# HKUDS/GPT-ST

Measured on AMD Instinct MI355X. Metric: pretrain steps/sec at (B=32,T=12,N=170,C=64), higher is better.
Workload: dtype f32; 1 GPU; BASELINE configs[1]: PEMS08-shape synthetic pretrain step, per-GPU B=32 T=12 N=170 C=64 base=1, epoch 200/300 (adaptive mask + KL), fwd+loss+bwd+clip+Adam, hipGraph=True, 4 full optimiser steps on 4 different resident batches per graph replay; global_batch=32, parallelism=dp1

## Files before the change

### gpt-st_amd/csrc/hypertem.hip

```cpp
#include "mfma_tile.h"
#include "wgrad64.h"
#include "kl_guest.h"
GPTST_STAMP_TABLES(hypertem)
GPTST_HANDOFF_COUNTER(hypertem)

#define HT_T 12
#ifndef HT_OCC
#define HT_OCC 2
#endif
#ifdef GPTST_DEBUG
__device__ long long g_ht_ts[64];
static thread_local int g_ht_dbg = 0, g_ht_nt_override = 0;
extern "C" int gptst_ht_dbg(int v) { g_ht_dbg = v; return 0; }
extern "C" int gptst_ht_variant(int fwd, int bwd) { g_ht_nt_override = fwd; (void)bwd; return 0; }
extern "C" int gptst_ht_ts(long long* out) { return (int)hipMemcpyFromSymbol(out, HIP_SYMBOL(g_ht_ts), sizeof(long long) * 64); }
#define HT_DBG(d) (d)
#else
#define HT_DBG(d) 0
static constexpr int g_ht_dbg = 0, g_ht_nt_override = 0;
#endif

__device__ __forceinline__ bool ht_work_at(int L, int ntiles, int B, int& b, int& tile) {
    const int xcd = L & 7, slot = L >> 3;
    b = xcd + 8 * (slot / ntiles);
    tile = slot % ntiles;
    return b < B;
}
__device__ __forceinline__ bool ht_work(int ntiles, int B, int& b, int& tile) { return ht_work_at(blockIdx.x, ntiles, B, b, tile); }

static int ht_pick_nt(int B, int N) {
    if (g_ht_nt_override >= 4 && g_ht_nt_override <= 16) return g_ht_nt_override;
    (void)B; (void)N;
    return 16;
}

__global__ __launch_bounds__(256, HT_OCC) void hypertem_fwd_kernel(const float* __restrict__ X, const float* __restrict__ G,
                                                              const float* __restrict__ Wbt, const float* __restrict__ bbt,
                                                              float* __restrict__ R_out, float* __restrict__ out, int N, int B, int NT,
                                                              int dbg) {
    constexpr int C = 64, P = C + 4, GP = 145;
    int tsi = 0;
#ifdef GPTST_DEBUG
#define TS() do { if ((dbg & 1) && blockIdx.x == 59 && threadIdx.x == 0) g_ht_ts[tsi] = clock64(); ++tsi; } while (0)
#else
#define TS() __builtin_amdgcn_sched_barrier(0)
#endif
    TS();
    extern __shared__ __attribute__((aligned(16))) float smem[];
    float* Xs = smem;
    float* Gs = Xs + HT_T * NT * P;
    int b, tile;
    if (!ht_work((N + NT - 1) / NT, B, b, tile)) return;
    const int n0 = tile * NT;
    const int tid = threadIdx.x, lane = tid & 63, wave = tid >> 6;
    {
        const int nl = tid >> 4, c4 = tid & 15;
        const int n = min(n0 + nl, N - 1);
        float4 v[HT_T];
        float gv[9];
#pragma unroll
        for (int t = 0; t < HT_T; ++t) v[t] = ld4(X + (((size_t)b * HT_T + t) * N + n) * C + 4 * c4);
#pragma unroll
        for (int k = 0; k < 9; ++k) gv[k] = G[min(n0 * 144 + tid + k * 256, N * 144 - 1)];
        if (nl < NT) {
#pragma unroll
            for (int t = 0; t < HT_T; ++t) st4(Xs + (t * NT + nl) * P + 4 * c4, n0 + nl < N ? v[t] : f4zero());
        }
#pragma unroll
        for (int k = 0; k < 9; ++k) {
            const int i = tid + k * 256;
            if (i < NT * 144) Gs[(i / 144) * GP + i % 144] = (n0 + i / 144 < N) ? gv[k] : 0.f;
        }
    }
    __syncthreads();
    TS();
    const int j = lane & 15, kk = lane >> 4;
    const int ja = j < NT ? j : 0;
    float4 bv[C / 16][4];
    float4 b4;
#define HT_LOAD_W(tt) do {                                                                                         \
        const float* W_ = Wbt + ((size_t)b * HT_T + (tt)) * C * C;                                                 \
        _Pragma("unroll") for (int q = 0; q < C / 16; ++q)                                                         \
            _Pragma("unroll") for (int e = 0; e < 4; ++e) bv[q][e] = ld4(W_ + (size_t)(16 * q + 4 * kk + e) * C + 4 * j); \
        b4 = ld4(bbt + ((size_t)b * HT_T + (tt)) * C + 4 * j);                                                     \
    } while (0)
    HT_LOAD_W(wave);
    for (int t = wave; t < HT_T; t += 4) {
        const size_t g = (size_t)b * HT_T + t;
        TS();
        float4 a4[C / 16];
#pragma unroll
        for (int q = 0; q < C / 16; ++q) a4[q] = f4zero();
        {
            const float* gr = Gs + ja * GP + t * HT_T;
            const float* xr = Xs + ja * P + 4 * kk;
#pragma unroll
            for (int u = 0; u < HT_T; ++u) {
                const float gu = gr[u];
#pragma unroll
                for (int q = 0; q < C / 16; ++q) a4[q] = f4fma(gu, ld4(xr + u * NT * P + 16 * q), a4[q]);
            }
        }
        TS();
        f32x4 acc[C / 16];
#pragma unroll
        for (int ct = 0; ct < C / 16; ++ct) acc[ct] = (f32x4){0.f, 0.f, 0.f, 0.f};
#pragma unroll
        for (int q = 0; q < C / 16; ++q) {
            const float av[4] = {a4[q].x, a4[q].y, a4[q].z, a4[q].w};
#pragma unroll
            for (int e = 0; e < 4; ++e) {
                acc[0] = __builtin_amdgcn_mfma_f32_16x16x4f32(av[e], bv[q][e].x, acc[0], 0, 0, 0);
                acc[1] = __builtin_amdgcn_mfma_f32_16x16x4f32(av[e], bv[q][e].y, acc[1], 0, 0, 0);
                acc[2] = __builtin_amdgcn_mfma_f32_16x16x4f32(av[e], bv[q][e].z, acc[2], 0, 0, 0);
                acc[3] = __builtin_amdgcn_mfma_f32_16x16x4f32(av[e], bv[q][e].w, acc[3], 0, 0, 0);
            }
        }
        TS();
        const float4 bias = b4;
        if (t + 4 < HT_T) HT_LOAD_W(t + 4);
        TS();
        if (R_out != nullptr && j < NT && n0 + j < N) {
#pragma unroll
            for (int q = 0; q < C / 16; ++q) st4_far(R_out + (g * N + n0 + j) * C + 16 * q + 4 * kk, a4[q]);
        }
#pragma unroll
        for (int r = 0; r < 4; ++r) {
            const int nl = kk * 4 + r;
            if (nl < NT && n0 + nl < N) {
                float4 y = f4add(f4add(make_float4(acc[0][r], acc[1][r], acc[2][r], acc[3][r]), bias), ld4(Xs + (t * NT + nl) * P + 4 * j));
                y.x = lrelu(y.x); y.y = lrelu(y.y); y.z = lrelu(y.z); y.w = lrelu(y.w);
                st4(out + (g * N + n0 + nl) * C + 4 * j, y);
            }
        }
        TS();
    }
}

static size_t ht_smem(int NT) { return ((size_t)HT_T * NT * 68 + NT * 145) * sizeof(float); }

extern "C" int gptst_hypertem_fwd(const float* X, const float* G, const float* Wbt, const float* bbt, float* R_out, float* out, int B,
                                  int T, int N, int C, void* stream) {
    if (!X || !G || !Wbt || !bbt || !out || T != HT_T) return GPTST_EARG;
    if (C != 64) return GPTST_ESHAPE;
    static int done = 0;
    if (!done) { hipFuncSetAttribute((const void*)hypertem_fwd_kernel, hipFuncAttributeMaxDynamicSharedMemorySize, (int)ht_smem(16)); done = 1; }
    const int NT = ht_pick_nt(B, N);
    hipLaunchKernelGGL(hypertem_fwd_kernel, dim3(8 * ((B + 7) / 8) * ((N + NT - 1) / NT)), dim3(256), ht_smem(NT), (hipStream_t)stream, X, G, Wbt, bbt, R_out, out, N, B, NT, g_ht_dbg);
    GPTST_CHECK_LAUNCH();
    return GPTST_OK;
}

template <bool HASY, bool PREMUL, int PAIR>
__device__ __forceinline__ void hypertem_bwd_stage(const float* __restrict__ dOut, const float* __restrict__ Y,
                                                   const float* __restrict__ X, const float* __restrict__ G,
                                                   const float* __restrict__ Wbt, float* __restrict__ dX,
                                                   float* __restrict__ dbias, float* __restrict__ dG, int N, int B, int dbg, int b, int tile,
                                                   float* __restrict__ smem, float4 (&dp)[HT_T]) {
    constexpr int C = 64, P = C + 4, GP = 145, NT = 16;
    float* Ds = smem;
    float* Gs = Ds + HT_T * NT * P;
    const int n0 = tile * NT;
    const int tid = threadIdx.x, lane = tid & 63, wave = tid >> 6;
    const int nl = tid >> 4, c4 = tid & 15;
    const bool valid = n0 + nl < N;
    const size_t rowoff = ((size_t)b * HT_T * N + min(n0 + nl, N - 1)) * C + 4 * c4;
    const int j = lane & 15, kk = lane >> 4;
    float4 aq[C / 16][C / 16];
#define HT_LOAD_WT(tt) do {                                                                                         \
        const float* W_ = Wbt + ((size_t)b * HT_T + (tt)) * C * C;                                                  \
        _Pragma("unroll") for (int it = 0; it < C / 16; ++it)                                                       \
            _Pragma("unroll") for (int q = 0; q < C / 16; ++q) aq[it][q] = ld4(W_ + (size_t)(it * 16 + j) * C + 16 * q + 4 * kk); \
    } while (0)
    static_assert(!(HASY && PREMUL), "one sign operand per launch");
    const float* __restrict__ Sg = HASY ? Y : X;
    float4 yv[HT_T];
    float gv[9];
    unsigned sb0 = 0u, sb1 = 0u;
#pragma unroll
    for (int t = 0; t < 4; ++t) { if (PAIR != 2) dp[t] = ld4(dOut + rowoff + (size_t)t * N * C); if (HASY || PREMUL) yv[t] = ld4(Sg + rowoff + (size_t)t * N * C); }
#pragma unroll
    for (int k = 0; k < 9; ++k) gv[k] = G[min(n0 * 144 + tid + k * 256, N * 144 - 1)];
    HT_LOAD_WT(wave);
#pragma unroll
    for (int t = 4; t < HT_T; ++t) { if (PAIR != 2) dp[t] = ld4(dOut + rowoff + (size_t)t * N * C); if (HASY || PREMUL) yv[t] = ld4(Sg + rowoff + (size_t)t * N * C); }
    SB();
#pragma unroll
    for (int grp = 0; grp < HT_T / 4; ++grp) {
#pragma unroll
        for (int tt = 0; tt < 4; ++tt) {
            const int t = 4 * grp + tt;
            float4 v = dp[t];
            if (HASY) v = make_float4(dp[t].x * lrelu_grad_from_out(yv[t].x), dp[t].y * lrelu_grad_from_out(yv[t].y),
                                      dp[t].z * lrelu_grad_from_out(yv[t].z), dp[t].w * lrelu_grad_from_out(yv[t].w));
            if (PREMUL) {
                const unsigned m4 = (yv[t].x > 0.f ? 1u : 0u) | (yv[t].y > 0.f ? 2u : 0u) | (yv[t].z > 0.f ? 4u : 0u) | (yv[t].w > 0.f ? 8u : 0u);
                if (t < 8) sb0 |= m4 << (4 * t); else sb1 |= m4 << (4 * (t - 8));
            }
            if (!valid) v = f4zero();
            dp[t] = v;
            st4(Ds + (t * NT + nl) * P + 4 * c4, v);
        }
        if (grp == 0) {
#pragma unroll
            for (int k = 0; k < 9; ++k) {
                const int i = tid + k * 256;
                Gs[(i / 144) * GP + i % 144] = (n0 + i / 144 < N) ? gv[k] : 0.f;
            }
        }
        __syncthreads();
        SB();
        if (PAIR != 0 && grp == 0) GPTST_STAMP(PAIR == 2 ? 6 : 1);
        const int t = 4 * grp + wave;
        if (HT_DBG(dbg) & 32) continue;
        const size_t g = (size_t)b * HT_T + t;
        float* dt = Ds + t * NT * P;
        float s = 0.f;
        if (dbias != nullptr) {
#pragma unroll
            for (int r = 0; r < NT; ++r) s += dt[r * P + lane];
        }
        float4 bq[C / 16];
#pragma unroll
        for (int q = 0; q < C / 16; ++q) bq[q] = ld4(dt + j * P + 16 * q + 4 * kk);
        f32x4 acc[C / 16];
#pragma unroll
        for (int it = 0; it < C / 16; ++it) acc[it] = (f32x4){0.f, 0.f, 0.f, 0.f};
        if (!(HT_DBG(dbg) & 64))
#pragma unroll
        for (int q = 0; q < C / 16; ++q) {
#pragma unroll
            for (int it = 0; it < C / 16; ++it) acc[it] = __builtin_amdgcn_mfma_f32_16x16x4f32(aq[it][q].x, bq[q].x, acc[it], 0, 0, 0);
#pragma unroll
            for (int it = 0; it < C / 16; ++it) acc[it] = __builtin_amdgcn_mfma_f32_16x16x4f32(aq[it][q].y, bq[q].y, acc[it], 0, 0, 0);
#pragma unroll
            for (int it = 0; it < C / 16; ++it) acc[it] = __builtin_amdgcn_mfma_f32_16x16x4f32(aq[it][q].z, bq[q].z, acc[it], 0, 0, 0);
#pragma unroll
            for (int it = 0; it < C / 16; ++it) acc[it] = __builtin_amdgcn_mfma_f32_16x16x4f32(aq[it][q].w, bq[q].w, acc[it], 0, 0, 0);
        }
        SB();
        if (t + 4 < HT_T && !(HT_DBG(dbg) & 128)) HT_LOAD_WT(t + 4);
        SB();
        if (dbias != nullptr && !(HT_DBG(dbg) & 4)) dbias[((size_t)tile * B * HT_T + g) * C + lane] = s;
#pragma unroll
        for (int it = 0; it < C / 16; ++it)
            st4(dt + j * P + it * 16 + kk * 4, make_float4(acc[it][0], acc[it][1], acc[it][2], acc[it][3]));
    }
    __syncthreads();
    if (PAIR != 0) GPTST_STAMP(PAIR == 2 ? 7 : 2);
    float4 xg[NT / 4][C / 16];
#pragma unroll
    for (int i = 0; i < NT / 4; ++i) {
        const int n = min(n0 + wave + 4 * i, N - 1);
#pragma unroll
        for (int q = 0; q < C / 16; ++q)
            xg[i][q] = j < HT_T ? ld4(X + (((size_t)b * HT_T + j) * N + n) * C + 16 * q + 4 * kk) : f4zero();
    }
    SB();
    if (valid && !(HT_DBG(dbg) & 16)) {
        float4 dr[HT_T];
#pragma unroll
        for (int t = 0; t < HT_T; ++t) dr[t] = ld4(Ds + (t * NT + nl) * P + 4 * c4);
        const float* gr = Gs + nl * GP;
#pragma unroll
        for (int u = 0; u < HT_T; ++u) {
            float4 acc = dp[u];
#pragma unroll
            for (int t = 0; t < HT_T; ++t) acc = f4fma(gr[t * HT_T + u], dr[t], acc);
            if (PREMUL) {
                const unsigned m4 = (u < 8 ? sb0 >> (4 * u) : sb1 >> (4 * (u - 8))) & 15u;
                acc.x *= (m4 & 1u) ? 1.f : LRELU_SLOPE; acc.y *= (m4 & 2u) ? 1.f : LRELU_SLOPE;
                acc.z *= (m4 & 4u) ? 1.f : LRELU_SLOPE; acc.w *= (m4 & 8u) ? 1.f : LRELU_SLOPE;
            }
            if (PAIR == 1) {
                const __amdgpu_buffer_rsrc_t rs = __builtin_amdgcn_make_buffer_rsrc(dX + (size_t)b * HT_T * N * C, 0, HT_T * N * C * 4, 0x00020000);
                st4_sc1(rs, (int)(((size_t)u * N + n0 + nl) * C + 4 * c4) * 4, acc);
                dp[u] = acc;
            } else if (!(HT_DBG(dbg) & 8)) st4(dX + rowoff + (size_t)u * N * C, acc);
            SB();
        }
    }
    SB();
    if (PAIR != 0) GPTST_STAMP(PAIR == 2 ? 8 : 3);
#pragma unroll
    for (int i = 0; i < NT / 4; ++i) {
        const int nn = wave + 4 * i, n = n0 + nn;
        if (n >= N) continue;
        f32x4 acc = {0.f, 0.f, 0.f, 0.f};
#pragma unroll
        for (int q = 0; q < C / 16; ++q) {
            const float4 a = j < HT_T ? ld4(Ds + (j * NT + nn) * P + 16 * q + 4 * kk) : f4zero();
            const float4 x = xg[i][q];
            acc = __builtin_amdgcn_mfma_f32_16x16x4f32(a.x, x.x, acc, 0, 0, 0);
            acc = __builtin_amdgcn_mfma_f32_16x16x4f32(a.y, x.y, acc, 0, 0, 0);
            acc = __builtin_amdgcn_mfma_f32_16x16x4f32(a.z, x.z, acc, 0, 0, 0);
            acc = __builtin_amdgcn_mfma_f32_16x16x4f32(a.w, x.w, acc, 0, 0, 0);
        }
#pragma unroll
        for (int r = 0; r < 4; ++r) {
            const int t = kk * 4 + r, u = j;
            if (t < HT_T && u < HT_T && !(HT_DBG(dbg) & 2)) dG[((size_t)b * N + n) * 144 + t * HT_T + u] = acc[r];
        }
    }
    if (PAIR != 0) GPTST_STAMP(PAIR == 2 ? 9 : 4);
}

template <bool HASY, bool PREMUL>
__device__ __forceinline__ void hypertem_bwd_body(const float* __restrict__ dOut, const float* __restrict__ Y,
                                                  const float* __restrict__ X, const float* __restrict__ G,
                                                  const float* __restrict__ Wbt, float* __restrict__ dX,
                                                  float* __restrict__ dbias, float* __restrict__ dG, int N, int B, int dbg, int L,
                                                  float* __restrict__ smem) {
    int b, tile;
    if (!ht_work_at(L, (N + 15) / 16, B, b, tile)) return;
    float4 dp[HT_T];
    hypertem_bwd_stage<HASY, PREMUL, 0>(dOut, Y, X, G, Wbt, dX, dbias, dG, N, B, dbg, b, tile, smem, dp);
}

template <bool HASY, bool PREMUL>
__global__ __launch_bounds__(256, HT_OCC) void hypertem_bwd_kernel(const float* __restrict__ dOut, const float* __restrict__ Y,
                                                              const float* __restrict__ X, const float* __restrict__ G,
                                                              const float* __restrict__ Wbt, float* __restrict__ dX,
                                                              float* __restrict__ dbias, float* __restrict__ dG, int N, int B, int dbg) {
    extern __shared__ __attribute__((aligned(16))) float smem[];
    hypertem_bwd_body<HASY, PREMUL>(dOut, Y, X, G, Wbt, dX, dbias, dG, N, B, dbg, blockIdx.x, smem);
}

template <bool HASY>
__device__ __forceinline__ void wgrad64_mix_body(const float* __restrict__ X, const float* __restrict__ G, const float* __restrict__ D,
                                                 const float* __restrict__ D2, float* __restrict__ dW, int N, int b, int t,
                                                 float* __restrict__ smem) {
    constexpr int C = 64, U = 2;
    float (*red)[C * C] = reinterpret_cast<float (*)[C * C]>(smem);
    float (*csred)[C] = reinterpret_cast<float (*)[C]>(smem + 4 * C * C);
    const int lane = threadIdx.x & 63, wave = threadIdx.x >> 6;
    const int j = lane & 15, kk = lane >> 4;
    const int q = (N + 3) / 4;
    const int mbeg = wave * q, mend = min(N, mbeg + q);
    const size_t g = (size_t)b * HT_T + t;
    f32x4 acc[4][4];
#pragma unroll
    for (int ca = 0; ca < 4; ++ca)
#pragma unroll
        for (int cb = 0; cb < 4; ++cb) acc[ca][cb] = (f32x4){0.f, 0.f, 0.f, 0.f};
    float4 sa = f4zero();
    for (int m0 = mbeg; m0 < mend; m0 += 4 * U) {
        float4 x[U][HT_T], gq[U][3], d[U], y[U];
#pragma unroll
        for (int u = 0; u < U; ++u) {
            const int m = min(m0 + 4 * u + kk, mend - 1);
#pragma unroll
            for (int k = 0; k < 3; ++k) gq[u][k] = ld4(G + (size_t)m * 144 + t * HT_T + 4 * k);
#pragma unroll
            for (int uu = 0; uu < HT_T; ++uu) x[u][uu] = ld4(X + (((size_t)b * HT_T + uu) * N + m) * C + 4 * j);
            const size_t off = (g * N + m) * C + 4 * j;
            d[u] = ld4(D + off);
            if (HASY) y[u] = ld4(D2 + off);
        }
        SB();
#pragma unroll
        for (int u = 0; u < U; ++u) {
            const float gs[HT_T] = {gq[u][0].x, gq[u][0].y, gq[u][0].z, gq[u][0].w, gq[u][1].x, gq[u][1].y, gq[u][1].z, gq[u][1].w,
                                    gq[u][2].x, gq[u][2].y, gq[u][2].z, gq[u][2].w};
            float4 a = f4zero();
#pragma unroll
            for (int uu = 0; uu < HT_T; ++uu) a = f4fma(gs[uu], x[u][uu], a);
            if (m0 + 4 * u + kk >= mend) a = f4zero();
            if (HASY) {
                d[u].x = __fmul_rn(d[u].x, lrelu_grad_from_out(y[u].x)); d[u].y = __fmul_rn(d[u].y, lrelu_grad_from_out(y[u].y));
                d[u].z = __fmul_rn(d[u].z, lrelu_grad_from_out(y[u].z)); d[u].w = __fmul_rn(d[u].w, lrelu_grad_from_out(y[u].w));
            }
            if (m0 + 4 * u + kk < mend) sa = make_float4(__fadd_rn(sa.x, d[u].x), __fadd_rn(sa.y, d[u].y), __fadd_rn(sa.z, d[u].z), __fadd_rn(sa.w, d[u].w));
            const float av[4] = {a.x, a.y, a.z, a.w}, dv[4] = {d[u].x, d[u].y, d[u].z, d[u].w};
#pragma unroll
            for (int ca = 0; ca < 4; ++ca)
#pragma unroll
                for (int cb = 0; cb < 4; ++cb) acc[ca][cb] = __builtin_amdgcn_mfma_f32_16x16x4f32(av[ca], dv[cb], acc[ca][cb], 0, 0, 0);
        }
        SB();
    }
#pragma unroll
    for (int ca = 0; ca < 4; ++ca)
#pragma unroll
        for (int r = 0; r < 4; ++r)
            st4(&red[wave][(4 * (kk * 4 + r) + ca) * C + 4 * j], make_float4(acc[ca][0][r], acc[ca][1][r], acc[ca][2][r], acc[ca][3][r]));
    sa.x += __shfl_xor(sa.x, 16, 64); sa.y += __shfl_xor(sa.y, 16, 64); sa.z += __shfl_xor(sa.z, 16, 64); sa.w += __shfl_xor(sa.w, 16, 64);
    sa.x += __shfl_xor(sa.x, 32, 64); sa.y += __shfl_xor(sa.y, 32, 64); sa.z += __shfl_xor(sa.z, 32, 64); sa.w += __shfl_xor(sa.w, 32, 64);
    if (kk == 0) st4(&csred[wave][4 * j], sa);
    __syncthreads();
    float* o = dW + g * (size_t)(C * C + C);
    if (threadIdx.x < C) o[C * C + threadIdx.x] = csred[0][threadIdx.x] + csred[1][threadIdx.x] + csred[2][threadIdx.x] + csred[3][threadIdx.x];
#pragma unroll
    for (int k = 0; k < C * C / 4 / 256; ++k) {
        const int f = threadIdx.x + k * 256;
        const float4 s = f4add(f4add(ld4(&red[0][4 * f]), ld4(&red[1][4 * f])), f4add(ld4(&red[2][4 * f]), ld4(&red[3][4 * f])));
        st4(o + 4 * f, s);
    }
}

template <int U, bool HASY, bool PREMUL, bool MIX>
__global__ __launch_bounds__(256, HT_OCC) void hypertem_bwd_wgrad_kernel(const float* __restrict__ dOut, const float* __restrict__ Y,
                                                                    const float* __restrict__ X, const float* __restrict__ G,
                                                                    const float* __restrict__ Wbt, const float* __restrict__ R,
                                                                    float* __restrict__ dX, float* __restrict__ dG, float* __restrict__ dWb,
                                                                    int N, int B, int nH, RowMap rm, int rows_per_split) {
    extern __shared__ __attribute__((aligned(16))) float smem[];
    if ((int)blockIdx.x < nH) {
        hypertem_bwd_body<HASY, PREMUL>(dOut, Y, X, G, Wbt, dX, nullptr, dG, N, B, 0, blockIdx.x, smem);
    } else if (MIX) {
        int b, t;
        if (!ht_work_at(blockIdx.x - nH, HT_T, B, b, t)) return;
        wgrad64_mix_body<HASY>(X, G, dOut, Y, dWb, N, b, t, smem);
    } else {
        const int w = blockIdx.x - nH;
        wgrad64_body<HASY ? PRO_DPRE : PRO_NONE, U>(R, dOut, Y, dWb, rm, rows_per_split, 64 * 64 + 64, 2, w % rm.G, w / rm.G, smem);
    }
}

extern "C" int gptst_hypertem_ntiles(int N) { return (N + 15) / 16; }

extern "C" int gptst_hypertem_bwd(const float* dOut, const float* Y, const float* X, const float* G, const float* Wbt, float* dX,
                                  float* dbias, float* dG, int premul, int B, int T, int N, int C, void* stream) {
    if (!dOut || !X || !G || !Wbt || !dX || !dG || T != HT_T || (Y && premul)) return GPTST_EARG;
    if (C != 64) return GPTST_ESHAPE;
    const size_t smem = ht_smem(16);
    static int done = 0;
    if (!done) {
        hipFuncSetAttribute((const void*)hypertem_bwd_kernel<true, false>, hipFuncAttributeMaxDynamicSharedMemorySize, (int)smem);
        hipFuncSetAttribute((const void*)hypertem_bwd_kernel<false, false>, hipFuncAttributeMaxDynamicSharedMemorySize, (int)smem);
        hipFuncSetAttribute((const void*)hypertem_bwd_kernel<false, true>, hipFuncAttributeMaxDynamicSharedMemorySize, (int)smem);
        done = 1;
    }
    const dim3 grid(8 * ((B + 7) / 8) * ((N + 15) / 16));
    if (Y) hipLaunchKernelGGL((hypertem_bwd_kernel<true, false>), grid, dim3(256), smem, (hipStream_t)stream, dOut, Y, X, G, Wbt, dX, dbias, dG, N, B, g_ht_dbg);
    else if (premul) hipLaunchKernelGGL((hypertem_bwd_kernel<false, true>), grid, dim3(256), smem, (hipStream_t)stream, dOut, Y, X, G, Wbt, dX, dbias, dG, N, B, g_ht_dbg);
    else hipLaunchKernelGGL((hypertem_bwd_kernel<false, false>), grid, dim3(256), smem, (hipStream_t)stream, dOut, Y, X, G, Wbt, dX, dbias, dG, N, B, g_ht_dbg);
    GPTST_CHECK_LAUNCH();
    return GPTST_OK;
}

extern "C" int gptst_wgrad_nsplit(int mode, int BT, int N, int C);
template <bool HASY, bool PREMUL>
static void ht_bwd_wgrad_launch(const float* dOut, const float* Y, const float* X, const float* G, const float* Wbt, const float* R, float* dX,
                                float* dG, float* dWb, int B, int N, bool u6, int nH, int nW, RowMap rm, int rps, size_t smem, hipStream_t st) {
    static int done = 0;
    if (!done) {
        hipFuncSetAttribute((const void*)hypertem_bwd_wgrad_kernel<4, HASY, PREMUL, false>, hipFuncAttributeMaxDynamicSharedMemorySize, (int)smem);
        hipFuncSetAttribute((const void*)hypertem_bwd_wgrad_kernel<6, HASY, PREMUL, false>, hipFuncAttributeMaxDynamicSharedMemorySize, (int)smem);
        hipFuncSetAttribute((const void*)hypertem_bwd_wgrad_kernel<4, HASY, PREMUL, true>, hipFuncAttributeMaxDynamicSharedMemorySize, (int)smem);
        done = 1;
    }
    if (R == nullptr) hipLaunchKernelGGL((hypertem_bwd_wgrad_kernel<4, HASY, PREMUL, true>), dim3(nH + 8 * ((B + 7) / 8) * HT_T), dim3(256), smem, st, dOut, Y, X, G, Wbt, R, dX, dG, dWb, N, B, nH, rm, rps);
    else if (u6) hipLaunchKernelGGL((hypertem_bwd_wgrad_kernel<6, HASY, PREMUL, false>), dim3(nH + nW), dim3(256), smem, st, dOut, Y, X, G, Wbt, R, dX, dG, dWb, N, B, nH, rm, rps);
    else hipLaunchKernelGGL((hypertem_bwd_wgrad_kernel<4, HASY, PREMUL, false>), dim3(nH + nW), dim3(256), smem, st, dOut, Y, X, G, Wbt, R, dX, dG, dWb, N, B, nH, rm, rps);
}

extern "C" int gptst_hypertem_bwd_wgrad(const float* dOut, const float* Y, const float* X, const float* G, const float* Wbt, const float* R,
                                        float* dX, float* dG, float* dWb, int premul, int B, int T, int N, int C, void* stream) {
    if (!dOut || !X || !G || !Wbt || !dX || !dG || !dWb || T != HT_T || (Y && premul)) return GPTST_EARG;
    if (C != 64) return GPTST_ESHAPE;
    const size_t smem_h = ht_smem(16), smem_w = WGRAD64_SMEM_FLOATS * sizeof(float), smem = smem_h > smem_w ? smem_h : smem_w;
    const RowMap rm = make_rowmap(0, B * T, N);
    const int ns = gptst_wgrad_nsplit(0, B * T, N, 64);
    if (!R && ns != 1) return GPTST_ESHAPE;
    int rps = (rm.M + ns - 1) / ns;
    rps = (rps + 1) & ~1;
    const int rows = rps < rm.M ? rps : rm.M, steps = ((rows + 3) / 4 + 3) / 4;
    const bool u6 = (steps + 5) / 6 * 6 <= (steps + 3) / 4 * 4;
    const int nH = 8 * ((B + 7) / 8) * ((N + 15) / 16), nW = rm.G * ns;
    if (Y) ht_bwd_wgrad_launch<true, false>(dOut, Y, X, G, Wbt, R, dX, dG, dWb, B, N, u6, nH, nW, rm, rps, smem, (hipStream_t)stream);
    else if (premul) ht_bwd_wgrad_launch<false, true>(dOut, Y, X, G, Wbt, R, dX, dG, dWb, B, N, u6, nH, nW, rm, rps, smem, (hipStream_t)stream);
    else ht_bwd_wgrad_launch<false, false>(dOut, Y, X, G, Wbt, R, dX, dG, dWb, B, N, u6, nH, nW, rm, rps, smem, (hipStream_t)stream);
    GPTST_CHECK_LAUNCH();
    return GPTST_OK;
}

struct HtPairArgs {
    const float* dOut1; const float* X1; const float* G1; const float* Wbt1; const float* R1;
    const float* X0; const float* G0; const float* Wbt0; const float* R0;
    float* dXmid; float* dX0; float* dG1; float* dG0; float* dWb1; float* dWb0; unsigned* cnt;
};

template <int U>
__global__ __launch_bounds__(256, HT_OCC) void hypertem_bwd_pair_kernel(HtPairArgs a, int N, int B, int nH, RowMap rm, int rows_per_split) {
    extern __shared__ __attribute__((aligned(16))) float smem[];
    const int ntiles = (N + 15) / 16;
    if ((int)blockIdx.x < nH) {
        int b, tile;
        if (!ht_work_at(blockIdx.x, ntiles, B, b, tile)) return;
        float4 dp[HT_T];
        GPTST_WG_BEGIN(); GPTST_STAMP(0);
        hypertem_bwd_stage<false, true, 1>(a.dOut1, nullptr, a.X1, a.G1, a.Wbt1, a.dXmid, nullptr, a.dG1, N, B, 0, b, tile, smem, dp);
        asm volatile("s_waitcnt vmcnt(0)" ::: "memory");
        __syncthreads();
        if (threadIdx.x == 0) { gptst_publish_fence(); __hip_atomic_fetch_add(a.cnt + b, 1u, __ATOMIC_RELAXED, __HIP_MEMORY_SCOPE_AGENT); }
        GPTST_STAMP(5);
        hypertem_bwd_stage<false, true, 2>(nullptr, nullptr, a.X0, a.G0, a.Wbt0, a.dX0, nullptr, a.dG0, N, B, 0, b, tile, smem, dp);
        GPTST_WG_END();
        return;
    }
    GPTST_WG_BEGIN();
    const int nW = rm.G * ((rm.M + rows_per_split - 1) / rows_per_split);
    int w = blockIdx.x - nH;
    if (w < nW) {
        wgrad64_body<PRO_NONE, U>(a.R1, a.dOut1, nullptr, a.dWb1, rm, rows_per_split, 64 * 64 + 64, 2, w % rm.G, w / rm.G, smem);
        GPTST_WG_END();
        return;
    }
    w -= nW;
    const int g = w % rm.G, sp = w / rm.G;
    unsigned* s_ok = reinterpret_cast<unsigned*>(smem);
    if (threadIdx.x == 0) *s_ok = gptst_wait_ge(a.cnt + g / HT_T, (unsigned)ntiles, &g_handoff_lost_hypertem) ? 1u : 0u;
    __syncthreads();
    const bool ok = *s_ok != 0u;
    __syncthreads();
    wgrad64_body<PRO_NONE, U, true>(a.R0, a.dXmid, nullptr, a.dWb0, rm, rows_per_split, 64 * 64 + 64, 2, g, sp, smem);
    if (!ok) a.dWb0[((size_t)sp * rm.G + g) * (size_t)(64 * 64 + 64) + threadIdx.x] = __int_as_float(0x7fc00000);
    GPTST_WG_END();
}

extern "C" int gptst_hypertem_bwd_pair(const float* dOut1, const float* X1, const float* G1, const float* Wbt1, const float* R1, const float* X0,
                                       const float* G0, const float* Wbt0, const float* R0, float* dXmid, float* dX0, float* dG1, float* dG0,
                                       float* dWb1, float* dWb0, void* cnt, int B, int T, int N, int C, void* stream) {
    if (!dOut1 || !X1 || !G1 || !Wbt1 || !R1 || !X0 || !G0 || !Wbt0 || !R0 || !dXmid || !dX0 || !dG1 || !dG0 || !dWb1 || !dWb0 || !cnt || T != HT_T)
        return GPTST_EARG;
    if (C != 64 || (size_t)HT_T * N * C * 4 >= ((size_t)1 << 31)) return GPTST_ESHAPE;
    const size_t smem_h = ht_smem(16), smem_w = WGRAD64_SMEM_FLOATS * sizeof(float), smem = smem_h > smem_w ? smem_h : smem_w;
    const RowMap rm = make_rowmap(0, B * T, N);
    const int ns = gptst_wgrad_nsplit(0, B * T, N, 64);
    int rps = (rm.M + ns - 1) / ns;
    rps = (rps + 1) & ~1;
    if ((rm.M + rps - 1) / rps != ns || (size_t)B * T * N * C * 4 >= ((size_t)1 << 31)) return GPTST_ESHAPE;
    const int rows = rps < rm.M ? rps : rm.M, steps = ((rows + 3) / 4 + 3) / 4;
    const bool u6 = (steps + 5) / 6 * 6 <= (steps + 3) / 4 * 4;
    const int nH = 8 * ((B + 7) / 8) * ((N + 15) / 16), nW = rm.G * ns;
    static int done = 0;
    if (!done) {
        hipFuncSetAttribute((const void*)hypertem_bwd_pair_kernel<4>, hipFuncAttributeMaxDynamicSharedMemorySize, (int)smem);
        hipFuncSetAttribute((const void*)hypertem_bwd_pair_kernel<6>, hipFuncAttributeMaxDynamicSharedMemorySize, (int)smem);
        done = 1;
    }
    const HtPairArgs a{dOut1, X1, G1, Wbt1, R1, X0, G0, Wbt0, R0, dXmid, dX0, dG1, dG0, dWb1, dWb0, (unsigned*)cnt};
    if (u6) hipLaunchKernelGGL((hypertem_bwd_pair_kernel<6>), dim3(nH + 2 * nW), dim3(256), smem, (hipStream_t)stream, a, N, B, nH, rm, rps);
    else hipLaunchKernelGGL((hypertem_bwd_pair_kernel<4>), dim3(nH + 2 * nW), dim3(256), smem, (hipStream_t)stream, a, N, B, nH, rm, rps);
    GPTST_CHECK_LAUNCH();
    return GPTST_OK;
}

struct HtStage { const float* G; const float* Wbt; const float* bbt; float* R_out; float* out; };
struct HtChain {
    int nstage;
    const float* X;
    HtStage st[3];
};

#ifndef HTC_NW
#define HTC_NW 4
#endif
template <int NSTAGE, int GUEST>
__global__ __launch_bounds__(64 * HTC_NW, HTC_NW == 6 ? 3 : HT_OCC) void hypertem_chain_fwd_kernel(HtChain ch, int N, int B, KlGuest kg) {
    constexpr int C = 64, P = C + 4, GP = 145, NT = 16, NW = HTC_NW, NTH = 64 * NW, TPW = HT_T / NW;
    static_assert(HT_T % NW == 0 && (HT_T * NT * (C / 4)) % NTH == 0 && (NT * 144) % NTH == 0, "waves must divide the steps and the staging loops");
    constexpr int GK = NT * 144 / NTH, XK = HT_T * NT * (C / 4) / NTH;
    extern __shared__ __attribute__((aligned(16))) float smem[];
    float* Xs = smem;
    float* Gs = Xs + HT_T * NT * P;
    if constexpr (GUEST != 0) {
        static_assert(NTH == 256, "the guest bodies are written for 256 threads");
        if ((int)blockIdx.x >= kg.base) { kl_guest_run<GUEST>(kg, kg.v0 + (int)blockIdx.x - kg.base, smem); return; }
    }
    int b, tile;
    if (!ht_work((N + NT - 1) / NT, B, b, tile)) return;
    const int n0 = tile * NT;
    const int tid = threadIdx.x, lane = tid & 63, wave = tid >> 6;
    const int j = lane & 15, kk = lane >> 4;
    float gv[GK];
#define HTC_LOAD_G(Gp) _Pragma("unroll") for (int k = 0; k < GK; ++k) gv[k] = (Gp)[min(n0 * 144 + tid + k * NTH, N * 144 - 1)]
#define HTC_STORE_G() _Pragma("unroll") for (int k = 0; k < GK; ++k) { const int i = tid + k * NTH; \
        Gs[(i / 144) * GP + i % 144] = (n0 + i / 144 < N) ? gv[k] : 0.f; }
    float4 bv[C / 16][4];
    float4 b4;
#define HTC_LOAD_W(W0, b0, tt) do {                                                                                \
        const float* W_ = (W0) + ((size_t)b * HT_T + (tt)) * C * C;                                                \
        _Pragma("unroll") for (int q = 0; q < C / 16; ++q)                                                         \
            _Pragma("unroll") for (int e = 0; e < 4; ++e) bv[q][e] = ld4(W_ + (size_t)(16 * q + 4 * kk + e) * C + 4 * j); \
        b4 = ld4((b0) + ((size_t)b * HT_T + (tt)) * C + 4 * j);                                                    \
    } while (0)

    {
        float4 v[XK];
#pragma unroll
        for (int k = 0; k < XK; ++k) {
            const int i = tid + k * NTH, t = i >> 8, nl = (i & 255) >> 4, c4 = i & 15;
            v[k] = ld4(ch.X + (((size_t)b * HT_T + t) * N + min(n0 + nl, N - 1)) * C + 4 * c4);
        }
        HTC_LOAD_G(ch.st[0].G);
#pragma unroll
        for (int k = 0; k < XK; ++k) {
            const int i = tid + k * NTH, t = i >> 8, nl = (i & 255) >> 4, c4 = i & 15;
            st4(Xs + (t * NT + nl) * P + 4 * c4, n0 + nl < N ? v[k] : f4zero());
        }
        HTC_STORE_G();
    }
    __syncthreads();
    SB();

#pragma unroll
    for (int s = 0; s < NSTAGE; ++s) {
        const HtStage S = ch.st[s];
        const HtStage S1 = ch.st[s + 1 < 3 ? s + 1 : 2];
        if (s + 1 < NSTAGE) {
            float4 a4a[C / 16], a4b[C / 16], a4c[C / 16];
#pragma unroll
            for (int q = 0; q < C / 16; ++q) { a4a[q] = f4zero(); a4b[q] = f4zero(); a4c[q] = f4zero(); }
            {
                const float* gr = Gs + j * GP + wave * HT_T;
                const float* xr = Xs + j * P + 4 * kk;
#pragma unroll
                for (int u = 0; u < HT_T; ++u) {
                    float4 x[C / 16];
#pragma unroll
                    for (int q = 0; q < C / 16; ++q) x[q] = ld4(xr + u * NT * P + 16 * q);
                    const float g0 = gr[u], g1 = gr[NW * HT_T + u], g2 = TPW == 3 ? gr[2 * NW * HT_T + u] : 0.f;
#pragma unroll
                    for (int q = 0; q < C / 16; ++q) {
                        a4a[q] = f4fma(g0, x[q], a4a[q]);
                        a4b[q] = f4fma(g1, x[q], a4b[q]);
                        if (TPW == 3) a4c[q] = f4fma(g2, x[q], a4c[q]);
                    }
                    if (TPW == 3 ? u % 3 == 2 : u % 2 == 1) SB();
                }
            }
            HTC_LOAD_W(S.Wbt, S.bbt, wave);
            HTC_LOAD_G(S1.G);
            __syncthreads();
            SB();
#pragma nounroll
            for (int ti = 0; ti < TPW; ++ti) {
                const int t = wave + NW * ti;
                const size_t g = (size_t)b * HT_T + t;
                float4 m4[C / 16];
#pragma unroll
                for (int q = 0; q < C / 16; ++q) { m4[q] = a4a[q]; a4a[q] = a4b[q]; a4b[q] = a4c[q]; }
                f32x4 acc[C / 16];
#pragma unroll
                for (int ct = 0; ct < C / 16; ++ct) acc[ct] = (f32x4){0.f, 0.f, 0.f, 0.f};
#pragma unroll
                for (int q = 0; q < C / 16; ++q) {
                    const float av[4] = {m4[q].x, m4[q].y, m4[q].z, m4[q].w};
#pragma unroll
                    for (int e = 0; e < 4; ++e) {
                        acc[0] = __builtin_amdgcn_mfma_f32_16x16x4f32(av[e], bv[q][e].x, acc[0], 0, 0, 0);
                        acc[1] = __builtin_amdgcn_mfma_f32_16x16x4f32(av[e], bv[q][e].y, acc[1], 0, 0, 0);
                        acc[2] = __builtin_amdgcn_mfma_f32_16x16x4f32(av[e], bv[q][e].z, acc[2], 0, 0, 0);
                        acc[3] = __builtin_amdgcn_mfma_f32_16x16x4f32(av[e], bv[q][e].w, acc[3], 0, 0, 0);
                    }
                }
                SB();
                const float4 bias = b4;
                if (ti < TPW - 1) HTC_LOAD_W(S.Wbt, S.bbt, t + NW);
                SB();
                if (S.R_out != nullptr && n0 + j < N) {
#pragma unroll
                    for (int q = 0; q < C / 16; ++q) st4_far(S.R_out + (g * N + n0 + j) * C + 16 * q + 4 * kk, m4[q]);
                }
#pragma unroll
                for (int r = 0; r < 4; ++r) {
                    const int nl = kk * 4 + r;
                    float* xs = Xs + (t * NT + nl) * P + 4 * j;
                    float4 y = f4add(f4add(make_float4(acc[0][r], acc[1][r], acc[2][r], acc[3][r]), bias), ld4(xs));
                    y.x = lrelu(y.x); y.y = lrelu(y.y); y.z = lrelu(y.z); y.w = lrelu(y.w);
                    if (n0 + nl < N) st4(S.out + (g * N + n0 + nl) * C + 4 * j, y);
                    else y = f4zero();
                    st4(xs, y);
                }
                SB();
            }
            HTC_STORE_G();
            __syncthreads();
            SB();
        } else {
            HTC_LOAD_W(S.Wbt, S.bbt, wave);
            for (int t = wave; t < HT_T; t += NW) {
                const size_t g = (size_t)b * HT_T + t;
                SB();
                float4 a4[C / 16];
#pragma unroll
                for (int q = 0; q < C / 16; ++q) a4[q] = f4zero();
                {
                    const float* gr = Gs + j * GP + t * HT_T;
                    const float* xr = Xs + j * P + 4 * kk;
#pragma unroll
                    for (int u = 0; u < HT_T; ++u) {
                        const float gu = gr[u];
#pragma unroll
                        for (int q = 0; q < C / 16; ++q) a4[q] = f4fma(gu, ld4(xr + u * NT * P + 16 * q), a4[q]);
                    }
                }
                SB();
                f32x4 acc[C / 16];
#pragma unroll
                for (int ct = 0; ct < C / 16; ++ct) acc[ct] = (f32x4){0.f, 0.f, 0.f, 0.f};
#pragma unroll
                for (int q = 0; q < C / 16; ++q) {
                    const float av[4] = {a4[q].x, a4[q].y, a4[q].z, a4[q].w};
#pragma unroll
                    for (int e = 0; e < 4; ++e) {
                        acc[0] = __builtin_amdgcn_mfma_f32_16x16x4f32(av[e], bv[q][e].x, acc[0], 0, 0, 0);
                        acc[1] = __builtin_amdgcn_mfma_f32_16x16x4f32(av[e], bv[q][e].y, acc[1], 0, 0, 0);
                        acc[2] = __builtin_amdgcn_mfma_f32_16x16x4f32(av[e], bv[q][e].z, acc[2], 0, 0, 0);
                        acc[3] = __builtin_amdgcn_mfma_f32_16x16x4f32(av[e], bv[q][e].w, acc[3], 0, 0, 0);
                    }
                }
                SB();
                const float4 bias = b4;
                if (t + NW < HT_T) HTC_LOAD_W(S.Wbt, S.bbt, t + NW);
                SB();
                if (S.R_out != nullptr && n0 + j < N) {
#pragma unroll
                    for (int q = 0; q < C / 16; ++q) st4_far(S.R_out + (g * N + n0 + j) * C + 16 * q + 4 * kk, a4[q]);
                }
#pragma unroll
                for (int r = 0; r < 4; ++r) {
                    const int nl = kk * 4 + r;
                    if (n0 + nl < N) {
                        float4 y = f4add(f4add(make_float4(acc[0][r], acc[1][r], acc[2][r], acc[3][r]), bias), ld4(Xs + (t * NT + nl) * P + 4 * j));
                        y.x = lrelu(y.x); y.y = lrelu(y.y); y.z = lrelu(y.z); y.w = lrelu(y.w);
                        st4(S.out + (g * N + n0 + nl) * C + 4 * j, y);
                    }
                }
            }
        }
    }
#undef HTC_LOAD_G
#undef HTC_STORE_G
#undef HTC_LOAD_W
}

static int ht_chain_args(HtChain& ch, const float* X, int nstage, const void* Gs, const void* Wbts, const void* bbts, const void* Rs, const void* outs,
                         int B, int T, int N, int C) {
    if (!X || nstage < 1 || nstage > 3 || !Gs || !Wbts || !bbts || !Rs || !outs || T != HT_T || B <= 0 || N <= 0) return GPTST_EARG;
    if (C != 64) return GPTST_ESHAPE;
    ch.nstage = nstage; ch.X = X;
    for (int s = 0; s < 3; ++s) {
        const int k = s < nstage ? s : nstage - 1;
        ch.st[s] = HtStage{((const float* const*)Gs)[k], ((const float* const*)Wbts)[k], ((const float* const*)bbts)[k],
                           ((float* const*)Rs)[k], ((float* const*)outs)[k]};
        if (!ch.st[s].G || !ch.st[s].Wbt || !ch.st[s].bbt || !ch.st[s].out) return GPTST_EARG;
    }
    return GPTST_OK;
}

static int ht_chain_grid(int B, int N) { return 8 * ((B + 7) / 8) * ((N + 15) / 16); }

extern "C" int gptst_hypertem_chain_fwd(const float* X, int nstage, const void* Gs, const void* Wbts, const void* bbts, const void* Rs,
                                        const void* outs, int B, int T, int N, int C, void* stream) {
    HtChain ch;
    const int rc = ht_chain_args(ch, X, nstage, Gs, Wbts, bbts, Rs, outs, B, T, N, C);
    if (rc != GPTST_OK) return rc;
    const dim3 grid(ht_chain_grid(B, N));
    const int smem = (int)ht_smem(16);
    hipStream_t st = (hipStream_t)stream;
    const KlGuest none{};
#define HTC_LAUNCH(NS_) do {                                                                                                          \
        static int done_ = 0;                                                                                                          \
        if (!done_) { (void)hipFuncSetAttribute((const void*)hypertem_chain_fwd_kernel<NS_, 0>, hipFuncAttributeMaxDynamicSharedMemorySize, smem); done_ = 1; } \
        hipLaunchKernelGGL((hypertem_chain_fwd_kernel<NS_, 0>), grid, dim3(64 * HTC_NW), smem, st, ch, N, B, none);                          \
    } while (0)
    if (nstage == 1) HTC_LAUNCH(1); else if (nstage == 2) HTC_LAUNCH(2); else HTC_LAUNCH(3);
#undef HTC_LAUNCH
    GPTST_CHECK_LAUNCH();
    return GPTST_OK;
}

GPTST_INTERNAL int gptst_tail_geometry(int rows, int* rows_per_block);
GPTST_INTERNAL int gptst_apply_wgrad_geometry(int mode, int BT, int N, int* tpw);

extern "C" int gptst_kl_guest_blocks(int stage, int B, int T, int N) {
    if (B <= 0 || T <= 0 || N <= 0) return GPTST_EARG;
    int aux;
    if (stage == 1) return gptst_tail_geometry(B * T * N, &aux);
    if (stage == 2) return B * T * gptst_apply_wgrad_geometry(0, B * T, N, &aux);
    if (stage == 3) return N;
    return GPTST_EARG;
}

extern "C" int gptst_hypertem_chain_fwd_kl(const float* X, int nstage, const void* Gs, const void* Wbts, const void* bbts, const void* Rs,
                                           const void* outs, int B, int T, int N, int C, int stage, const void* ops, int v0, int v1, int HS,
                                           int lda, float w, void* stream) {
    HtChain ch;
    const int rc = ht_chain_args(ch, X, nstage, Gs, Wbts, bbts, Rs, outs, B, T, N, C);
    if (rc != GPTST_OK) return rc;
    if (!ops || stage < 1 || stage > 3) return GPTST_EARG;
    if (nstage != 2 || HTC_NW != 4 || HS <= 0 || HS > TL_MAXJ) return GPTST_ESHAPE;
    const int nv = gptst_kl_guest_blocks(stage, B, T, N);
    if (v0 < 0 || v1 <= v0 || v1 > nv) return GPTST_EARG;
    const float* const* p = (const float* const*)ops;
    const int np = stage == 1 ? 7 : stage == 2 ? 6 : 7;
    for (int i = 0; i < np; ++i) if (!p[i]) return GPTST_EARG;
    KlGuest kg{};
    kg.base = ht_chain_grid(B, N);
    kg.v0 = v0;
    if (stage == 1) {
        TailArgs& t = kg.tail;
        t.X = p[0]; t.W = p[1]; t.prob = p[2]; t.c = p[3]; t.dX = (float*)p[4]; t.part = (float*)p[5]; t.sws = (float*)p[6];
        t.rows = B * T * N; t.J = HS; t.N = N; t.w = w; t.premul = 1;
        gptst_tail_geometry(t.rows, &t.rows_per_block);
    } else if (stage == 2) {
        kg.dOut = p[0]; kg.S = p[1]; kg.W = p[2]; kg.dS = (float*)p[3]; kg.dW = (float*)p[4]; kg.colsum = (float*)p[5];
        kg.rm = make_rowmap(0, B * T, N);
        gptst_apply_wgrad_geometry(0, B * T, N, &kg.tpw);
    } else {
        if (lda <= 0) return GPTST_EARG;
        kg.dPre = p[0]; kg.src = p[1]; kg.lda = lda; kg.w1 = p[2]; kg.b1 = p[3]; kg.Wn = p[4]; kg.dWb = (float*)p[5]; kg.dinp = (float*)p[6];
        kg.BT = B * T; kg.N = N;
    }
    const dim3 grid(kg.base + (v1 - v0));
    const size_t sg = kl_guest_lds_bytes(stage), sh = ht_smem(16);
    const int smem = (int)(sg > sh ? sg : sh);
    hipStream_t st = (hipStream_t)stream;
#define HTC_LAUNCH(G_) do {                                                                                                           \
        static int done_ = 0;                                                                                                          \
        if (!done_) { (void)hipFuncSetAttribute((const void*)hypertem_chain_fwd_kernel<2, G_>, hipFuncAttributeMaxDynamicSharedMemorySize, smem); done_ = 1; } \
        hipLaunchKernelGGL((hypertem_chain_fwd_kernel<2, G_>), grid, dim3(64 * HTC_NW), smem, st, ch, N, B, kg);                           \
    } while (0)
    if (stage == 1) HTC_LAUNCH(1); else if (stage == 2) HTC_LAUNCH(2); else HTC_LAUNCH(3);
#undef HTC_LAUNCH
    GPTST_CHECK_LAUNCH();
    return GPTST_OK;
}
```

### gpt-st_amd/csrc/wgrad64.h

```cpp
#pragma once
#include "common.h"

enum { PRO_NONE = 0, PRO_DPRE = 1 };
enum { EPI_PLAIN = 0, EPI_RES_LRELU = 1, EPI_ADD_DPRE = 2, EPI_LRELU = 3, EPI_ADD_PREMUL = 4, EPI_PREMUL = 5 };

struct RowMap {
    int G, M;
    long rs_g, rs_m;
};

__host__ __device__ inline RowMap make_rowmap(int mode, int BT, int N) {
    RowMap r;
    if (mode == 0) { r.G = BT; r.M = N; r.rs_g = N; r.rs_m = 1; }
    else if (mode == 1) { r.G = N; r.M = BT; r.rs_g = 1; r.rs_m = N; }
    else { r.G = 1; r.M = BT * N; r.rs_g = 0; r.rs_m = 1; }
    return r;
}


#define WGRAD64_SMEM_FLOATS (4 * 64 * 64 + 4 * 64)

template <int PRO, int U, bool ACQ = false>
__device__ __forceinline__ void wgrad64_body(const float* __restrict__ A, const float* __restrict__ D, const float* __restrict__ D2,
                                             float* __restrict__ dW, RowMap rm, int rows_per_split, int ostride, int csa, int g, int sp,
                                             float* __restrict__ smem) {
    constexpr int C = 64;
    float (*red)[C * C] = reinterpret_cast<float (*)[C * C]>(smem);
    float (*csred)[C] = reinterpret_cast<float (*)[C]>(smem + 4 * C * C);
    const int lane = threadIdx.x & 63, wave = threadIdx.x >> 6;
    const int j = lane & 15, kk = lane >> 4;
    const int mbeg0 = sp * rows_per_split;
    const int mend0 = min(rm.M, mbeg0 + rows_per_split);
    const int q = (mend0 - mbeg0 + 3) / 4;
    const int mbeg = mbeg0 + wave * q, mend = min(mend0, mbeg + q);
    f32x4 acc[4][4];
#pragma unroll
    for (int ca = 0; ca < 4; ++ca)
#pragma unroll
        for (int cb = 0; cb < 4; ++cb) acc[ca][cb] = (f32x4){0.f, 0.f, 0.f, 0.f};
    float4 sa = f4zero();
    const __amdgpu_buffer_rsrc_t rsD = __builtin_amdgcn_make_buffer_rsrc(const_cast<float*>(D), 0, ACQ ? (int)((size_t)rm.G * rm.M * C * 4) : 0, 0x00020000);
    for (int m0 = mbeg; m0 < mend; m0 += 4 * U) {
        float4 a[U], d[U], y[U];
#pragma unroll
        for (int u = 0; u < U; ++u) {
            const int m = min(m0 + 4 * u + kk, mend - 1);
            const size_t off = ((size_t)g * rm.rs_g + (size_t)m * rm.rs_m) * C + 4 * j;
            a[u] = ld4(A + off); d[u] = ACQ ? ld4_sc1(rsD, (int)(off * 4)) : ld4(D + off);
            if (PRO == PRO_DPRE) y[u] = ld4(D2 + off);
        }
        SB();
#pragma unroll
        for (int u = 0; u < U; ++u) {
            if (m0 + 4 * u + kk >= mend) a[u] = f4zero();
            if (PRO == PRO_DPRE) {
                d[u].x = __fmul_rn(d[u].x, lrelu_grad_from_out(y[u].x)); d[u].y = __fmul_rn(d[u].y, lrelu_grad_from_out(y[u].y));
                d[u].z = __fmul_rn(d[u].z, lrelu_grad_from_out(y[u].z)); d[u].w = __fmul_rn(d[u].w, lrelu_grad_from_out(y[u].w));
            }
            if (csa == 2) {
                if (m0 + 4 * u + kk < mend) sa = make_float4(__fadd_rn(sa.x, d[u].x), __fadd_rn(sa.y, d[u].y), __fadd_rn(sa.z, d[u].z), __fadd_rn(sa.w, d[u].w));
            }
            else sa = f4add(sa, a[u]);
            const float av[4] = {a[u].x, a[u].y, a[u].z, a[u].w}, dv[4] = {d[u].x, d[u].y, d[u].z, d[u].w};
#pragma unroll
            for (int ca = 0; ca < 4; ++ca)
#pragma unroll
                for (int cb = 0; cb < 4; ++cb) acc[ca][cb] = __builtin_amdgcn_mfma_f32_16x16x4f32(av[ca], dv[cb], acc[ca][cb], 0, 0, 0);
        }
    }
#pragma unroll
    for (int ca = 0; ca < 4; ++ca)
#pragma unroll
        for (int r = 0; r < 4; ++r)
            st4(&red[wave][(4 * (kk * 4 + r) + ca) * C + 4 * j], make_float4(acc[ca][0][r], acc[ca][1][r], acc[ca][2][r], acc[ca][3][r]));
    if (csa) {
        sa.x += __shfl_xor(sa.x, 16, 64); sa.y += __shfl_xor(sa.y, 16, 64); sa.z += __shfl_xor(sa.z, 16, 64); sa.w += __shfl_xor(sa.w, 16, 64);
        sa.x += __shfl_xor(sa.x, 32, 64); sa.y += __shfl_xor(sa.y, 32, 64); sa.z += __shfl_xor(sa.z, 32, 64); sa.w += __shfl_xor(sa.w, 32, 64);
        if (kk == 0) st4(&csred[wave][4 * j], sa);
    }
    __syncthreads();
    float* o = dW + ((size_t)sp * rm.G + g) * (size_t)ostride;
    if (csa && threadIdx.x < C) o[C * C + threadIdx.x] = csred[0][threadIdx.x] + csred[1][threadIdx.x] + csred[2][threadIdx.x] + csred[3][threadIdx.x];
#pragma unroll
    for (int k = 0; k < C * C / 4 / 256; ++k) {
        const int f = threadIdx.x + k * 256;
        const float4 s = f4add(f4add(ld4(&red[0][4 * f]), ld4(&red[1][4 * f])), f4add(ld4(&red[2][4 * f]), ld4(&red[3][4 * f])));
        st4(o + 4 * f, s);
    }
}
```

### gpt-st_amd/engine.py

```python
import contextlib
import os
import threading
from typing import Any, NamedTuple

import torch

from . import _C, ops
from .ops import (EPI_ADD_DPRE, EPI_ADD_PREMUL, EPI_LRELU, EPI_PREMUL, EPI_PLAIN, EPI_RES_LRELU, MODE_NODE, MODE_SHARED, MODE_TIME, PRO_DPRE, PRO_NONE)

TF_NAMES = ("ln_day", "ln_week", "ln1", "ln2", "ln")


class ZeroArena:

    def __init__(self, device):
        self.device, self.buf, self.off, self.need = device, None, 0, 0

    def begin(self, zero=True):
        pending = None
        if self.buf is None or self.buf.numel() < self.need:
            self.buf = torch.zeros(max(self.need, 1), device=self.device) if self.need else None
        elif self.buf is not None:
            if zero:
                self.buf.zero_()
            else:
                pending = self.buf
        self.off, self.need = 0, 0
        return pending

    def zeros(self, *shape):
        n = 1
        for d in shape:
            n *= d
        n4 = (n + 3) // 4 * 4
        self.need += n4
        if self.buf is None or self.off + n4 > self.buf.numel():
            return torch.zeros(*shape, device=self.device)
        t = self.buf[self.off:self.off + n].view(*shape)
        self.off += n4
        return t


class _Context(threading.local):
    ARENA = None
    NODE_REDUCE = None
    NO_HANDOFFS = False


CTX = _Context()




class Reductions:

    def __init__(self):
        self.jobs = ops.PoolJobs()
        self.late = ops.PoolJobs()
        self.no_carry = False
        self.grams = []
        self.tf = []
        self.keep = []
        self.on_bucket = None
        self.nbucket = 0
        self.bucket_inline = False
        self.fork_side = None
        self.forked = False
        self._dG = self._dA = None

    def take_carry(self, mb):
        if not CARRY_RED or self.no_carry or self.on_bucket is not None or CTX.NODE_REDUCE is not None or not self.jobs.jobs:
            return None
        take, rest, nb = [], [], 0.0
        for j in self.jobs.jobs:
            b = 4.0 * j.R * j.cols * j.nsplit / 2 ** 20
            if j.kind in (ops.PoolJobs.BWD_POOL, ops.PoolJobs.BWD_EMB) and nb + b <= mb and len(take) < 100 and (j.cols | j.ldx) % 4 == 0:
                take.append(j); nb += b
            else:
                rest.append(j)
        if not take:
            return None
        self.jobs.jobs = rest
        c = ops.PoolJobs()
        c.jobs = take
        return c

    def untake(self, carry):
        if carry is not None and carry.jobs:
            self.jobs.jobs = carry.jobs + self.jobs.jobs
            carry.jobs = []

    def gram(self, A, dG, dA, N, nsG):
        self.grams.append((A, dG, dA, N, nsG))

    def timefeat(self, p, g, pfx, tidx, dout, spg=False):
        self.tf.append(_tf_job(p, pfx, tidx, spg)._replace(grads=_tf_tensors(g, pfx), dout=dout))

    def flush_async(self, tidx):
        if self.bucket_inline and self.on_bucket is not None and self.nbucket == 0 and (self.jobs.jobs or self.late.jobs or self.grams or self.tf):
            self._run(tidx)
            self.fork_side.wait_stream(torch.cuda.current_stream())
            with torch.cuda.stream(self.fork_side):
                self.on_bucket(0)
            self.forked = True
            self.nbucket += 1

    def flush(self, tidx):
        self._run(tidx)
        if self.forked:
            torch.cuda.current_stream().wait_stream(self.fork_side)
            self.forked = False

    def _run(self, tidx):
        gr, self.grams = sorted(self.grams, key=lambda t: t[0].data_ptr()), []
        while gr:
            A, dG, dA, N, nsG = gr.pop(0)
            while gr and gr[0][0].data_ptr() == A.data_ptr() + 4 * A.numel() and gr[0][1].data_ptr() == dG.data_ptr() + 4 * dG.numel() \
                    and gr[0][2].data_ptr() == dA.data_ptr() + 4 * dA.numel() and gr[0][3:] == (N, nsG):
                A2, dG2, dA2 = gr.pop(0)[:3]
                A = torch.as_strided(A, (A.shape[0] + A2.shape[0],) + tuple(A.shape[1:]), A.stride())
                dG = torch.as_strided(dG, (dG.shape[0] + dG2.shape[0],) + tuple(dG.shape[1:]), dG.stride())
                dA = torch.as_strided(dA, (dA.shape[0] + dA2.shape[0],) + tuple(dA.shape[1:]), dA.stride())
            ops.gram_bwd(A, dG, out=dA, layers=A.shape[0] // N, nsplit=nsG)
        self.jobs.jobs, self.late.jobs = self.jobs.jobs + self.late.jobs, []
        self.jobs.launch()
        tf, self.tf = self.tf, []
        ops.timefeat_jobs_bwd(tf, tidx)
        self.keep = []


def _zeros(ref, *shape):
    if CTX.ARENA is not None:
        return CTX.ARENA.zeros(*shape)
    return torch.zeros(*shape, device=ref.device)


def _tf_tensors(d, pfx):
    out = []
    for n in TF_NAMES:
        out += [d[pfx + n + ".weight"], d[pfx + n + ".bias"]]
    return out


def _tf_job(p, pfx, tidx, spg=False):
    B, T = tidx.shape[0], tidx.shape[1]
    rows, K = (B, T) if spg else (B * T, 1)
    return ops.TimefeatJob(_tf_tensors(p, pfx), rows, K)


DROP_R = os.environ.get("GPTST_DROP_R", "0") == "1"


class HtSaved(NamedTuple):
    x: Any
    R: Any
    out: Any
    G: Any
    Wbt: Any


class WgradParts(NamedTuple):
    dW: Any
    ns: int
    db: Any


def _ht_fused_bwd(dims):
    return dims[3] == 64 and FUSE_HT_BWD


def hypertem_core_fwd(x, G, Wbt, bbt, dims):
    B, T, N, C = dims
    if C == 64:
        keep = not (DROP_R and _ht_fused_bwd(dims) and ops.wgrad_nsplit(MODE_TIME, B * T, N, C) == 1)
        R, out = ops.hypertem_fwd(x.view(B, T, N, C), G, Wbt, bbt, want_R=keep)
        R, out = (R.view(-1, C) if keep else None), out.view(-1, C)
    else:
        R = ops.tmix(x.view(B, T, N, C), G).view(-1, C)
        out = ops.apply(R, Wbt, MODE_TIME, B * T, N, bias=bbt, resid=x, epi=EPI_RES_LRELU)
    return out, HtSaved(x, R, out, G, Wbt)


FUSE_HT_BWD = True


def graph_grad_splits(dims):
    return dims[0] if dims[3] == 64 else 1


CHAIN128 = os.environ.get("GPTST_CHAIN128", "1") == "1"


def chain_ok(dims):
    return _ht_fused_bwd(dims) or (CHAIN128 and dims[3] == 128)


def _wb_parts(dWb, C, ns=1):
    return WgradParts(dWb[:, :C * C], ns, dWb[:, C * C:])


def _wgrad_parts(a, dout, out, mode, dims):
    B, T, N, C = dims
    dWb, ns = ops.wgrad(a, dout, mode, B * T, N, D2=out, pro=PRO_NONE if out is None else PRO_DPRE, colsum_d=True)
    return _wb_parts(dWb, C, ns)


def _genlin_bwd(dout, out, x, W, mode, dims, chain, premul=False):
    B, T, N, C = dims
    BT = B * T
    if C == 64:
        dx, dW, db, ns = ops.apply_wgrad(dout, None if chain else out, x, W, mode, BT, N, premul=chain and premul)
        return dx, WgradParts(dW, ns, db)
    if chain:
        dx = (ops.apply(dout, W, mode, BT, N, transw=True, resid2=x, epi=EPI_PREMUL) if premul
              else ops.apply(dout, W, mode, BT, N, transw=True))
        return dx, _wgrad_parts(x, dout, None, mode, dims)
    dx = ops.apply(dout, W, mode, BT, N, A2=out, transw=True, pro=PRO_DPRE)
    return dx, _wgrad_parts(x, dout, out, mode, dims)


def hypertem_core_bwd(saved, dout, dG_out, dims, chain=False, premul=False):
    B, T, N, C = dims
    x, R, out, G, Wbt = saved
    BT = B * T
    v = lambda a: a.view(B, T, N, C)
    assert not chain or chain_ok(dims)
    if _ht_fused_bwd(dims):
        dx, dWb, ns, _ = ops.hypertem_bwd_wgrad(v(dout), None if chain else v(out), v(x), G, Wbt, v(R) if R is not None else None, dG=dG_out,
                                                premul=chain and premul)
        return dx.view(-1, C), _wb_parts(dWb, C, ns)
    hp = _wgrad_parts(R, dout, None if chain else out, MODE_TIME, dims)
    if C == 64:
        dx, _, _ = ops.hypertem_bwd(v(dout), v(out), v(x), G, Wbt, dG=dG_out, want_dbias=False)
    elif chain:
        dR = ops.apply(dout, Wbt, MODE_TIME, BT, N, transw=True)
        dx, _ = ops.tmix_bwd_chain(v(dR), v(x), G, v(dout), premul=premul, dG=dG_out[0])
    else:
        dR = ops.apply(dout, Wbt, MODE_TIME, BT, N, A2=out, transw=True, pro=PRO_DPRE)
        dx, _ = ops.tmix_bwd(v(dR), v(x), G, v(dout), v(out), dG=dG_out[0])
    return dx.view(-1, C), hp


CARRY_RED = os.environ.get("GPTST_CARRY_RED", "1") == "1"
CARRY_MB = float(os.environ.get("GPTST_CARRY_MB", "25"))
CARRY_KL = os.environ.get("GPTST_CARRY_KL", "1") == "1"
PAIR_UNDER_DP = os.environ.get("GPTST_PAIR_UNDER_DP", "1") == "1"
PAIR_BWD = os.environ.get("GPTST_PAIR_BWD", "1") == "1"


@contextlib.contextmanager
def no_handoffs():
    from . import _C
    keep = (CTX.NO_HANDOFFS, _C.lib().value("gptst_mask_cooperative_state"))
    CTX.NO_HANDOFFS = True
    _C.lib().call("gptst_mask_cooperative", 0)
    try:
        yield
    finally:
        CTX.NO_HANDOFFS = keep[0]
        _C.lib().call("gptst_mask_cooperative", keep[1])


def pair_bwd_on():
    return PAIR_BWD and not CTX.NO_HANDOFFS


def cross_role():
    return 0 if CTX.NO_HANDOFFS else CROSS_ROLE


def _ht_pair_shape_ok(dims):
    B, T, N, C = dims
    if T != 12 or C != 64:
        return False
    ns = ops.wgrad_nsplit(MODE_TIME, B * T, N, C)
    rps = (-(-N // ns) + 1) & ~1
    return -(-N // rps) == ns


def ht_pair_ok(saved1, saved0, dims):
    return (pair_bwd_on() and dims[3] == 64 and not isinstance(saved1, EncIn) and saved1.R is not None and saved0.R is not None
            and _ht_fused_bwd(dims) and _ht_pair_shape_ok(dims))


class PendingH1:

    def __init__(self, saved, dd, dG, dWb):
        self.saved, self.dd, self.dG, self.dWb = saved, dd, dG, dWb


def ht_pair_bwd(saved1, saved0, dout, dG1, dG0, dims, dWb1=None):
    B, T, N, C = dims
    if not ht_pair_ok(saved1, saved0, dims):
        assert dWb1 is None
        return None
    s1, s0 = saved1, saved0
    v = lambda a: a.view(B, T, N, C)
    r = ops.hypertem_bwd_pair(v(dout), v(s1.x), s1.G, s1.Wbt, v(s1.R), v(s0.x), s0.G, s0.Wbt, v(s0.R), dG1, dG0, _zeros(dout, B), dWb1=dWb1)
    assert r is not None or dWb1 is None
    if r is None:
        return None
    dmid, dx0, dWb1, dWb0, ns = r
    return dx0.view(-1, C), _wb_parts(dWb1, C, ns), _wb_parts(dWb0, C, ns)


FUSE_CROSS = os.environ.get("GPTST_FUSE_CROSS", "1") == "1"
CAP_LIN = os.environ.get("GPTST_CAP_LIN", "1") == "1"
CROSS_ROLE = int(os.environ.get("GPTST_CROSS_ROLE", "1"))


class CapSaved(NamedTuple):
    x: Any
    out: Any
    rec: Any
    c: Any
    s: Any
    v: Any
    Ht: Any
    Rt: Any
    dyn: Any
    Wn: Any
    Y: Any


class CapParts(NamedTuple):
    wn: WgradParts
    ddyn: Any
    dlogit: Any


def cap_head_fwd(p, pfx, x, dadj, dyn, dims, num_route, HS, HT):
    B, T, N, C = dims
    c, s, Y = ops.cap_route_fwd(x.view(B, T, N, C), p[pfx + "ln_p.weight"], p[pfx + "ln_p.bias"], dadj, HS, num_route,
                                reduce_nodes=CTX.NODE_REDUCE, want_Y=True)
    fused = ops.cap_cross_rec_fwd(s, dyn, p[pfx + "mask_template"], c, B, T, N, HS, HT) if (FUSE_CROSS and CTX.NODE_REDUCE is None) else None
    if fused is not None:
        v, Ht, Rt, rec = fused
    else:
        v, Ht, Rt = ops.cap_cross_fwd(s, dyn, p[pfx + "mask_template"], B, T, HS, HT)
        rec = ops.cap_rec_fwd(c, v, N, C)
    return rec, c, (s, v, Ht, Rt, Y)


def cap_core_fwd(p, pfx, x, dadj, dyn, Wn, bn, dims, num_route, HS, HT):
    B, T, N, C = dims
    rec, c, (s, v, Ht, Rt, Y) = cap_head_fwd(p, pfx, x, dadj, dyn, dims, num_route, HS, HT)
    out = ops.apply(rec, Wn, MODE_NODE, B * T, N, bias=bn, resid=x, epi=EPI_RES_LRELU)
    return out, c, CapSaved(x, out, rec, c, s, v, Ht, Rt, dyn, Wn, Y)


CHAIN_FWD = os.environ.get("GPTST_CHAIN_FWD", "1") == "1"


def chain_fwd_ok(dims):
    return CHAIN_FWD and dims[3] == 64 and not DROP_R


def ht_chain_fwd(x, stages, dims, kl=None):
    B, T, N, C = dims
    res = ops.hypertem_chain_fwd(x.view(B, T, N, C), stages, guest=kl.guest() if kl is not None else None)
    saved, xin = [], x
    for (G, Wbt, _b), (R, o) in zip(stages, res):
        o = o.view(-1, C)
        saved.append(HtSaved(xin, R.view(-1, C), o, G, Wbt))
        xin = o
    return saved, xin


def cap_core_bwd(p, g, pfx, saved, dout, dims, HS, HT, red, chain=False):
    B, T, N, C = dims
    x, out, rec, c, s, v, Ht, Rt, dyn, Wn, Y = saved
    BT, dev = B * T, x.device
    assert not chain or chain_ok(dims)
    drec, wn = _genlin_bwd(dout, out, rec, Wn, MODE_NODE, dims, chain)
    dc1, dv = ops.cap_rec_bwd(drec, c, v, reduce_nodes=CTX.NODE_REDUCE)
    gw, gb = g[pfx + "ln_p.weight"], g[pfx + "ln_p.bias"]
    if FUSE_CROSS and CAP_LIN and C == 64 and CTX.NODE_REDUCE is None and Y is None:
        carry = red.take_carry(CARRY_MB) if cross_role() and _C.lib().value("gptst_cap_route_roles_ok", B, T, N, C, HS, HT) == 1 else None
        lin = ops.cap_cross_route_lin_bwd(x.view(B, T, N, C), p[pfx + "ln_p.weight"], p[pfx + "ln_p.bias"], c, dc1, dv, s, Rt, Ht, dyn,
                                          p[pfx + "mask_template"], dout, None if chain else out, chain, B, T, HS, HT,
                                          flags=_zeros(x, 4 * B) if cross_role() else None, jobs=carry)
        red.untake(carry)
        if lin is not None:
            dx, dWp, dbp, dlogit, ddyn = lin
            red.jobs.bwd_pool(_ones(dev, dWp.shape[0]), dWp, gw.view(1, C * C))
            red.jobs.bwd_pool(_ones(dev, dbp.shape[0]), dbp, gb.view(1, C))
            return dx, CapParts(wn, ddyn, dlogit)
    fused = None
    if FUSE_CROSS and CTX.NODE_REDUCE is None and Y is None:
        fused = ops.cap_cross_route_bwd(x.view(B, T, N, C), p[pfx + "ln_p.weight"], p[pfx + "ln_p.bias"], c, dc1, dv, s, Rt, Ht, dyn,
                                        p[pfx + "mask_template"], B, T, HS, HT, flags=_zeros(x, 4 * B) if cross_role() else None)
    if fused is not None:
        dY, dlogit, ddyn = fused
    else:
        dS, ddyn = ops.cap_cross_bwd(dv, s, Rt, Ht, dyn, p[pfx + "mask_template"], B, T, HS, HT)
        dY, dlogit = ops.cap_route_bwd(x.view(B, T, N, C), p[pfx + "ln_p.weight"], p[pfx + "ln_p.bias"], c, dc1, dS, Y=Y)
    if C == 64:
        dx, dWp, dbp, ns2 = ops.linear_bwd(dY, x, p[pfx + "ln_p.weight"], dout, None if chain else out, premul=chain)
        red.jobs.bwd_pool(_ones(dev, ns2), dWp, gw.view(1, C * C))
        red.jobs.bwd_pool(_ones(dev, ns2), dbp, gb.view(1, C))
    else:
        if chain:
            dx = ops.apply(dY, p[pfx + "ln_p.weight"], MODE_SHARED, BT, N, resid=dout, resid2=x, epi=EPI_ADD_PREMUL)
        else:
            dx = ops.apply(dY, p[pfx + "ln_p.weight"], MODE_SHARED, BT, N, resid=dout, resid2=out, epi=EPI_ADD_DPRE)
        dWp, ns2 = ops.wgrad(dY, x, MODE_SHARED, BT, N, colsum_a=True)
        wp = _wb_parts(dWp, C, ns2)
        red.jobs.bwd_pool(_ones(dev, ns2), wp.dW, gw.view(1, C * C))
        red.jobs.bwd_pool(_ones(dev, ns2), wp.db, gb.view(1, C))
    return dx, CapParts(wn, ddyn, dlogit)


_ONES = {}


def _ones(dev, n=1):
    if (dev, n) not in _ONES:
        _ONES[(dev, n)] = torch.ones(n, 1, device=dev)
    return _ONES[(dev, n)]


class CondLinSaved(NamedTuple):
    x: Any
    out: Any
    W: Any


def condlin_fwd(x, Wg, bg, mode, dims):
    B, T, N, C = dims
    out = ops.apply(x, Wg, mode, B * T, N, bias=bg, epi=EPI_LRELU)
    return out, CondLinSaved(x, out, Wg)


def condlin_bwd(saved, dout, emb, wpool, bpool, g_wpool, g_bpool, d_emb, mode, dims, red, chain=False, premul=False, carried=None):
    C = dims[3]
    R, K = emb.shape
    assert not chain or chain_ok(dims)
    dx, w = carried if carried is not None else _genlin_bwd(dout, saved.out, saved.x, saved.W, mode, dims, chain, premul)
    ns, db = w.ns, w.db
    dW = w.dW if w.dW.dim() == 2 else w.dW.view(ns * R, C * C)
    red.jobs.bwd_pool(emb, dW, g_wpool.view(K, C * C), nsplit=ns)
    red.jobs.bwd_pool(emb, db, g_bpool, nsplit=ns)
    red.jobs.bwd_emb(dW, wpool.view(K, C * C), d_emb, nsplit=ns)
    red.jobs.bwd_emb(db, bpool, d_emb, nsplit=ns)
    return dx


ENC, DEC = "encoder.STHCN_encode.", "decoder.STHCN_decode."
GUIDE_TF = "encoder.teb4mask."


def _sthcn_names(pfx):
    return [pfx + "hyperTem%d." % i for i in (1, 2, 3, 4)], [pfx + "cap1.", pfx + "cap2."]


class SthcnGen(NamedTuple):
    emb: Any
    A_all: Any
    G_all: Any
    Wb: Any
    Wn: Any
    dadj: Any
    dyn: Any
    hts: Any
    cps: Any
    d: int
    Hm: int
    ds: int
    HS: int
    HT: int
    slot: Any

    def ht(self, i):
        return (self.G_all[i],) + self.Wb[i]


class SthcnSaved(NamedTuple):
    h1: Any
    h2: Any
    h3: Any
    h4: Any
    c1: Any
    c2: Any
    emb: Any
    gen: SthcnGen
    slot: Any


class GenAll(NamedTuple):
    sthcn: Any
    guide: Any
    pending: Any


def _sthcn_gen_jobs(p, pfx, emb, jobs, A_all, dims, G_all, slot=None):
    B, T, N, C = dims
    time_eb, teb, tes = emb
    ne, nes = p[pfx + "node_embeddings"], p[pfx + "node_embeddings_spg"]
    hts, cps = _sthcn_names(pfx)
    adj0 = p[hts[0] + "adj"]
    d, Hm = adj0.shape[0], adj0.shape[1]
    cadj, tadj = p[cps[0] + "adj"], p[cps[0] + "t_adj"]
    ds, HS, HT = cadj.shape[0], cadj.shape[1], tadj.shape[1]
    for i, h in enumerate(hts):
        jobs.fwd(ne, p[h + "adj"].view(d, Hm * T), out=A_all[i])
        jobs.gram(ne, p[h + "adj"].view(d, Hm * T), out=G_all[i], A=A_all[i])
    Wb = [(jobs.fwd(time_eb, p[h + "weights_pool"]), jobs.fwd(time_eb, p[h + "bias_pool"])) for h in hts]
    Wn = [(jobs.fwd(nes, p[c + "weights_spa"]), jobs.fwd(nes, p[c + "bias_spa"])) for c in cps]
    dadj = [jobs.fwd(teb, p[c + "adj"].view(ds, HS * N)) for c in cps]
    dyn = [jobs.fwd(tes, p[c + "t_adj"].view(ds, HT * T * HS)).view(B, HT, T * HS) for c in cps]
    return SthcnGen(emb, A_all, G_all, Wb, Wn, dadj, dyn, hts, cps, d, Hm, ds, HS, HT, slot)


def gen_all(p, tidx, dims, which=(ENC, DEC), guide=True, defer=False):
    B, T, N, C = dims
    tfj = []
    for pfx in which:
        tfj += [_tf_job(p, pfx + "time_feature1.", tidx), _tf_job(p, pfx + "time_feature1_.", tidx),
                _tf_job(p, pfx + "time_feature2.", tidx, spg=True)]
    if guide:
        tfj.append(_tf_job(p, GUIDE_TF, tidx))
    embs = ops.timefeat_jobs_fwd(tfj, tidx)
    jobs = ops.PoolJobs()
    now = ops.PoolJobs() if defer else jobs
    sthcn, gd = {}, None
    L = 4 * len(which)
    if guide:
        gj = now
        m = "encoder.MLP_RL."
        t4m = embs[-1]
        gd = (t4m, gj.fwd(p["encoder.neb4mask"], p[m + "weights_pool_spa"]), gj.fwd(p["encoder.neb4mask"], p[m + "bias_pool_spa"]),
              gj.fwd(t4m, p[m + "weights_pool_tem"]), gj.fwd(t4m, p[m + "bias_pool_tem"]))
    if L:
        adj0 = p[which[0] + "hyperTem1.adj"]
        Hm = adj0.shape[1]
        A_all = torch.empty(L, N, Hm * T, device=tidx.device)
        G_all = torch.empty(L, N, T, T, device=tidx.device)
        for k, pfx in enumerate(which):
            sthcn[pfx] = _sthcn_gen_jobs(p, pfx, embs[3 * k:3 * k + 3], jobs, A_all[4 * k:4 * k + 4], dims, G_all[4 * k:4 * k + 4], (k, len(which)))
    now.launch()
    return GenAll(sthcn, gd, jobs if defer else None)


def sthcn_fwd(p, pfx, tidx, x, dims, num_route, gen=None, head=None, next_gen=None, kl=None):
    if gen is None:
        gen = gen_all(p, tidx, dims, which=(pfx,), guide=False).sthcn[pfx]
    ht = gen.ht
    cap = lambda i, x: cap_core_fwd(p, gen.cps[i], x, gen.dadj[i], gen.dyn[i], *gen.Wn[i], dims, num_route, gen.HS, gen.HT)
    pairs = chain_fwd_ok(dims)
    nhead = None
    x, h1 = head if head is not None else hypertem_core_fwd(x, *ht(0), dims)
    x, c1, sc1 = cap(0, x)
    if pairs:
        if kl is not None and kl.c1 is None:
            kl.c1 = c1
        (h2, h3), x = ht_chain_fwd(x, [ht(1), ht(2)], dims, kl)
    else:
        x, h2 = hypertem_core_fwd(x, *ht(1), dims)
        x, h3 = hypertem_core_fwd(x, *ht(2), dims)
    x, _, sc2 = cap(1, x)
    if pairs and next_gen is not None:
        (h4, h1n), xn = ht_chain_fwd(x, [ht(3), next_gen.ht(0)], dims, kl)
        x, nhead = h4.out, (xn, h1n)
    else:
        x, h4 = hypertem_core_fwd(x, *ht(3), dims)
    return x, c1, SthcnSaved(h1, h2, h3, h4, sc1, sc2, gen.emb, gen, gen.slot), nhead


def _grad_buffers(red, slot, N, T, HmT, ref, nsG):
    if slot is None:
        return torch.empty(4, nsG, N, T, T, device=ref.device), torch.empty(4, N, HmT, device=ref.device)
    k, n = slot
    if red._dG is None or red._dG.shape[0] != 4 * n:
        red._dG = torch.empty(4 * n, nsG, N, T, T, device=ref.device)
        red._dA = torch.empty(4 * n, N, HmT, device=ref.device)
    return red._dG[4 * k:4 * k + 4], red._dA[4 * k:4 * k + 4]


def sthcn_bwd(p, g, pfx, tidx, sv, dout, dims, red, chain=False, premul_in=False, defer_h1=False, after_pending=None):
    B, T, N, C = dims
    time_eb, teb, tes = sv.emb
    gn = sv.gen
    A_all, hts, cps, d, Hm, ds, HS, HT = gn.A_all, gn.hts, gn.cps, gn.d, gn.Hm, gn.ds, gn.HS, gn.HT
    ne, nes = p[pfx + "node_embeddings"], p[pfx + "node_embeddings_spg"]
    dne, dnes = g[pfx + "node_embeddings"], g[pfx + "node_embeddings_spg"]
    d_te, d_teb, d_tes = _zeros(time_eb, *time_eb.shape), _zeros(teb, *teb.shape), _zeros(tes, *tes.shape)
    nsG = graph_grad_splits(dims)
    dG_all, dA_all = _grad_buffers(red, sv.slot, N, T, Hm * T, dout, nsG)
    J = red.jobs
    CC, BT = C * C, B * T

    def queue_ht(h, hp):
        J.bwd_pool(time_eb, hp.dW, g[h + "weights_pool"].view(d, CC), nsplit=hp.ns)
        J.bwd_pool(time_eb, hp.db, g[h + "bias_pool"], nsplit=hp.ns)
        J.bwd_emb(hp.dW, p[h + "weights_pool"].view(d, CC), d_te, nsplit=hp.ns)
        J.bwd_emb(hp.db, p[h + "bias_pool"], d_te, nsplit=hp.ns)

    def queue_cap(c, cp):
        w, ns = cp.wn, cp.wn.ns
        dW2 = w.dW if w.dW.dim() == 2 else w.dW.view(ns * N, CC)
        J.bwd_pool(nes, dW2, g[c + "weights_spa"].view(d, CC), nsplit=ns)
        J.bwd_pool(nes, w.db, g[c + "bias_spa"], nsplit=ns)
        J.bwd_emb(dW2, p[c + "weights_spa"].view(d, CC), dnes, nsplit=ns)
        J.bwd_emb(w.db, p[c + "bias_spa"], dnes, nsplit=ns)
        dd2 = cp.ddyn.view(B, HT * T * HS)
        J.bwd_pool(tes, dd2, g[c + "t_adj"].view(ds, HT * T * HS))
        J.bwd_emb(dd2, p[c + "t_adj"].view(ds, HT * T * HS), d_tes)
        dl2 = cp.dlogit.view(BT, HS * N)
        J.bwd_pool(teb, dl2, g[c + "adj"].view(ds, HS * N))
        J.bwd_emb(dl2, p[c + "adj"].view(ds, HS * N), d_teb)

    if isinstance(dout, PendingH1):
        up = dout
        dd, _, hp4 = ht_pair_bwd(up.saved, sv.h4, up.dd, up.dG, dG_all[3], dims, dWb1=up.dWb)
        red.keep.append(up)
        if after_pending is not None:
            after_pending()
    else:
        dd, hp4 = hypertem_core_bwd(sv.h4, dout, dG_all[3], dims, chain, True)
    queue_ht(hts[3], hp4)
    dd, cp2 = cap_core_bwd(p, g, cps[1], sv.c2, dd, dims, HS, HT, red, chain)
    queue_cap(cps[1], cp2)
    pair = ht_pair_bwd(sv.h3, sv.h2, dd, dG_all[2], dG_all[1], dims) if chain and pair_bwd_on() else None
    if pair is not None:
        dd, hp3, hp2 = pair
    else:
        dd, hp3 = hypertem_core_bwd(sv.h3, dd, dG_all[2], dims, chain, True)
        dd, hp2 = hypertem_core_bwd(sv.h2, dd, dG_all[1], dims, chain, True)
    queue_ht(hts[2], hp3)
    queue_ht(hts[1], hp2)
    dd, cp1 = cap_core_bwd(p, g, cps[0], sv.c1, dd, dims, HS, HT, red, chain)
    queue_cap(cps[0], cp1)
    if isinstance(sv.h1, EncIn):
        assert chain
        e = sv.h1
        w, bi = p["encoder.dim_in_flow.weight"], p["encoder.dim_in_flow.bias"]
        if nsG == B:
            dWb, _, dinp = ops.encin_ht1_bwd(dd.view(B, T, N, C), e.source, e.mask, e.fill, w, bi, e.Wbt, e.ab, e.wv, dG=dG_all[0])
        else:
            dWb, dGb, dinp = ops.encin_ht1_bwd(dd.view(B, T, N, C), e.source, e.mask, e.fill, w, bi, e.Wbt, e.ab, e.wv)
            torch.sum(dGb, 0, out=dG_all[0][0])
        hp1 = _wb_parts(dWb, C)
        wb = _wb_view(g["encoder.dim_in_flow.weight"], g["encoder.dim_in_flow.bias"])
        if wb is not None:
            red.jobs.bwd_pool(_ones(dd.device, dinp.shape[0]), dinp, wb)
        else:
            g["encoder.dim_in_flow.weight"].add_(dinp[:, :C].sum(0).view(C, 1))
            g["encoder.dim_in_flow.bias"].add_(dinp[:, C:].sum(0))
        red.keep.append((dinp, dWb))
        dd = None
    elif defer_h1:
        assert chain and premul_in
        ns = ops.wgrad_nsplit(MODE_TIME, B * T, N, C)
        dWb = torch.empty(ns * B * T, C * C + C, device=dd.device, dtype=torch.float32)
        hp1 = _wb_parts(dWb, C, ns)
        dd = PendingH1(sv.h1, dd, dG_all[0], dWb)
    else:
        dd, hp1 = hypertem_core_bwd(sv.h1, dd, dG_all[0], dims, chain, premul_in)
    queue_ht(hts[0], hp1)
    red.gram(A_all.view(4 * N, Hm, T), dG_all, dA_all.view(4 * N, Hm, T), N, nsG)
    for i, h in enumerate(hts):
        red.late.bwd_pool(ne, dA_all[i], g[h + "adj"].view(d, Hm * T))
        red.late.bwd_emb(dA_all[i], p[h + "adj"].view(d, Hm * T), dne)
    red.timefeat(p, g, pfx + "time_feature1.", tidx, d_te)
    red.timefeat(p, g, pfx + "time_feature1_.", tidx, d_teb)
    red.timefeat(p, g, pfx + "time_feature2.", tidx, d_tes, spg=True)
    red.keep.append((sv, hp1, hp2, hp3, hp4, cp1, cp2, dout))
    return dd


class EncIn:

    def __init__(self, source, mask, fill, Wbt, ab, wv):
        self.source, self.mask, self.fill, self.Wbt, self.ab, self.wv = source, mask, fill, Wbt, ab, wv


ENCIN = os.environ.get("GPTST_ENCIN", "1") == "1"


def encin_ok(dims, base):
    return ENCIN and base == 1 and dims[3] in (64, 128) and dims[1] == 12 and chain_ok(dims)


GUIDEIN = os.environ.get("GPTST_GUIDEIN", "1") == "1"
GUIDE_HEAD = os.environ.get("GPTST_GUIDE_HEAD", "1") == "1"


class LowRankIn(NamedTuple):
    Wspa: Any


class GuideSaved(NamedTuple):
    t4m: Any
    spa: Any
    tem: Any
    h2: Any
    label: Any


def guide_fwd(p, source, tidx, dims, base, gen=None, lowrank_in=False):
    B, T, N, C = dims
    if gen is None:
        gen = gen_all(p, tidx, dims, which=(), guide=True).guide
    t4m, Wspa, bspa, Wtem, btem = gen
    m = "encoder.MLP_RL."
    if lowrank_in and GUIDEIN and GUIDE_HEAD and base == 1 and C == 64:
        r = ops.guide_head_fwd(source, p[m + "ln1.weight"], p[m + "ln1.bias"], Wspa, bspa, Wtem, btem, p[m + "ln3.weight"], p[m + "ln3.bias"])
        if r is not None:
            h1, h2, prob, label = r
            return prob, GuideSaved(t4m, LowRankIn(Wspa), CondLinSaved(h1, h2, Wtem), h2, label)
    if lowrank_in and GUIDEIN and base == 1 and C in (64, 128):
        h1 = ops.guide_in_fwd(source, p[m + "ln1.weight"], p[m + "ln1.bias"], Wspa, bspa)
        s1 = LowRankIn(Wspa)
    else:
        h0 = ops.lin_in(source, base + 2, base, p[m + "ln1.weight"], p[m + "ln1.bias"], C)
        h1, s1 = condlin_fwd(h0, Wspa, bspa, MODE_NODE, dims)
    h2, s2 = condlin_fwd(h1, Wtem, btem, MODE_TIME, dims)
    prob, label = ops.rowdot(h2, p[m + "ln3.weight"], p[m + "ln3.bias"], softmax=True, want_label=True)
    return prob, GuideSaved(t4m, s1, s2, h2, label)


def _wb_view(gw, gb):
    n = gw.numel() + gb.numel()
    if gb.data_ptr() != gw.data_ptr() + 4 * gw.numel():
        return None
    return torch.as_strided(gw, (1, n), (n, 1))


def fused_tails_ok(p, C, base, HS):
    return (C in (64, 128) and base <= ops.TAIL_MAXJ and HS <= ops.TAIL_MAXJ
            and _wb_view(p["decoder.dim_flow_out.weight"], p["decoder.dim_flow_out.bias"]) is not None
            and _wb_view(p["encoder.MLP_RL.ln3.weight"], p["encoder.MLP_RL.ln3.bias"]) is not None)


def loss_tail(p, g, dec, source, mask, base, sigma, mu, thresh, sws, red, chain=False):
    wo = "decoder.dim_flow_out."
    out, dd, part = ops.tail_mae(dec, p[wo + "weight"], p[wo + "bias"], source, base + 2, mask, sigma, mu, thresh, sws, premul=chain)
    red.jobs.bwd_pool(_ones(dec.device, part.shape[0]), part, _wb_view(g[wo + "weight"], g[wo + "bias"]))
    red.keep.append((part, dd))
    return out, dd


def kl_head(p, g, sv_g, prob, c1, N, w, sws, red, chain=False, carried=None):
    m = "encoder.MLP_RL."
    dh2, part = carried if carried is not None else ops.tail_kl(sv_g.h2, p[m + "ln3.weight"], prob, c1, N, w, sws, premul=chain)
    red.jobs.bwd_pool(_ones(prob.device, part.shape[0]), part, _wb_view(g[m + "ln3.weight"], g[m + "ln3.bias"]))
    red.keep.append((part, dh2))
    return dh2


def _linear_out_bwd(p, g, pfx, h, dy, C, chain, d_h=None):
    J = dy.shape[1]
    dh = ops.lin_in(dy, J, J, p[pfx + "weight"], None, C, wlayout=1)
    ops.rowouter(dy, J, J, h, g[pfx + "weight"], 1, asum=g[pfx + "bias"])
    if d_h is not None:
        dh = dh + d_h
    if chain:
        dh = dh * torch.where(h > 0, 1.0, 0.01)
    return dh


def guide_bwd(p, g, source, tidx, saved, dlogit, dims, base, red, dh2=None, chain=False, carried=None):
    B, T, N, C = dims
    carried = carried or KlOut()
    t4m, s1, s2, h2 = saved.t4m, saved.spa, saved.tem, saved.h2
    m = "encoder.MLP_RL."
    if dh2 is None:
        dh2 = _linear_out_bwd(p, g, m + "ln3.", h2, dlogit, C, chain)
    d_t4m = _zeros(t4m, *t4m.shape)
    dh1 = condlin_bwd(s2, dh2, t4m, p[m + "weights_pool_tem"], p[m + "bias_pool_tem"], g[m + "weights_pool_tem"],
                      g[m + "bias_pool_tem"], d_t4m, MODE_TIME, dims, red, chain, True, carried=carried.tem)
    if isinstance(s1, LowRankIn):
        assert chain
        neb, wpool, bpool = p["encoder.neb4mask"], p[m + "weights_pool_spa"], p[m + "bias_pool_spa"]
        K = neb.shape[1]
        dWb, dinp = carried.inp if carried.inp is not None else ops.guide_in_bwd(dh1, source, p[m + "ln1.weight"], p[m + "ln1.bias"], s1.Wspa)
        w = _wb_parts(dWb, C)
        red.jobs.bwd_pool(neb, w.dW, g[m + "weights_pool_spa"].view(K, C * C))
        red.jobs.bwd_pool(neb, w.db, g[m + "bias_pool_spa"])
        red.jobs.bwd_emb(w.dW, wpool.view(K, C * C), g["encoder.neb4mask"])
        red.jobs.bwd_emb(w.db, bpool, g["encoder.neb4mask"])
        wb = _wb_view(g[m + "ln1.weight"], g[m + "ln1.bias"])
        if wb is not None:
            red.jobs.bwd_pool(_ones(dh1.device, N), dinp, wb)
        else:
            g[m + "ln1.weight"].add_(dinp[:, :C].sum(0).view(C, 1))
            g[m + "ln1.bias"].add_(dinp[:, C:].sum(0))
        red.keep.append((dWb, dinp))
        dh0 = None
    else:
        dh0 = condlin_bwd(s1, dh1, p["encoder.neb4mask"], p[m + "weights_pool_spa"], p[m + "bias_pool_spa"],
                          g[m + "weights_pool_spa"], g[m + "bias_pool_spa"], g["encoder.neb4mask"], MODE_NODE, dims, red, chain, False)
        _in_proj_grads(source, base, dh0, g[m + "ln1.weight"], g[m + "ln1.bias"], None, 0.0, red)
    red.timefeat(p, g, GUIDE_TF, tidx, d_t4m)
    red.keep.append((saved, dlogit, dh2, dh1, dh0))


def kl_carry_ok(dims, HS, sv_g):
    B, T, N, C = dims
    return (CARRY_KL and C == 64 and T == 12 and HS <= ops.TAIL_MAXJ and chain_fwd_ok(dims) and chain_ok(dims)
            and sv_g is not None and isinstance(sv_g.spa, LowRankIn))


class KlOut:

    def __init__(self):
        self.head = None
        self.tem = None
        self.inp = None


class KlCarry:

    def __init__(self, p, sv_g, prob, source, dims, w, sws):
        self.p, self.sv_g, self.prob, self.source, self.dims, self.w, self.sws = p, sv_g, prob, source, dims, w, sws
        self.c1 = None
        self.stage = 0
        self.out = KlOut()

    def guest(self):
        if self.c1 is None or self.stage == 3:
            return None
        B, T, N, C = self.dims
        m = "encoder.MLP_RL."
        p, sv_g, dev = self.p, self.sv_g, self.prob.device
        HS = self.prob.shape[1]
        st = self.stage + 1
        f = dict(device=dev, dtype=torch.float32)
        if st == 1:
            h2, W3 = sv_g.h2, p[m + "ln3.weight"]
            dh2 = torch.empty_like(h2)
            part = torch.empty(ops.tail_parts(B * T * N), HS * C + HS, **f)
            self.out.head = (dh2, part)
            ts = [h2, W3, self.prob, self.c1, dh2, part, self.sws]
        elif st == 2:
            h1, Wtem = sv_g.tem.x, sv_g.tem.W
            dh2, _ = self.out.head
            ns = _C.lib().value("gptst_apply_wgrad_nsplit", MODE_TIME, B * T, N)
            dh1, dW, db = torch.empty_like(h1), torch.empty(ns * B * T, C * C, **f), torch.empty(ns * B * T, C, **f)
            self.out.tem = (dh1, WgradParts(dW, ns, db))
            ts = [dh2, h1, Wtem, dh1, dW, db]
        else:
            dh1, _ = self.out.tem
            dWb, dinp = torch.empty(N, C * C + C, **f), torch.empty(N, 2 * C, **f)
            self.out.inp = (dWb, dinp)
            ts = [dh1, self.source, p[m + "ln1.weight"], p[m + "ln1.bias"], sv_g.spa.Wspa, dWb, dinp]
        self.stage = st
        return (st, ts, 0, ops.kl_guest_blocks(st, B, T, N), HS, self.source.shape[-1], self.w)


def _in_proj_grads(source, base, dY, gW, gb, mask, fill, red):
    wb = _wb_view(gW, gb)
    if base == 1 and wb is not None:
        C = dY.shape[1]
        part = ops.rowouter_part(source, base + 2, base, dY, mask=mask, fill=fill)
        red.jobs.bwd_pool(_ones(dY.device, part.shape[0]), part[:, :2 * C], wb)
        red.keep.append(part)
    else:
        ops.rowouter(source, base + 2, base, dY, gW, 0, csum=gb, mask=mask, fill=fill)


class Forward(NamedTuple):
    emb: Any
    c1: Any
    dec: Any
    out: Any
    sv_e: Any
    sv_d: Any


def autoencoder_fwd(p, source, mask, dims, base, num_route, scaler_zeros, gen=None, tidx=None, lowrank_in=False, kl=None, head=True,
                    decoder=True, join=True):
    B, T, N, C = dims
    if tidx is None:
        tidx = source[:, :, 0, base:base + 2].contiguous()
    gen_e, gen_d = (gen.sthcn[ENC], gen.sthcn[DEC] if decoder else None) if gen is not None else (None, None)
    first = None
    if lowrank_in and gen_e is not None and encin_ok(dims, base):
        w, bi = p["encoder.dim_in_flow.weight"], p["encoder.dim_in_flow.bias"]
        G1, Wbt1, bbt1 = gen_e.ht(0)
        o1, ab, wv = ops.encin_ht1_fwd(source, base, mask, 0.0 if mask is None else scaler_zeros, w, bi, G1, Wbt1, bbt1)
        first = (o1.view(-1, C), EncIn(source, mask, 0.0 if mask is None else scaler_zeros, Wbt1, ab, wv))
        x0 = None
    else:
        x0 = ops.lin_in(source, base + 2, base, p["encoder.dim_in_flow.weight"], p["encoder.dim_in_flow.bias"], C,
                        mask=mask, fill=scaler_zeros)
    emb, c1, sv_e, dec_h1 = sthcn_fwd(p, ENC, tidx, x0, dims, num_route, gen=gen_e, head=first, next_gen=gen_d if join else None, kl=kl)
    if not decoder:
        return Forward(emb, c1, None, None, sv_e, None)
    dec, _, sv_d, _ = sthcn_fwd(p, DEC, tidx, emb, dims, num_route, gen=gen_d, head=dec_h1, kl=kl)
    out = ops.rowdot(dec, p["decoder.dim_flow_out.weight"], p["decoder.dim_flow_out.bias"]) if head else None
    return Forward(emb, c1, dec, out, sv_e, sv_d)


def model_bwd(p, g, source, mask, tidx, sv_e, sv_d, dec, d_out, d_dec, dims, base, scaler_zeros, red, dd=None, chain=False):
    B, T, N, C = dims
    if dd is None:
        dd = _linear_out_bwd(p, g, "decoder.dim_flow_out.", dec, d_out, C, chain, d_h=d_dec)
    defer = (chain and (red.on_bucket is None or PAIR_UNDER_DP) and not isinstance(sv_d.h1, EncIn)
             and ht_pair_ok(sv_d.h1, sv_e.h4, dims))
    late = defer and red.on_bucket is not None
    d_emb = sthcn_bwd(p, g, DEC, tidx, sv_d, dd, dims, red, chain, True, defer_h1=defer)
    if not late:
        red.flush_async(tidx)
    d_x0 = sthcn_bwd(p, g, ENC, tidx, sv_e, d_emb, dims, red, chain, False,
                     after_pending=(lambda: red.flush_async(tidx)) if late else None)
    red.flush_async(tidx)
    if d_x0 is not None:
        _in_proj_grads(source, base, d_x0, g["encoder.dim_in_flow.weight"], g["encoder.dim_in_flow.bias"], mask, scaler_zeros, red)


def step_bwd(p, g, source, mask, tidx, fw, prob, sv_g, dims, base, scaler_zeros, red, loss, stats, sws=None, with_kl=False, kl=None):
    B, T, N, C = dims
    sigma, mu, thresh = loss
    if sws is not None:
        chain = chain_ok(dims)
        done = kl.out if kl is not None else KlOut()
        _, dd = loss_tail(p, g, fw.dec, source, mask, base, sigma, mu, thresh, sws, red, chain=chain)
        model_bwd(p, g, source, mask, tidx, fw.sv_e, fw.sv_d, fw.dec, None, None, dims, base, scaler_zeros, red, dd=dd, chain=chain)
        if with_kl:
            dh2 = kl_head(p, g, sv_g, prob, fw.c1, N, 0.1, sws, red, chain=chain, carried=done.head)
            guide_bwd(p, g, source, tidx, sv_g, None, dims, base, red, dh2=dh2, chain=chain, carried=done)
    else:
        M = B * T * N
        ops.mae_fwd(fw.out, source, base + 2, mask, sigma, mu, thresh, M, base, stats)
        d_out = ops.mae_bwd(fw.out, source, base + 2, mask, sigma, mu, thresh, M, base, stats, normalize=False)
        model_bwd(p, g, source, mask, tidx, fw.sv_e, fw.sv_d, fw.dec, d_out, None, dims, base, scaler_zeros, red)
        if with_kl:
            dlogit = ops.kl(prob, fw.c1, N, 0.1, stats)
            guide_bwd(p, g, source, tidx, sv_g, dlogit, dims, base, red)


def module_bwd(p, g, source, mask, tidx, fw, prob, sv_g, dims, base, scaler_zeros, red, d_out, d_dec=None, d_prob=None, chain=False):
    model_bwd(p, g, source, mask, tidx, fw.sv_e, fw.sv_d, fw.dec, d_out, d_dec, dims, base, scaler_zeros, red, chain=chain)
    if d_prob is not None:
        dlogit = (prob * (d_prob - (d_prob * prob).sum(-1, keepdim=True))).contiguous()
        guide_bwd(p, g, source, tidx, sv_g, dlogit, dims, base, red, chain=chain)


def warm_up(fn):
    s = torch.cuda.Stream()
    s.wait_stream(torch.cuda.current_stream())
    with torch.cuda.stream(s):
        for _ in range(2):
            fn()
    torch.cuda.current_stream().wait_stream(s)
    torch.cuda.synchronize()
```

### gpt-st_amd/ops.py

```python
import ctypes
from typing import Any, NamedTuple

import torch

from . import _C

MODE_TIME, MODE_NODE, MODE_SHARED = 0, 1, 2
PRO_NONE, PRO_DPRE = 0, 1
EPI_PLAIN, EPI_RES_LRELU, EPI_ADD_DPRE, EPI_LRELU, EPI_ADD_PREMUL, EPI_PREMUL = 0, 1, 2, 3, 4, 5

_p = _C.ptr


TIMER = None
LAST_CALL = {}


CALL_LOCK = None


def _call(name, *args, tag="", nbytes=0):
    if CALL_LOCK is not None:
        with CALL_LOCK:
            _C.lib().call(name, *args, _C.stream())
# ... 89 lines not shown
class PoolJob(NamedTuple):
    kind: int
    emb: Any
    dW: Any
    pool: Any
    out: Any
    R: int
    K: int
    cols: int
    nsplit: int
    ldx: int


class PoolJobs:
    FWD, BWD_POOL, BWD_EMB, GRAM = 0, 1, 2, 3

    def __init__(self):
        self.jobs = []
        self.post = []

    def fwd(self, emb, pool, out=None):
        _chk(emb, pool, out)
        R, K = emb.shape
        if out is None:
            out = torch.empty((R,) + tuple(pool.shape[1:]), device=emb.device, dtype=torch.float32)
        self.jobs.append(PoolJob(self.FWD, emb, None, pool, out, R, K, pool.numel() // K, 1, 0))
        return out

    def gram(self, emb, pool, out, A=None):
        _chk(emb, pool, out, A)
        R, K = emb.shape
        cols = pool.numel() // K
        assert cols % 12 == 0 and out.numel() == R * 144 and out.is_contiguous()
        if _C.lib().value("gptst_pool_jobs_gram_rows", K, cols) <= 0:
            assert A is not None and A.numel() == R * cols, "gram job does not fit and no forward output was given"
            self.post.append((A, out, R, cols // 12))
            return out
        self.jobs.append(PoolJob(self.GRAM, emb, None, pool, out, R, K, cols, 1, 0))
        return out

    @staticmethod
    def _ldx(dW, cols):
        assert dW.is_cuda and dW.dtype == torch.float32 and dW.dim() == 2 and dW.shape[1] == cols and dW.stride(1) == 1, (dW.shape, dW.stride(), cols)
        return dW.stride(0)

    def bwd_pool(self, emb, dW, dpool, nsplit=1):
        _chk(emb, dpool)
        R, K = emb.shape
        cols = dpool.numel() // K
        self.jobs.append(PoolJob(self.BWD_POOL, emb, dW, None, dpool, R, K, cols, nsplit, self._ldx(dW, cols)))

    def bwd_emb(self, dW, pool, demb, nsplit=1):
        _chk(pool, demb)
        R, K = demb.shape
        cols = pool.numel() // K
        self.jobs.append(PoolJob(self.BWD_EMB, None, dW, pool, demb, R, K, cols, nsplit, self._ldx(dW, cols)))

    @staticmethod
    def columns(js, fields=PoolJob._fields):
        return [len(js)] + [(_ptrs0 if f in ("emb", "dW", "pool", "out") else _ints)([getattr(j, f) for j in js])
                            for f in PoolJob._fields if f in fields]

    def launch(self):
        js, self.jobs = self.jobs, []
        post, self.post = self.post, []
        if js:
            _call("gptst_pool_jobs", *self.columns(js), nbytes=_nb(*[t for j in js for t in (j.emb, j.dW, j.pool, j.out)]))
        for A, G, rows, Hm in post:
            _call("gptst_gram_fwd", _p(A), _p(G), rows, Hm)


def _ptrs0(ts):
    return (ctypes.c_void_p * len(ts))(*[(t.data_ptr() if t is not None else None) for t in ts])


def apply(A, W, mode, BT, N, bias=None, resid=None, A2=None, transw=False, pro=PRO_NONE, epi=EPI_PLAIN, colsum=None,
          out=None, resid2=None):
    _chk(A, W, bias, resid, A2, resid2)
    C = A.shape[-1]
    if out is None:
        out = torch.empty_like(A)
    cs, ns = None, 0
    if colsum is not None:
        G = BT if mode == MODE_TIME else (N if mode == MODE_NODE else 1)
        ns = _C.lib().value("gptst_apply_nsplit", mode, BT, N, C)
        cs = torch.empty(ns * G, C, device=A.device, dtype=torch.float32)
    _call("gptst_apply", _p(A), _p(A2), _p(W), int(W.dim() == 3), int(transw), _p(bias), _p(resid), _p(resid2), _p(out), _p(cs),
          mode, pro, epi, BT, N, C, tag="mode%d pro%d epi%d" % (mode, pro, epi), nbytes=_nb(A, A2, W, bias, resid, resid2, out))
    if colsum is True:
        return out, cs, ns
    if colsum is not None:
        colsum.add_(cs.view(ns, -1, C).sum(0).view_as(colsum))
    return out


def apply_wgrad(dOut, Y, S, W, mode, BT, N, premul=False):
    _chk(dOut, Y, S, W)
    C = dOut.shape[-1]
    G = BT if mode == MODE_TIME else N
    ns = _C.lib().value("gptst_apply_wgrad_nsplit", mode, BT, N)
    dS = torch.empty_like(dOut)
    dW = torch.empty(ns * G, C * C, device=dOut.device, dtype=torch.float32)
    db = torch.empty(ns * G, C, device=dOut.device, dtype=torch.float32)
    _call("gptst_apply_wgrad", _p(dOut), _p(Y), _p(S), _p(W), _p(dS), _p(dW), _p(db), int(premul), mode, BT, N, C, tag="mode%d" % mode,
          nbytes=_nb(dOut, Y, S, W, dS, dW))
    return dS, dW, db, ns


def linear_bwd(dY, X, Wp, dOut, out, premul=False):
    _chk(dY, X, Wp, dOut, out)
    rows, C = dY.shape
    ns = _C.lib().value("gptst_linear_bwd_nsplit", rows)
    dX = torch.empty_like(dY)
    dWp = torch.empty(ns, C * C, device=dY.device, dtype=torch.float32)
    dbp = torch.empty(ns, C, device=dY.device, dtype=torch.float32)
    _call("gptst_linear_bwd", _p(dY), _p(X), _p(Wp), _p(dOut), _p(out), _p(dX), _p(dWp), _p(dbp), int(premul), rows, C,
          nbytes=_nb(dY, X, dOut, out, dX, dWp))
    return dX, dWp, dbp, ns


def wgrad_nsplit(mode, BT, N, C=64):
    return _C.lib().value("gptst_wgrad_nsplit", mode, BT, N, C)


def wgrad(A, D, mode, BT, N, D2=None, pro=PRO_NONE, colsum_a=False, colsum_d=False):
    _chk(A, D, D2)
    C = A.shape[-1]
    ns = wgrad_nsplit(mode, BT, N, C)
    G = BT if mode == MODE_TIME else (N if mode == MODE_NODE else 1)
    if colsum_a or colsum_d:
        dW = torch.empty(ns * G, C * C + C, device=A.device, dtype=torch.float32)
        _call("gptst_wgrad_colsum", _p(A), _p(D), _p(D2), _p(dW), mode, pro, 1 if colsum_a else 2, BT, N, C,
              tag="mode%d pro%d cs" % (mode, pro), nbytes=_nb(A, D, D2, dW))
    else:
        dW = torch.empty(ns * G, C, C, device=A.device, dtype=torch.float32)
        _call("gptst_wgrad", _p(A), _p(D), _p(D2), _p(dW), mode, pro, BT, N, C, tag="mode%d pro%d" % (mode, pro), nbytes=_nb(A, D, D2, dW))
    return dW, ns


def gram_fwd(A):
    N, Hm, T = A.shape
    G = torch.empty(N, T, T, device=A.device, dtype=torch.float32)
    _call("gptst_gram_fwd", _p(A), _p(G), N, Hm)
    return G


def gram_bwd(A, dG, out=None, layers=1, nsplit=1):
    LN, Hm, T = A.shape
    dA = out if out is not None else torch.empty_like(A)
    _call("gptst_gram_bwd", _p(A), _p(dG), _p(dA), layers, LN // layers, Hm, nsplit)
    return dA


def tmix(X, G, dOut=None, Y=None):
    _chk(X, G, dOut, Y)
    B, T, N, C = X.shape
    out = torch.empty_like(X)
    _call("gptst_tmix", _p(X), _p(G), _p(dOut), _p(Y), _p(out), B, T, N, C, tag="bwd" if dOut is not None else "fwd",
          nbytes=_nb(X, G, dOut, Y, out))
    return out


def hypertem_fwd(X, G, Wbt, bbt, want_R=True):
    _chk(X, G, Wbt, bbt)
    B, T, N, C = X.shape
    R = torch.empty_like(X) if want_R else None
    out = torch.empty_like(X)
    _call("gptst_hypertem_fwd", _p(X), _p(G), _p(Wbt), _p(bbt), _p(R), _p(out), B, T, N, C, nbytes=_nb(X, G, Wbt, bbt, R, out))
    return R, out


def hypertem_chain_fwd(X, stages, want_R=True, guest=None):
    B, T, N, C = X.shape
    _chk(X, *[t for st in stages for t in st])
    f = lambda: torch.empty(B, T, N, C, device=X.device, dtype=torch.float32)
    Rs = [f() if want_R else None for _ in stages]
    outs = [f() for _ in stages]
    chain = (_p(X), len(stages), _ptrs0([st[0] for st in stages]), _ptrs0([st[1] for st in stages]), _ptrs0([st[2] for st in stages]),
             _ptrs0(Rs), _ptrs0(outs), B, T, N, C)
    if guest is None:
        _call("gptst_hypertem_chain_fwd", *chain, tag="x%d" % len(stages), nbytes=_nb(X, *Rs, *outs))
    else:
        stage, ts, v0, v1, HS, lda, w = guest
        _chk(*ts)
        _call("gptst_hypertem_chain_fwd_kl", *chain, stage, _ptrs0(ts), v0, v1, HS, lda, float(w), tag="x%d+kl%d" % (len(stages), stage),
              nbytes=_nb(X, *Rs, *outs))
    return list(zip(Rs, outs))


def kl_guest_blocks(stage, B, T, N):
    return _C.lib().value("gptst_kl_guest_blocks", stage, B, T, N)


def encin_ht1_fwd(source, base, mask, fill, w, bi, G, Wbt, bbt):
    B, T, N, F = source.shape
    C = Wbt.shape[-1]
    assert base == 1
    _chk(source, mask, w, bi, G, Wbt, bbt)
    f = dict(device=source.device, dtype=torch.float32)
    out, ab, wv = torch.empty(B, T, N, C, **f), torch.empty(B * T * N, 2, **f), torch.empty(B * T, 2 * C, **f)
    _call("gptst_encin_ht1_fwd", _p(source), F, _p(mask), float(fill), _p(w), _p(bi), _p(G), _p(Wbt), _p(bbt), _p(out), _p(ab), _p(wv), B, T, N, C,
          nbytes=_nb(Wbt, out))
    return out, ab, wv


def encin_ht1_bwd(dPre, source, mask, fill, w, bi, Wbt, ab, wv, dG=None):
    B, T, N, F = source.shape
    C = Wbt.shape[-1]
    _chk(dPre, source, mask, w, bi, Wbt, ab, wv, dG)
    f = dict(device=source.device, dtype=torch.float32)
    dWb, dinp = torch.empty(B * T, C * C + C, **f), torch.empty(B * T, 2 * C, **f)
    if dG is None:
        dG = torch.empty(B, N, T, T, **f)
    _call("gptst_encin_ht1_bwd", _p(dPre), _p(source), F, _p(mask), float(fill), _p(w), _p(bi), _p(Wbt), _p(ab), _p(wv), _p(dWb), _p(dG), _p(dinp),
          B, T, N, C, nbytes=_nb(dPre, Wbt, dWb, dG))
    return dWb, dG, dinp


def guide_in_fwd(source, w1, b1, Wn, bn):
    B, T, N, F = source.shape
    C = Wn.shape[-1]
    _chk(source, w1, b1, Wn, bn)
    h1 = torch.empty(B * T * N, C, device=source.device, dtype=torch.float32)
    _call("gptst_guide_in_fwd", _p(source), F, _p(w1), _p(b1), _p(Wn), _p(bn), _p(h1), B * T, N, C, nbytes=_nb(Wn, h1))
    return h1


def guide_head_fwd(source, w1, b1, Wn, bn, Wbt, bbt, W3, b3):
    B, T, N, F = source.shape
    C, J = Wn.shape[-1], W3.shape[0]
    if C != 64 or J > 16:
        return None
    _chk(source, w1, b1, Wn, bn, Wbt, bbt, W3, b3)
    dev = source.device
    f = dict(device=dev, dtype=torch.float32)
    uc = torch.empty(N, 2 * C, **f)
    h1, h2 = torch.empty(B * T * N, C, **f), torch.empty(B * T * N, C, **f)
    prob = torch.empty(B * T * N, J, **f)
    label = torch.empty(B * T * N, device=dev, dtype=torch.int32)
    _call("gptst_guide_head_fwd", _p(source), F, _p(w1), _p(b1), _p(Wn), _p(bn), _p(Wbt), _p(bbt), _p(W3), _p(b3), _p(uc), _p(h1), _p(h2), _p(prob),
          _p(label), B * T, N, C, J, nbytes=_nb(Wbt, h1, h2, prob))
    return h1, h2, prob, label


def guide_in_bwd(dPre, source, w1, b1, Wn):
    B, T, N, F = source.shape
    C = Wn.shape[-1]
    _chk(dPre, source, w1, b1, Wn)
    f = dict(device=source.device, dtype=torch.float32)
    dWb, dinp = torch.empty(N, C * C + C, **f), torch.empty(N, 2 * C, **f)
    _call("gptst_guide_in_bwd", _p(dPre), _p(source), F, _p(w1), _p(b1), _p(Wn), _p(dWb), _p(dinp), B * T, N, C, nbytes=_nb(dPre, Wn, dWb))
    return dWb, dinp


def hypertem_ntiles(N):
    return _C.lib().value("gptst_hypertem_ntiles", N)


def hypertem_bwd(dOut, Y, X, G, Wbt, dG=None, want_dbias=True, premul=False):
    _chk(dOut, Y, X, G, Wbt, dG)
    B, T, N, C = X.shape
    dX = torch.empty_like(X)
    nt = hypertem_ntiles(N)
    dbias = torch.empty(nt * B * T, C, device=X.device, dtype=torch.float32) if want_dbias else None
    if dG is None:
        dG = torch.empty(B, N, T, T, device=X.device, dtype=torch.float32)
    _call("gptst_hypertem_bwd", _p(dOut), _p(Y), _p(X), _p(G), _p(Wbt), _p(dX), _p(dbias), _p(dG), int(premul), B, T, N, C,
          nbytes=_nb(dOut, Y, X, G, Wbt, dX))
    return dX, dbias, dG


def hypertem_bwd_wgrad(dOut, Y, X, G, Wbt, R, dG=None, premul=False):
    _chk(dOut, Y, X, G, Wbt, R, dG)
    B, T, N, C = X.shape
    dX = torch.empty_like(X)
    if dG is None:
        dG = torch.empty(B, N, T, T, device=X.device, dtype=torch.float32)
    ns = wgrad_nsplit(MODE_TIME, B * T, N, C)
    dWb = torch.empty(ns * B * T, C * C + C, device=X.device, dtype=torch.float32)
    _call("gptst_hypertem_bwd_wgrad", _p(dOut), _p(Y), _p(X), _p(G), _p(Wbt), _p(R), _p(dX), _p(dG), _p(dWb), int(premul), B, T, N, C,
          nbytes=_nb(dOut, Y, X, G, Wbt, R, dX, dWb))
    return dX, dWb, ns, dG


def hypertem_bwd_pair(dOut1, X1, G1, Wbt1, R1, X0, G0, Wbt0, R0, dG1, dG0, cnt, dWb1=None):
    _chk(dOut1, X1, G1, Wbt1, R1, X0, G0, Wbt0, R0, dG1, dG0, cnt, dWb1)
    B, T, N, C = X1.shape
    if C != 64:
        return None
    dXmid, dX0 = torch.empty_like(X1), torch.empty_like(X0)
    ns = wgrad_nsplit(MODE_TIME, B * T, N, C)
    dWb0 = torch.empty(ns * B * T, C * C + C, device=X1.device, dtype=torch.float32)
    if dWb1 is None:
        dWb1 = torch.empty_like(dWb0)
    assert dWb1.shape == dWb0.shape
    try:
        _call("gptst_hypertem_bwd_pair", _p(dOut1), _p(X1), _p(G1), _p(Wbt1), _p(R1), _p(X0), _p(G0), _p(Wbt0), _p(R0), _p(dXmid), _p(dX0),
              _p(dG1), _p(dG0), _p(dWb1), _p(dWb0), _p(cnt), B, T, N, C, nbytes=_nb(dOut1, X1, R1, X0, R0, dXmid, dX0, dWb0, dWb1))
    except _C.GptstError as e:
        if e.code != _C.ESHAPE:
            raise
        return None
    return dXmid, dX0, dWb1, dWb0, ns


def tmix_bwd(dR, X, G, dOut, Y, dG=None):
    _chk(dR, X, G, dOut, Y, dG)
    B, T, N, C = X.shape
    dX = torch.empty_like(X)
    if dG is None:
        dG = torch.empty(N, T, T, device=X.device, dtype=torch.float32)
    _call("gptst_tmix_bwd", _p(dR), _p(X), _p(G), _p(dOut), _p(Y), _p(dX), _p(dG), B, T, N, C, nbytes=_nb(dR, X, dOut, Y, dX))
    return dX, dG


def tmix_bwd_chain(dR, X, G, dPre, premul=False, dG=None):
    _chk(dR, X, G, dPre, dG)
    B, T, N, C = X.shape
    dX = torch.empty_like(X)
    if dG is None:
        dG = torch.empty(N, T, T, device=X.device, dtype=torch.float32)
    _call("gptst_tmix_bwd_chain", _p(dR), _p(X), _p(G), _p(dPre), int(bool(premul)), _p(dX), _p(dG), B, T, N, C, nbytes=_nb(dR, X, dPre, dX))
    return dX, dG


def tmix_dgraph(dR, X, out=None):
    _chk(dR, X, out)
    B, T, N, C = X.shape
    dG = out if out is not None else torch.empty(N, T, T, device=X.device, dtype=torch.float32)
    _call("gptst_tmix_dgraph", _p(dR), _p(X), _p(dG), B, T, N, C, nbytes=_nb(dR, X, dG))
    return dG


FORCE_CAP_BIG = False


def cap_fits_lds(N, C, HS):
    return (not FORCE_CAP_BIG) and bool(_C.lib().value("gptst_cap_fits_lds", N, C, HS))


def _lds_or_stream(lds_call, stream_call):
    if FORCE_CAP_BIG:
        return stream_call()
    try:
        return lds_call()
    except _C.GptstError as e:
        if e.code != _C.ESHAPE:
            raise
        return stream_call()


def _capbig_linear(X, Wp, bp):
    B, T, N, C = X.shape
    return apply(X.reshape(-1, C), Wp, MODE_SHARED, B * T, N, bias=bp, transw=True)


def _capbig_type1(cs, P, S, BT, HS, N, C, reduce_nodes=None):
    _call("gptst_capbig_type1", _p(cs), _p(P), _p(S), BT, HS, N, C)
    if reduce_nodes is not None:
        reduce_nodes(S)


def _cap_route_fwd_big(X, Wp, bp, dadj, HS, R, reduce_nodes=None):
    B, T, N, C = X.shape
    BT, dev = B * T, X.device
    P = _capbig_linear(X, Wp, bp)
    _call("gptst_capbig_squash_rows", _p(P), BT * N, C)
    f = dict(device=dev, dtype=torch.float32)
    cs, c = torch.empty(BT, HS, N, **f), torch.empty(BT, HS, N, **f)
    S, V0, V, s = (torch.empty(BT, HS, C, **f) for _ in range(4))
    bl = torch.zeros(BT, HS, N, **f)
    _call("gptst_capbig_softmax", None, _p(dadj), _p(cs), BT, HS, N, 0, 1)
    _capbig_type1(cs, P, S, BT, HS, N, C, reduce_nodes)
    _call("gptst_capbig_post", _p(S), None, _p(V0), BT * HS, C, 1)
    for r in range(R):
        if r > 0:
            _call("gptst_capbig_type2", _p(V), _p(P), _p(bl), BT, HS, N, C)
        _call("gptst_capbig_softmax", _p(bl), None, _p(cs), BT, HS, N, 1, 0)
        _capbig_type1(cs, P, S, BT, HS, N, C, reduce_nodes)
        _call("gptst_capbig_post", _p(S), _p(V0), _p(V), BT * HS, C, 2)
    if R > 0:
        _call("gptst_capbig_type2", _p(V), _p(P), _p(bl), BT, HS, N, C)
    _call("gptst_capbig_softmax", _p(bl), _p(dadj), _p(c), BT, HS, N, 1, 1)
    _capbig_type1(c, P, S, BT, HS, N, C, reduce_nodes)
    _call("gptst_capbig_post", _p(S), None, _p(s), BT * HS, C, 0)
    return c, s


CAP_FLOW = True


def capflow_ok(HS, C):
    return CAP_FLOW and bool(_C.lib().value("gptst_capflow_supported", HS, C))


def _capflow_post(part, nparts, prow, V0, Vout, mode, BT, HS, C, reduce_nodes):
    if reduce_nodes is not None:
        full = torch.empty(BT, prow, C, device=part.device, dtype=torch.float32)
        _call("gptst_capflow_post", _p(part), nparts, prow, None, _p(full), 3, BT, HS, C)
        reduce_nodes(full)
        part, nparts = full, 1
    _call("gptst_capflow_post", _p(part), nparts, prow, _p(V0), _p(Vout), mode, BT, HS, C)


def _cap_route_fwd_flow(X, Wp, bp, dadj, HS, R, reduce_nodes=None):
    B, T, N, C = X.shape
    BT, dev = B * T, X.device
    f = dict(device=dev, dtype=torch.float32)
    Y = _capbig_linear(X, Wp, bp)
    P = torch.empty_like(Y)
    npart = _C.lib().value("gptst_capflow_nparts", N)
    part = torch.empty(BT, npart, HS + 1, C, **f)
    c = torch.empty(BT, HS, N, **f)
    V0, V, s = (torch.empty(BT, HS, C, **f) for _ in range(3))
    _call("gptst_capflow_squash", _p(Y), _p(dadj), _p(P), _p(part), BT, HS, N, C)
    _capflow_post(part, npart, HS + 1, V0, V if R > 0 else None, 0, BT, HS, C, reduce_nodes)
    bl = None
    for r in range(1, R):
        bl2 = torch.empty(BT, HS, N, **f)
        _call("gptst_capflow_route", _p(P), _p(V), _p(bl), _p(bl2), None, None, None, _p(part), BT, HS, N, C)
        bl = bl2
        _capflow_post(part, npart, HS, V0, V, 1, BT, HS, C, reduce_nodes)
    _call("gptst_capflow_route", _p(P), _p(V) if R > 0 else None, _p(bl), None, _p(dadj), None, _p(c), _p(part), BT, HS, N, C)
    _capflow_post(part, npart, HS, None, s, 2, BT, HS, C, reduce_nodes)
    return c, s, Y


def cap_route_fwd(X, Wp, bp, dadj, HS, R, reduce_nodes=None, want_Y=False):
    _chk(X, Wp, bp, dadj)
    B, T, N, C = X.shape

    def stream():
        if capflow_ok(HS, C):
            return _cap_route_fwd_flow(X, Wp, bp, dadj, HS, R, reduce_nodes)
        return _cap_route_fwd_big(X, Wp, bp, dadj, HS, R, reduce_nodes) + (None,)

    def lds():
        c = torch.empty(B * T, HS, N, device=X.device, dtype=torch.float32)
        s = torch.empty(B * T, HS, C, device=X.device, dtype=torch.float32)
        _call("gptst_cap_route_fwd", _p(X), _p(Wp), _p(bp), _p(dadj), _p(c), _p(s), B * T, N, C, HS, R, nbytes=_nb(X, Wp, bp, dadj, c, s))
        return c, s, None
    out = stream() if reduce_nodes is not None else _lds_or_stream(lds, stream)
    return out if want_Y else out[:2]


def cap_cross_fwd(s, dyn, tmpl, B, T, HS, HT):
    _chk(s, dyn, tmpl)
    C = s.shape[-1]
    v = torch.empty_like(s)
    Ht = torch.empty(B, HT, C, device=s.device, dtype=torch.float32)
    Rt = torch.empty_like(s)
    _call("gptst_cap_cross_fwd", _p(s), _p(dyn), _p(tmpl), _p(v), _p(Ht), _p(Rt), B, T, C, HS, HT)
    return v, Ht, Rt


def cap_cross_rec_fwd(s, dyn, tmpl, c, B, T, N, HS, HT):
    _chk(s, dyn, tmpl, c)
    C = s.shape[-1]
    if C != 64 or FORCE_CAP_BIG:
        return None
    v, Rt = torch.empty_like(s), torch.empty_like(s)
    Ht = torch.empty(B, HT, C, device=s.device, dtype=torch.float32)
    rec = torch.empty(B * T * N, C, device=s.device, dtype=torch.float32)
    try:
        _call("gptst_cap_cross_rec_fwd", _p(s), _p(dyn), _p(tmpl), _p(c), _p(v), _p(Ht), _p(Rt), _p(rec), B, T, N, C, HS, HT,
              nbytes=_nb(s, dyn, c, v, Rt, rec))
    except _C.GptstError as e:
        if e.code != _C.ESHAPE:
            raise
        return None
    return v, Ht, Rt, rec


def cap_cross_bwd(dv, s, Rt, Ht, dyn, tmpl, B, T, HS, HT):
    _chk(dv, s, Rt, Ht, dyn, tmpl)
    C = s.shape[-1]
    dS = torch.empty_like(s)
    ddyn = torch.empty_like(dyn)
    nws = _C.lib().value("gptst_cap_cross_ws_floats", B, T, C, HS, HT)
    ws = torch.empty(nws, device=s.device, dtype=torch.float32) if nws else None
    _call("gptst_cap_cross_bwd", _p(dv), _p(s), _p(Rt), _p(Ht), _p(dyn), _p(tmpl), _p(dS), _p(ddyn), _p(ws), B, T, C, HS, HT)
    return dS, ddyn


def cap_rec_fwd(c, v, N, C):
    _chk(c, v)
    BT, HS = c.shape[0], c.shape[1]
    rec = torch.empty(BT * N, C, device=c.device, dtype=torch.float32)

    def stream():
        if capflow_ok(HS, C):
            return _call("gptst_capflow_rec_fwd", _p(c), _p(v), _p(rec), BT, HS, N, C)
        return _call("gptst_capbig_rec_fwd", _p(c), _p(v), _p(rec), BT, HS, N, C)
    _lds_or_stream(lambda: _call("gptst_cap_rec_fwd", _p(c), _p(v), _p(rec), BT, N, C, HS, nbytes=_nb(c, v, rec)), stream)
    return rec


def cap_rec_bwd(drec, c, v, reduce_nodes=None):
    _chk(drec, c, v)
    BT, HS, N = c.shape
    C = v.shape[-1]
    dc1 = torch.empty_like(c)
    dv = torch.empty_like(v)

    def stream():
        if capflow_ok(HS, C):
            npart = _C.lib().value("gptst_capflow_nparts", N)
            part = torch.empty(BT, npart, HS, C, device=c.device, dtype=torch.float32)
            _call("gptst_capflow_route", _p(drec), _p(v), None, _p(dc1), None, _p(c), None, _p(part), BT, HS, N, C)
            _capflow_post(part, npart, HS, None, dv, 2, BT, HS, C, reduce_nodes)
            return
        _call("gptst_capbig_rec_bwd_dc", _p(drec), _p(v), _p(dc1), BT, HS, N, C)
        _capbig_type1(c, drec, dv, BT, HS, N, C, reduce_nodes)
    if reduce_nodes is not None or (HS > 16 and capflow_ok(HS, C)):
        stream()
    else:
        _lds_or_stream(lambda: _call("gptst_cap_rec_bwd", _p(drec), _p(c), _p(v), _p(dc1), _p(dv), BT, N, C, HS, nbytes=_nb(drec, c, v, dc1, dv)),
                       stream)
    return dc1, dv


def cap_route_bwd(X, Wp, bp, c, dc1, dS, Y=None):
    _chk(X, Wp, bp, c, dc1, dS)
    B, T, N, C = X.shape
    HS = c.shape[1]
    dY = torch.empty(B * T * N, C, device=X.device, dtype=torch.float32)
    dlogit = torch.empty_like(c)

    def stream():
        Yv = Y if Y is not None else _capbig_linear(X, Wp, bp)
        name = "gptst_capflow_route_bwd" if capflow_ok(HS, C) else "gptst_capbig_route_bwd_rows"
        _call(name, _p(Yv), _p(c), _p(dc1), _p(dS), _p(dY), _p(dlogit), B * T, HS, N, C)
    if Y is not None:
        stream()
    else:
        _lds_or_stream(lambda: _call("gptst_cap_route_bwd", _p(X), _p(Wp), _p(bp), _p(c), _p(dc1), _p(dS), _p(dY), _p(dlogit), B * T, N, C, HS,
                                     nbytes=_nb(X, Wp, bp, c, dc1, dS, dY, dlogit)), stream)
    return dY, dlogit


def cap_cross_route_bwd(X, Wp, bp, c, dc1, dv, s, Rt, Ht, dyn, tmpl, B, T, HS, HT, flags=None):
    _chk(X, Wp, bp, c, dc1, dv, s, Rt, Ht, dyn, tmpl)
    N, C = X.shape[2], X.shape[3]
    if C != 64 or FORCE_CAP_BIG:
        return None
    dY = torch.empty(B * T * N, C, device=X.device, dtype=torch.float32)
    dlogit = torch.empty_like(c)
    ddyn = torch.empty_like(dyn)
    try:
        dS_ws = torch.empty(B * T, HS, C, device=X.device, dtype=torch.float32) if flags is not None else None
        _call("gptst_cap_cross_route_bwd", _p(X), _p(Wp), _p(bp), _p(c), _p(dc1), _p(dv), _p(s), _p(Rt), _p(Ht), _p(dyn), _p(tmpl), _p(dY),
              _p(dlogit), _p(ddyn), _p(dS_ws), _p(flags), B, T, N, C, HS, HT, nbytes=_nb(X, Wp, bp, c, dc1, dv, s, Rt, dY, dlogit))
    except _C.GptstError as e:
        if e.code != _C.ESHAPE:
            raise
        return None
    return dY, dlogit, ddyn


def cap_cross_route_lin_bwd(X, Wp, bp, c, dc1, dv, s, Rt, Ht, dyn, tmpl, dPre, out, premul, B, T, HS, HT, flags=None, jobs=None, nsplit=None):
    _chk(X, Wp, bp, c, dc1, dv, s, Rt, Ht, dyn, tmpl, dPre, out)
    N, C = X.shape[2], X.shape[3]
    if C != 64 or FORCE_CAP_BIG:
        return None
    dev = X.device
    if nsplit is None:
        nsplit = _C.lib().value("gptst_cap_split_units", B * T, N, C, HS)
    rows = B * T + nsplit
    dX = torch.empty(B * T * N, C, device=dev, dtype=torch.float32)
    dWp = torch.empty(rows, C * C, device=dev, dtype=torch.float32)
    dbp = torch.empty(rows, C, device=dev, dtype=torch.float32)
    dlogit = torch.empty_like(c)
    ddyn = torch.empty_like(dyn)
    try:
        dS_ws = torch.empty(B * T, HS, C, device=dev, dtype=torch.float32) if flags is not None else None
        js = jobs.jobs if jobs is not None and not jobs.post and all(j.kind in (PoolJobs.BWD_POOL, PoolJobs.BWD_EMB) for j in jobs.jobs) else []
        _call("gptst_cap_cross_route_lin_bwd_split", _p(X), _p(Wp), _p(bp), _p(c), _p(dc1), _p(dv), _p(s), _p(Rt), _p(Ht), _p(dyn), _p(tmpl),
              _p(dPre), _p(out), int(bool(premul)), _p(dX), _p(dWp), _p(dbp), _p(dlogit), _p(ddyn), _p(dS_ws), _p(flags), B, T, N, C, HS, HT, nsplit,
              *PoolJobs.columns(js), nbytes=_nb(X, Wp, bp, c, dc1, dv, s, Rt, dPre, out, dX, dWp, dlogit))
        if js:
            jobs.jobs = []
    except _C.GptstError as e:
        if e.code != _C.ESHAPE:
            raise
        return None
    return dX, dWp, dbp, dlogit, ddyn


_MASK_WS = {}


def _mask_ws(dev):
    if dev not in _MASK_WS:
        _MASK_WS[dev] = torch.zeros(_C.lib().value("gptst_mask_ws_bytes") // 4, dtype=torch.int32, device=dev)
    return _MASK_WS[dev]


def mask_ws_floats():
    return _C.lib().value("gptst_mask_ws_bytes") // 4


def _fused_jobs(jobs, u24):
    if jobs is None or not (jobs.jobs or jobs.post):
        return None
    if not u24 or jobs.post or any(j.kind not in (PoolJobs.FWD, PoolJobs.GRAM) for j in jobs.jobs):
        jobs.launch()
# ... 229 lines not shown
```

### gpt-st_amd/step.py

```python
import contextlib
import math
import os
import random
from typing import Any, NamedTuple

import torch

from . import engine, ops

DEFER_GEN = os.environ.get("GPTST_DEFER_GEN", "1") == "1"
U24 = os.environ.get("GPTST_MASK_U24", "1") == "1"


class Part1(NamedTuple):
    tidx: Any
    gen: Any
    red: Any
    prob: Any
    sv_g: Any


class PretrainStep:
    RING = 8
    DETERMINISTIC_MODE = True

    def __init__(self, model, args, scaler_mean, scaler_std, batch_size, use_graph=True, dp=None, seed=0, global_mask=True,
                 deterministic=None):
        self.model, self.args = model, args
        self.mean, self.std = float(scaler_mean), float(scaler_std)
        self.B, self.T, self.N = batch_size, args.lag, args.num_nodes
        self.C, self.base, self.HS = args.hidden_dim, args.input_base_dim, args.HS
        self.dims = (self.B, self.T, self.N, self.C)
        self.dev = model.flat.device
        assert self.dev.type == "cuda", "PretrainStep needs the model on an MI355X (no CPU fallback)"
        self.use_graph, self.dp = use_graph, dp
        self.deterministic = self.DETERMINISTIC_MODE and ((os.environ.get("GPTST_DETERMINISTIC", "0") == "1") if deterministic is None else bool(deterministic))
        n = model.flat.numel()
        self.gbuf = torch.zeros(n + 8, device=self.dev)
        self.gflat, self.stats = self.gbuf[:n], self.gbuf[n:]
        self.g = model.views_of(self.gflat)
        self.m, self.v = torch.zeros(n, device=self.dev), torch.zeros(n, device=self.dev)
        M = self.B * self.T * self.N
        self.src = torch.zeros(self.B, self.T, self.N, self.base + 2, device=self.dev)
        self.noise = torch.zeros(M * self.base, device=self.dev)
        self.noise_ar = torch.zeros(2 * M, device=self.dev)
        self.noise_a, self.noise_r = self.noise_ar[:M], self.noise_ar[M:]
        self.hc = torch.zeros(16 + self.HS + 4, dtype=torch.int32, device=self.dev)
        self.hyper = self.hc[:16].view(torch.float32)
        self.ctrl = self.hc[16:16 + self.HS + 2]
        self.rng_words = self.hc[16 + self.HS + 2:]
        self.noise_seed = 1234567 + seed
        self._ring = [self._views(torch.zeros(16 + self.HS + 4, dtype=torch.int32).pin_memory()) for _ in range(self.RING)]
        self._ring_i = 0
        self.phase_kl = False
        self._gK, self._g_last, self._group_failed = 0, None, False
        self.stats_out = torch.zeros(8, device=self.dev)
        self.mask_buf = torch.ones(M * self.base, device=self.dev)
        self.last_mask = None
        self.force_mask = False
        self.tA = self.tB = 0
        self.lr = args.lr_init
        self.rng = random.Random(seed)
        self.graphs = {}
        self._g_graphs = {}
        self._g_fallback = None
        self._graph_comm_failed = False
        self._ctx_keep = []
        self._sws = None
        self.inject_noise = False
        self.global_count_scale = False
        self.node_reduce = None
        self.join_enc_dec = True
        self.safe_mode = False
        self.lost_steps = 0
        self.lost_batches = 0
        self._unseen = []
        self._last_call = None
        self._g_list_cs = None
        self.arena = engine.ZeroArena(self.dev)
        self.fused_tails = os.environ.get("GPTST_FUSED_TAILS", "1") == "1" and engine.fused_tails_ok(model.param_views(), self.C, self.base, self.HS)
        self.W = dp.world if dp is not None else 1
        self.gmask = bool(global_mask) and dp is not None and self.W > 1
        if self.gmask:
            Mg = M * self.W
            self.noise_g = torch.zeros(Mg * self.base, device=self.dev)
            self.noise_ar_g = torch.zeros(2 * Mg, device=self.dev)
            self.noise_a_g, self.noise_r_g = self.noise_ar_g[:Mg], self.noise_ar_g[Mg:]
            self.label_l = torch.zeros(M, dtype=torch.int32, device=self.dev)
            self.label_g = torch.zeros(Mg, dtype=torch.int32, device=self.dev)
        self.always_guide = os.environ.get("GPTST_ALWAYS_GUIDE", "0") == "1"
        self.dp_overlap = (os.environ.get("GPTST_DP_OVERLAP", "0") != "0" and dp is not None and getattr(dp, "capturable", False)
                           and (self.W > 1 or os.environ.get("GPTST_FORCE_DP", "0") == "1"))
        self.dec_lo, self.dec_hi = self._decoder_bucket(model)
        self.rank_weight = 1.0
        self.fork_side = torch.cuda.Stream() if self.dp_overlap else None

    def _needs_exchange(self, phase):
        return self.gmask and phase == 1 and not self.force_mask

    @staticmethod
    def _decoder_bucket(model):
        offs = [(o, model.state_dict()[k].numel()) for k, o in model._offs.items() if k.startswith("decoder.") and o < model.nA]
        lo = min(o for o, _ in offs)
        hi = max(o + (n + 3) // 4 * 4 for o, n in offs)
        assert hi == model.nA and all(o >= lo for o, _ in offs), (lo, hi, model.nA)
        assert not any(lo <= o < hi for k, o in model._offs.items() if not k.startswith("decoder.")), "decoder bucket is not contiguous"
        return lo, hi

    def _allreduce(self, sl):
        if self.rank_weight != 1.0:
            assert not self.use_graph, "a rank weight is baked into a captured graph: tail rounds use eager steppers"
            lost = self.stats[5:6].clone()
            sl.mul_(self.rank_weight)
            self.stats[5:6].copy_(lost)
        self.dp.allreduce_(sl)

    def _bucket_ready(self, k):
        if k == 0:
            self._allreduce(self.gbuf[self.dec_lo:self.dec_hi])
            self._dec_reduced = True

    def _dp_in_graph(self):
        return self.dp is not None and getattr(self.dp, "capturable", False) and not self._graph_comm_failed

    def _part1(self, phase):
        p, dims, base = self.model.param_views(), self.dims, self.base
        engine.CTX.ARENA, engine.CTX.NODE_REDUCE = self.arena, self.node_reduce
        src = self.src
        noise = None if self.inject_noise or self.force_mask else self._noise_buffer(phase)
        tidx = ops.step_begin(self.gbuf, self.arena.begin(zero=False), src, base, noise=noise, rng=self.rng_words)
        need_guide = self._need_guide(phase)
        gen = engine.gen_all(p, tidx, dims, guide=need_guide, defer=DEFER_GEN)
        red = engine.Reductions()
        red.no_carry = self.deterministic
        self._dec_reduced = False
        if self.dp_overlap and self._dp_in_graph():
            red.on_bucket = self._bucket_ready
            red.bucket_inline, red.fork_side = True, self.fork_side
        lowrank = self.fused_tails and engine.chain_ok(dims)
        prob, sv_g = engine.guide_fwd(p, src, tidx, dims, base, gen=gen.guide, lowrank_in=lowrank) if need_guide else (None, None)
        if self._needs_exchange(phase):
            self.label_l.copy_(sv_g.label)
        return Part1(tidx, gen, red, prob, sv_g)

    def _part2(self, phase, ctx):
        if not self.safe_mode:
            return self._part2_impl(phase, ctx)
        with engine.no_handoffs():
            return self._part2_impl(phase, ctx)

    def _part2_impl(self, phase, ctx):
        mdl, p, g, dims, base = self.model, self.model.param_views(), self.g, self.dims, self.base
        a = self.args
        src, tidx, gen, red, prob, sv_g = self.src, ctx.tidx, ctx.gen, ctx.red, ctx.prob, ctx.sv_g
        engine.CTX.ARENA, engine.CTX.NODE_REDUCE = self.arena, self.node_reduce
        pend = gen.pending
        mask = self._make_mask(phase, prob, sv_g.label if sv_g is not None else None, pend)
        if pend is not None:
            pend.launch()
        self.last_mask = mask
        fused = self.fused_tails
        kl, sws = None, None
        if phase == 1 and self._carry_kl(sv_g):
            sws = self._tail_sws()
            kl = engine.KlCarry(p, sv_g, prob, src, dims, 0.1, sws)
        fw = engine.autoencoder_fwd(p, src, mask, dims, base, mdl.num_route, mdl.scaler_zeros, gen=gen, tidx=tidx,
                                    lowrank_in=fused and engine.chain_ok(dims), kl=kl, head=not fused, join=self.join_enc_dec)
        if fused and sws is None:
            sws = self._tail_sws()
        engine.step_bwd(p, g, src, mask, tidx, fw, prob, sv_g, dims, base, mdl.scaler_zeros, red, (self.std, self.mean, a.mape_thresh),
                        self.stats, sws=sws, with_kl=phase == 1, kl=kl)
        self._fold_stats(sws)
        red.flush(tidx)
        engine.CTX.ARENA = engine.CTX.NODE_REDUCE = None
        self._after_backward(phase)

    def _noise_buffer(self, phase):
        if self.gmask:
            return self.noise_g if phase == 0 else self.noise_ar_g
        return self.noise if phase == 0 else self.noise_ar

    def _need_guide(self, phase):
        return phase == 1 or self.always_guide

    def _make_mask(self, phase, prob, label, pend):
        a, base, M = self.args, self.base, self.B * self.T * self.N
        if self.gmask:
            return self._global_mask(phase, jobs=pend)
        if self.force_mask:
            return self.mask_buf
        if phase == 0:
            return ops.mask_random(self.noise, int(M * base * a.mask_ratio), ws=self._mask_ws(), u24=U24, jobs=pend)
        return ops.mask_adaptive(label, None, self.ctrl[:self.HS], self.ctrl[self.HS:], self.noise_a, self.noise_r,
                                 a.ada_type == "all", base, ws=self._mask_ws(), u24=U24, jobs=pend)[2]

    def _fold_stats(self, sws):
        if sws is None:
            return
        if self.dp is None:
            self._sws = sws
        else:
            ops.stats_fold(sws, self.stats)

    def _after_backward(self, phase):
        if self.dp is None:
            self._optim()
        elif self._dp_in_graph():
            if self._dec_reduced:
                self._allreduce(self.gbuf[:self.dec_lo])
                self._allreduce(self.gbuf[self.dec_hi:])
            else:
                self._allreduce(self.gbuf)
            self._optim()

    def _tail_sws(self):
        return self.arena.zeros(ops.tail_parts(self.B * self.T * self.N), 4)

    def _carry_kl(self, sv_g):
        return (self.fused_tails and self.dp is None and not self.global_count_scale and not self.deterministic and not self.safe_mode
                and not self.always_guide and engine.CTX.NODE_REDUCE is None and engine.kl_carry_ok(self.dims, self.HS, sv_g))

    def _mask_ws(self):
        return self.arena.zeros(ops.mask_ws_floats())

    def _global_mask(self, phase, jobs=None):
        a, base, M = self.args, self.base, self.B * self.T * self.N
        Mg = M * self.W
        if self.force_mask:
            return self.mask_buf
        if phase == 0:
            mask_g = ops.mask_random(self.noise_g, int(Mg * base * a.mask_ratio), ws=self._mask_ws(), u24=U24, jobs=jobs)
        else:
            mask_g = ops.mask_adaptive(self.label_g, None, self.ctrl[:self.HS], self.ctrl[self.HS:], self.noise_a_g,
                                       self.noise_r_g, a.ada_type == "all", base, ws=self._mask_ws(), u24=U24, jobs=jobs)[2]
        self.last_mask_global = mask_g
        return self.dp.rows_of(mask_g, M * base)

    def _exchange_labels(self):
        self.dp.gather_labels(self.label_l, out=self.label_g)

    def _optim(self):
        sws, self._sws = self._sws, None
        ops.clip_adam(self.model.flat, self.gflat, self.m, self.v, self.model.nA, self.model.nB, self.hyper, self.stats,
                      stats_out=self.stats_out, sws=sws)

    @contextlib.contextmanager
    def _launch_mode(self):
        if self.DETERMINISTIC_MODE:
            ops.set_deterministic(self.deterministic)
        try:
            yield
        finally:
            if self.DETERMINISTIC_MODE:
                ops.set_deterministic(False)
            engine.CTX.ARENA = engine.CTX.NODE_REDUCE = None

    def _enqueue(self, phase):
        ctx = self._part1(phase)
        if self._needs_exchange(phase):
            self._exchange_labels()
        self._part2(phase, ctx)

    def _body(self, phase):
        with self._launch_mode():
            self._enqueue(phase)

    def _views(self, hc):
        HS = self.HS
        n = hc.numpy()
        return dict(hc=hc, hyper=n[:16].view("float32"), ctrl=n[16:16 + HS + 2], rng=n[16 + HS + 2:], ev=None)

    def _slot(self):
        sl = self._ring[self._ring_i]
        self._ring_i = (self._ring_i + 1) % self.RING
        if sl["ev"] is not None:
            sl["ev"].synchronize()
        return sl

    def _host_prepare(self, phase, epoch, list_c):
        sl = self._slot()
        self._fill(sl, phase, epoch, list_c)
        self.hc.copy_(sl["hc"], non_blocking=True)
        if sl["ev"] is None:
            sl["ev"] = torch.cuda.Event()
        sl["ev"].record()

    def _fill(self, sl, phase, epoch, list_c):
        a = self.args
        self.tA += 1
        if phase == 1:
            self.tB += 1
        self.phase_kl = phase == 1
        b1, b2 = 0.9, 0.999
        tA, tB = self.tA, self.tB
        sl["hyper"][11:13] = (1 - b1, 1 - b2)
        sl["hyper"][:11] = (self.lr / (1 - b1 ** tA), math.sqrt(1 - b2 ** tA),
                            self.lr / (1 - b1 ** tB) if tB else 0.0, math.sqrt(1 - b2 ** tB) if tB else 1.0,
                            b1, b2, 1e-8, float(a.max_grad_norm) if a.grad_norm else 0.0, 1.0 if phase == 1 else 0.0,
                            1.0,
                            1.0)
        sl["rng"][:2] = (self.noise_seed & 0x7FFFFFFF, tA & 0x7FFFFFFF)
        if phase == 1:
            if list_c is None:
                list_c = list(range(self.HS))
                self.rng.shuffle(list_c)
            ada, rnd = self.model.adaptive_counts(self.B * self.T * self.N * (self.W if self.gmask else 1), epoch)
            ada, rnd = self._budgets(ada, rnd, epoch)
            sl["ctrl"][:] = [int(v) for v in list_c] + [int(ada), int(rnd)]
        self._filled_list_c = [int(v) for v in list_c] if phase == 1 else None

    def _budgets(self, ada, rnd, epoch):
        return ada, rnd

    def step(self, source, epoch, noise=None, noise_a=None, noise_r=None, list_c=None, forced_mask=None):
        phase = 0 if epoch <= self.args.change_epoch else 1
        self._g_last = None
        self._g_fallback = None
        if source is not self.src:
            self.src.copy_(source, non_blocking=True)
        inject = noise is not None or noise_a is not None
        if inject:
            n0, na, nr = (self.noise_g, self.noise_a_g, self.noise_r_g) if self.gmask else (self.noise, self.noise_a, self.noise_r)
            if phase == 0:
                n0.copy_(noise.reshape(-1), non_blocking=True)
            else:
                na.copy_(noise_a.reshape(-1), non_blocking=True)
                nr.copy_(noise_r.reshape(-1), non_blocking=True)
        if forced_mask is not None:
            self.mask_buf.copy_(forced_mask.reshape(-1), non_blocking=True)
        self._host_prepare(phase, epoch, list_c)
        self._last_call = (epoch, self._filled_list_c, self.rank_weight) if not inject and forced_mask is None else None
        self._unseen.append(phase)
        if len(self._unseen) > 4096:
            del self._unseen[:2048]
        key = (phase, inject, forced_mask is not None)
        if not self.use_graph:
            self.inject_noise, self.force_mask = inject, forced_mask is not None
            self._body(phase)
        else:
            if key not in self.graphs:
                self._capture(key)
            g1, g2 = self.graphs[key]
            g1.replay()
            if g2 is not None:
                self._exchange_labels()
                g2.replay()
        if self.dp is not None and not self._dp_in_graph():
            self._allreduce(self.gbuf)
            self._optim()

    def _capture(self, key):
        try:
            return self._capture_impl(key)
        except Exception as e:
            if not self._dp_in_graph():
                raise
            import sys
            print("gpt-st_amd: capturing the step with its collectives failed (%s: %s) -> collectives between graph replays"
                  % (type(e).__name__, str(e).splitlines()[0][:200]), file=sys.stderr)
            self._graph_comm_failed = True
            self.graphs.clear()
            self._g_graphs.clear()
            torch.cuda.synchronize()
            return self._capture_impl(key)

    def _capture_impl(self, key):
        phase, inject, forced = key
        self.inject_noise, self.force_mask = inject, forced
        keep = (self.model.flat.clone(), self.m.clone(), self.v.clone())
        engine.warm_up(lambda: self._body(phase))
        try:
            with self._launch_mode():
                g1 = torch.cuda.CUDAGraph()
                if self._needs_exchange(phase) and not self._dp_in_graph():
                    with torch.cuda.graph(g1, capture_error_mode="thread_local"):
                        ctx = self._part1(phase)
                    g2 = torch.cuda.CUDAGraph()
                    with torch.cuda.graph(g2, pool=g1.pool(), capture_error_mode="thread_local"):
                        self._part2(phase, ctx)
                    self._ctx_keep.append(ctx)
                else:
                    g2 = None
                    with torch.cuda.graph(g1, capture_error_mode="thread_local"):
                        self._enqueue(phase)
        finally:
            self.model.flat.copy_(keep[0]); self.m.copy_(keep[1]); self.v.copy_(keep[2])
            torch.cuda.synchronize()
        self.graphs[key] = (g1, g2)

    def group_ok(self, epoch):
        phase = 0 if epoch <= self.args.change_epoch else 1
        if self._group_failed:
            return False
        return self.use_graph and (self.dp is None or self._dp_in_graph()) and not (self._needs_exchange(phase) and not self._dp_in_graph())

    def _group_init(self, K):
        if self._gK == K:
            return
        W = self.hc.numel()
        self._gK = K
        self._g_hc = torch.zeros(K, W, dtype=torch.int32, device=self.dev)
        self._g_src = [torch.zeros_like(self.src) for _ in range(K)]
        self._g_stats = torch.zeros(K, 8, device=self.dev)
        self._g_ring = []
        for _ in range(self.RING):
            hc = torch.zeros(K, W, dtype=torch.int32).pin_memory()
            self._g_ring.append(dict(hc=hc, rows=[self._views(hc[j]) for j in range(K)], ev=None))
        self._g_ring_i = 0
        self._g_graphs = {}

    def group_sources(self, K):
        self._group_init(K)
        return self._g_src

    def _sub(self, j):
        HS = self.HS
        r = self._g_hc[j]
        self.src, self.stats_out = self._g_src[j], self._g_stats[j]
        self.hyper, self.ctrl, self.rng_words = r[:16].view(torch.float32), r[16:16 + HS + 2], r[16 + HS + 2:]

    def step_group(self, sources, epoch, list_cs=None):
        K = len(sources)
        if K == 1 or not self.group_ok(epoch):
            snaps = []
            for j, src in enumerate(sources):
                self.step(src, epoch, list_c=None if list_cs is None else list_cs[j])
                snaps.append((self.stats_out.clone(), bool(self.tB and self.phase_kl), src, self._filled_list_c, epoch))
            self._g_last = None
            self._g_fallback = snaps
            return
        phase = 0 if epoch <= self.args.change_epoch else 1
        self._group_init(K)
        for j, src in enumerate(sources):
            if src is not self._g_src[j]:
                self._g_src[j].copy_(src, non_blocking=True)
        if phase not in self._g_graphs:
            keep = (self.src, self.stats_out, self.hyper, self.ctrl, self.rng_words)
            try:
                self._capture_group(phase, K, epoch)
            except Exception as e:
                import sys
                print("gpt-st_amd: capturing %d steps in one graph failed (%s: %s) -> one replay per step"
                      % (K, type(e).__name__, str(e).splitlines()[0][:200] if str(e) else ""), file=sys.stderr)
                self._group_failed = True
                torch.cuda.synchronize()
                torch.cuda.empty_cache()
            finally:
                self.src, self.stats_out, self.hyper, self.ctrl, self.rng_words = keep
            if self.dp is not None and getattr(self.dp, "world", 1) > 1 and hasattr(self.dp, "max_over_ranks"):
                if self.dp.max_over_ranks(1.0 if self._group_failed else 0.0) > 0 and not self._group_failed:
                    self._group_failed = True
                    self._g_graphs.pop(phase, None)
            if self._group_failed:
                return self.step_group(sources, epoch, list_cs)
        sl = self._g_ring[self._g_ring_i]
        self._g_ring_i = (self._g_ring_i + 1) % self.RING
        if sl["ev"] is not None:
            sl["ev"].synchronize()
        self._g_list_cs = []
        for j in range(K):
            self._fill(sl["rows"][j], phase, epoch, None if list_cs is None else list_cs[j])
            self._g_list_cs.append(self._filled_list_c)
        self._g_epoch = epoch
        self._g_hc.copy_(sl["hc"], non_blocking=True)
        if sl["ev"] is None:
            sl["ev"] = torch.cuda.Event()
        sl["ev"].record()
        self._g_graphs[phase].replay()
        self._g_last = (K, phase)

    def _capture_group(self, phase, K, epoch):
        self.inject_noise, self.force_mask = False, False
        keep = (self.model.flat.clone(), self.m.clone(), self.v.clone())
        st = (self.tA, self.tB, self.phase_kl, self.rng.getstate())
        for j in range(K):
            self._fill(self._g_ring[0]["rows"][j], phase, epoch, None)
        self._g_hc.copy_(self._g_ring[0]["hc"])
        torch.cuda.synchronize()
        self.tA, self.tB, self.phase_kl = st[:3]
        self.rng.setstate(st[3])
        base = torch.cuda.memory_allocated()
        torch.cuda.reset_peak_memory_stats()
        subs = iter(range(K))
        engine.warm_up(lambda: (self._sub(next(subs)), self._body(phase)))
        per_step = torch.cuda.max_memory_allocated() - base
        total = torch.cuda.get_device_properties(self.dev).total_memory
        if self.dp is not None and getattr(self.dp, "world", 1) > 1 and hasattr(self.dp, "max_over_ranks"):
            per_step = int(self.dp.max_over_ranks(per_step))
            total = -int(self.dp.max_over_ranks(-total))
        if per_step * K > 0.25 * total:
            self.model.flat.copy_(keep[0]); self.m.copy_(keep[1]); self.v.copy_(keep[2])
            torch.cuda.synchronize()
            raise RuntimeError("a group of %d steps would need ~%.0f GB of activations (device: %.0f GB)" % (K, per_step * K / 2**30, total / 2**30))
        try:
            with self._launch_mode():
                g = torch.cuda.CUDAGraph()
                with torch.cuda.graph(g, capture_error_mode="thread_local"):
                    for j in range(K):
                        self._sub(j)
                        self._enqueue(phase)
        finally:
            self.model.flat.copy_(keep[0]); self.m.copy_(keep[1]); self.v.copy_(keep[2])
            torch.cuda.synchronize()
        self._g_graphs[phase] = g

    def losses_group(self):
        if self._g_last is None:
            if self._g_fallback:
                snaps, self._g_fallback = self._g_fallback, None
                rows = [(st.cpu(), kl) for st, kl, _, _, _ in snaps]
                out = [self._stats_row(st, kl) for st, kl in rows]
                lost = [j for j, (st, _) in enumerate(rows) if float(st[5]) > 0]
                del self._unseen[:]
                if lost:
                    j0 = lost[0]
                    self._enter_safe_mode(len(snaps) - j0, sum(1 for _, kl, _, _, _ in snaps[j0:] if kl))
                    for j in range(j0, len(snaps)):
                        _, kl, src, lc, ep = snaps[j]
                        self.step(src, ep, list_c=lc)
                        out[j] = self._stats_row(self.stats_out.cpu(), kl)
                    del self._unseen[:]
                return out
            return [self.losses()]
        K, phase = self._g_last
        st = self._g_stats.cpu()
        del self._unseen[:]
        rerun = {}
        if float(st[:, 5].max()) > 0:
            j0 = int((st[:, 5] > 0).float().argmax())
            extra = max(0, int(st[K - 1, 6]) - (K - j0))
            if extra:
                import sys
                self.lost_batches += extra
                print("gpt-st_amd: %d step(s) of earlier groups were skipped too and cannot be repeated (their batches are gone): the optimiser counters "
                      "were taken back, the batches were not trained on" % extra, file=sys.stderr)
            self._enter_safe_mode(K - j0 + extra, (K - j0 + extra) if phase == 1 else 0)
            srcs, lcs, epoch = [t.clone() for t in self._g_src[j0:]], self._g_list_cs[j0:], self._g_epoch
            for j, (src, lc) in enumerate(zip(srcs, lcs)):
                self.step(src, epoch, list_c=lc)
                rerun[j0 + j] = self._stats_row(self.stats_out.cpu(), phase == 1)
            del self._unseen[:]
            self._g_last = (K, phase)
        out = []
        for j in range(K):
            out.append(rerun[j] if j in rerun else self._stats_row(st[j], phase == 1))
        return out

    @staticmethod
    def _stats_row(st, kl):
        lf = float(st[0] / max(float(st[1]), 1.0))
        ls = float(st[2]) * 0.1 if kl else 0.0
        return (lf + ls, lf, ls)

    def _enter_safe_mode(self, nsteps, nkl):
        import sys
        from . import _C
        torch.cuda.synchronize()
        print("gpt-st_amd: an in-launch hand-off expired (the GPU was shared?) — %d skipped step(s) are re-run without hand-off launches; "
              "this stepper stays in that mode" % nsteps, file=sys.stderr)
        self.tA -= nsteps
        self.tB -= nkl
        self.lost_steps += nsteps
        self.safe_mode = True
        self.graphs.clear()
        self._g_graphs.clear()
        _C.lib().call("gptst_handoff_reset")

    def losses(self):
        if self._g_last is not None:
            return self.losses_group()[-1]
        st = self.stats_out.cpu()
        unseen, self._unseen = self._unseen, []
        if float(st[5]) > 0:
            if self._last_call is None:
                raise RuntimeError("an in-launch hand-off expired in a step with injected mask inputs: call _enter_safe_mode() and repeat the step")
            nskip = max(1, min(int(st[6]), len(unseen))) if unseen else 1
            epoch, lc, weight = self._last_call
            self._enter_safe_mode(nskip, sum(unseen[-nskip:]) if unseen else (1 if self.phase_kl else 0))
            if nskip > 1:
                import sys
                self.lost_batches += nskip - 1
                print("gpt-st_amd: %d step(s) enqueued before the last one were skipped with it and cannot be repeated (their batches are gone): "
                      "the optimiser counters were taken back, the batches were not trained on" % (nskip - 1), file=sys.stderr)
            keep_w, self.rank_weight = self.rank_weight, weight
            try:
                self.step(self.src, epoch, list_c=lc)
            finally:
                self.rank_weight = keep_w
            st = self.stats_out.cpu()
            del self._unseen[:]
        return self._stats_row(st, bool(self.tB and self.phase_kl))
```

### include/gptst_hip.h

```cpp
#ifndef GPTST_HIP_H
#define GPTST_HIP_H
#include <stdint.h>

#ifdef __cplusplus
extern "C" {
#endif
#if defined(__GNUC__)
#pragma GCC visibility push(default)
#endif

#define GPTST_ABI_VERSION 16
int gptst_abi_version(void);
int gptst_set_deterministic(int on);
int gptst_handoff_timeouts(int* out);
int gptst_handoff_reset(void);
int gptst_mask_cooperative(int on);
int gptst_mask_cooperative_state(void);
int gptst_set_handoff_guard(int on);

int gptst_poolgen_fwd(const float* emb, const float* pool, float* out, int cols, const float* pool2, float* out2,
                      int cols2, int R, int K, void* stream);
int gptst_poolgen_bwd_pool(const float* emb, const float* dW, float* dpool, int cols, const float* dW2, float* dpool2,
                           int cols2, int R, int nsplit, int K, void* stream);
int gptst_poolgen_bwd_emb(const float* dW, const float* pool, int cols, const float* dW2, const float* pool2, int cols2,
                          float* demb, int R, int nsplit, int K, void* stream);

int gptst_poolgen_fwd_multi(const float* emb, int nprob, const void* pools, const void* outs, const int* cols, int R, int K,
                            void* stream);
int gptst_poolgen_bwd_pool_multi(const float* emb, int nprob, const void* dWs, const void* dpools, const int* cols, const int* nsplit,
                                 int R, int K, void* stream);
int gptst_poolgen_bwd_emb_multi(int nprob, const void* dWs, const void* pools, const int* cols, const int* nsplit, float* demb, int R,
                                int K, void* stream);

int gptst_pool_jobs(int njobs, const int* kind, const void* const* emb, const void* const* x, const void* const* pool,
                    const void* const* out, const int* R, const int* K, const int* cols, const int* nsplit, const int* ldx, void* stream);
int gptst_pool_jobs_gram_rows(int K, int cols);

int gptst_apply_nsplit(int mode, int BT, int N, int C);
int gptst_apply(const float* A, const float* A2, const float* W, int w_per_group, int transw, const float* bias,
                const float* resid, const float* resid2, float* out, float* colsum, int mode, int pro, int epi, int BT,
                int N, int C, void* stream);
int gptst_wgrad_nsplit(int mode, int BT, int N, int C);
int gptst_wgrad(const float* A, const float* D, const float* D2, float* dW, int mode, int pro, int BT, int N, int C,
                void* stream);
int gptst_wgrad_colsum(const float* A, const float* D, const float* D2, float* dW, int mode, int pro, int which, int BT, int N, int C,
                       void* stream);

int gptst_apply_wgrad_nsplit(int mode, int BT, int N);
int gptst_apply_wgrad(const float* dOut, const float* Y, const float* S, const float* W, float* dS, float* dW, float* colsum, int premul,
                      int mode, int BT, int N, int C, void* stream);

int gptst_linear_bwd_nsplit(int rows);
int gptst_linear_bwd(const float* dY, const float* X, const float* Wp, const float* dOut, const float* out, float* dX, float* dWp, float* dbp,
                     int premul, int rows, int C, void* stream);

int gptst_gram_fwd(const float* A, float* G, int N, int Hm, void* stream);
int gptst_gram_bwd(const float* A, const float* dG, float* dA, int L, int N, int Hm, int nsplit, void* stream);
int gptst_tmix(const float* X, const float* G, const float* dOut, const float* Y, float* out, int B, int T, int N, int C,
               void* stream);
int gptst_tmix_dgraph(const float* dR, const float* X, float* dG, int B, int T, int N, int C, void* stream);
int gptst_tmix_bwd(const float* dR, const float* X, const float* G, const float* dOut, const float* Y, float* dX, float* dG, int B, int T,
                   int N, int C, void* stream);
int gptst_tmix_bwd_chain(const float* dR, const float* X, const float* G, const float* dPre, int premul, float* dX, float* dG, int B, int T,
                         int N, int C, void* stream);

int gptst_hypertem_fwd(const float* X, const float* G, const float* Wbt, const float* bbt, float* R_out, float* out, int B, int T,
                       int N, int C, void* stream);
int gptst_hypertem_chain_fwd(const float* X, int nstage, const void* Gs, const void* Wbts, const void* bbts, const void* Rs, const void* outs,
                             int B, int T, int N, int C, void* stream);
int gptst_hypertem_chain_fwd_kl(const float* X, int nstage, const void* Gs, const void* Wbts, const void* bbts, const void* Rs, const void* outs,
                                int B, int T, int N, int C, int stage, const void* ops, int v0, int v1, int HS, int lda, float w, void* stream);
int gptst_kl_guest_blocks(int stage, int B, int T, int N);

int gptst_encin_ht1_fwd(const float* src, int lda, const float* mask, float fill, const float* w, const float* bi, const float* G,
                        const float* Wbt, const float* bbt, float* out, float* ab, float* wv, int B, int T, int N, int C, void* stream);
int gptst_encin_ht1_bwd(const float* dPre, const float* src, int lda, const float* mask, float fill, const float* w, const float* bi,
                        const float* Wbt, const float* ab, const float* wv, float* dWb, float* dG, float* dinp, int B, int T, int N, int C,
                        void* stream);

int gptst_guide_in_fwd(const float* src, int lda, const float* w1, const float* b1, const float* Wn, const float* bn, float* h1, int BT, int N,
                       int C, void* stream);
int gptst_guide_in_bwd(const float* dPre, const float* src, int lda, const float* w1, const float* b1, const float* Wn, float* dWb, float* dinp,
                       int BT, int N, int C, void* stream);
int gptst_guide_uc_floats(int N, int C);
int gptst_guide_head_fwd(const float* src, int lda, const float* w1, const float* b1, const float* Wn, const float* bn, const float* Wbt,
                         const float* bbt, const float* W3, const float* b3, float* uc, float* h1, float* h2, float* prob, int* label,
                         int BT, int N, int C, int J, void* stream);

int gptst_hypertem_ntiles(int N);
int gptst_hypertem_bwd(const float* dOut, const float* Y, const float* X, const float* G, const float* Wbt, float* dX, float* dbias,
                       float* dG, int premul, int B, int T, int N, int C, void* stream);
int gptst_hypertem_bwd_wgrad(const float* dOut, const float* Y, const float* X, const float* G, const float* Wbt, const float* R, float* dX,
                             float* dG, float* dWb, int premul, int B, int T, int N, int C, void* stream);
int gptst_hypertem_bwd_pair(const float* dOut1, const float* X1, const float* G1, const float* Wbt1, const float* R1, const float* X0,
                            const float* G0, const float* Wbt0, const float* R0, float* dXmid, float* dX0, float* dG1, float* dG0,
                            float* dWb1, float* dWb0, void* cnt, int B, int T, int N, int C, void* stream);

int gptst_cap_route_fwd(const float* X, const float* Wp, const float* bp, const float* dadj, float* c_out, float* s_out, int BT, int N,
                        int C, int HS, int R, void* stream);
int gptst_cap_cross_fwd(const float* s, const float* dyn, const float* tmpl, float* v, float* Ht, float* Rt, int B, int T, int C,
                        int HS, int HT, void* stream);
int gptst_cap_cross_ws_floats(int B, int T, int C, int HS, int HT);
int gptst_cap_cross_bwd(const float* dv, const float* s, const float* Rt, const float* Ht, const float* dyn, const float* tmpl,
                        float* dS, float* ddyn, float* ws, int B, int T, int C, int HS, int HT, void* stream);
int gptst_cap_rec_fwd(const float* c, const float* v, float* rec, int BT, int N, int C, int HS, void* stream);
int gptst_cap_cross_rec_fwd(const float* s, const float* dyn, const float* tmpl, const float* c, float* v, float* Ht, float* Rt, float* rec,
                            int B, int T, int N, int C, int HS, int HT, void* stream);
int gptst_cap_rec_bwd(const float* drec, const float* c, const float* v, float* dc1, float* dv, int BT, int N, int C, int HS,
                      void* stream);
int gptst_cap_route_bwd(const float* X, const float* Wp, const float* bp, const float* c, const float* dc1, const float* dS,
                        float* dY, float* dlogit, int BT, int N, int C, int HS, void* stream);
int gptst_cap_cross_route_bwd(const float* X, const float* Wp, const float* bp, const float* c, const float* dc1, const float* dv,
                              const float* s, const float* Rt, const float* Ht, const float* dyn, const float* tmpl, float* dY,
                              float* dlogit, float* ddyn, float* dS_ws, void* flags, int B, int T, int N, int C, int HS, int HT, void* stream);
int gptst_cap_cross_route_lin_bwd(const float* X, const float* Wp, const float* bp, const float* c, const float* dc1, const float* dv,
                                  const float* s, const float* Rt, const float* Ht, const float* dyn, const float* tmpl,
                                  const float* dPre, const float* out, int premul, float* dX, float* dWp, float* dbp, float* dlogit,
                                  float* ddyn, float* dS_ws, void* flags, int B, int T, int N, int C, int HS, int HT, void* stream);
int gptst_cap_route_roles_ok(int B, int T, int N, int C, int HS, int HT);
int gptst_cap_cross_route_lin_bwd_jobs(const float* X, const float* Wp, const float* bp, const float* c, const float* dc1, const float* dv,
                                       const float* s, const float* Rt, const float* Ht, const float* dyn, const float* tmpl,
                                       const float* dPre, const float* out, int premul, float* dX, float* dWp, float* dbp, float* dlogit,
                                       float* ddyn, float* dS_ws, void* flags, int B, int T, int N, int C, int HS, int HT,
                                       int njobs, const int* jkind, const void* const* jemb, const void* const* jx, const void* const* jpool,
                                       const void* const* jout, const int* jR, const int* jK, const int* jcols, const int* jnsplit, const int* jldx,
                                       void* stream);
int gptst_cap_split_units(int BT, int N, int C, int HS);
int gptst_cap_cross_route_lin_bwd_split(const float* X, const float* Wp, const float* bp, const float* c, const float* dc1, const float* dv,
                                        const float* s, const float* Rt, const float* Ht, const float* dyn, const float* tmpl,
                                        const float* dPre, const float* out, int premul, float* dX, float* dWp, float* dbp, float* dlogit,
                                        float* ddyn, float* dS_ws, void* flags, int B, int T, int N, int C, int HS, int HT, int nsplit,
                                        int njobs, const int* jkind, const void* const* jemb, const void* const* jx, const void* const* jpool,
                                        const void* const* jout, const int* jR, const int* jK, const int* jcols, const int* jnsplit, const int* jldx,
                                        void* stream);

int gptst_cap_fits_lds(int N, int C, int HS);
int gptst_capbig_squash_rows(float* Y, long rows, int C, void* stream);
int gptst_capbig_softmax(const float* bl, const float* l0, float* cs, int BT, int HS, int N, int use_bl, int use_l0, void* stream);
int gptst_capbig_type1(const float* cs, const float* P, float* S, int BT, int HS, int N, int C, void* stream);
int gptst_capbig_post(const float* S, const float* V0, float* out, long rows, int C, int post, void* stream);
int gptst_capbig_type2(const float* V, const float* P, float* bl, int BT, int HS, int N, int C, void* stream);
int gptst_capbig_rec_fwd(const float* c, const float* v, float* rec, int BT, int HS, int N, int C, void* stream);
int gptst_capbig_rec_bwd_dc(const float* drec, const float* v, float* dc1, int BT, int HS, int N, int C, void* stream);
int gptst_capbig_route_bwd_rows(const float* Y, const float* c, const float* dc1, const float* dS, float* dY, float* dlogit, int BT,
                                int HS, int N, int C, void* stream);

int gptst_capflow_supported(int HS, int C);
int gptst_capflow_nparts(int N);
int gptst_capflow_squash(const float* Y, const float* dadj, float* P, float* part, int BT, int HS, int N, int C, void* stream);
int gptst_capflow_route(const float* rows, const float* V, const float* bl_in, float* bl_out, const float* l0, const float* c_in,
                        float* c_out, float* part, int BT, int HS, int N, int C, void* stream);
int gptst_capflow_post(const float* part, int nparts, int prow, float* V0, float* Vout, int mode, int BT, int HS, int C, void* stream);
int gptst_capflow_rec_fwd(const float* c, const float* v, float* rec, int BT, int HS, int N, int C, void* stream);
int gptst_capflow_route_bwd(const float* Y, const float* c, const float* dc1, const float* dS, float* dY, float* dlogit, int BT,
                            int HS, int N, int C, void* stream);

int gptst_metrics_accum(const float* out, const float* src, int lda, const float* vis, float sigma, float mu, int has_mae_thresh,
                        float mae_thresh, float mape_thresh, int B, int T, int N, int D, double* sums_t, double* sums_tn, void* stream);

int gptst_mask_ws_bytes(void);
int gptst_mask_random(const float* noise, int M, int k, float* mask, void* ws, int ws_zeroed, void* stream);
int gptst_mask_labels(const float* prob, int rows, int HS, int* label, int* counts, void* stream);
int gptst_mask_adaptive(const int* label, const int* counts, const int* list_c, const int* nums, const float* noise_a,
                        const float* noise_r, int ada_all, int M, int HS, int base, float* m_ada, float* m_rnd, float* mask,
                        void* ws, int ws_zeroed, void* stream);

int gptst_mask_random_u24(const float* noise, int M, int k, float* mask, void* ws, int ws_zeroed, void* stream);
int gptst_mask_adaptive_u24(const int* label, const int* counts, const int* list_c, const int* nums, const float* noise_a, const float* noise_r,
                            int ada_all, int M, int HS, int base, float* m_ada, float* m_rnd, float* mask, void* ws, int ws_zeroed, void* stream);
int gptst_mask_u24_fwd_jobs(int adaptive, const int* label, const int* counts, const int* list_c, const int* nums, const float* noise_a,
                            const float* noise_r, int ada_all, int M, int HS, int base, int k, float* m_ada, float* m_rnd, float* mask, void* ws,
                            int ws_zeroed, int njobs, const int* kind, const void* const* emb, const void* const* pool, const void* const* out,
                            const int* R, const int* K, const int* cols, void* stream);

int gptst_lin_in(const float* a, int lda, const float* mask, float fill, const float* W, int wlayout, const float* b, float* Y,
                 int rows, int J, int C, void* stream);
int gptst_rowdot(const float* X, const float* W, const float* b, float* Z, int rows, int J, int C, int do_softmax, int* label,
                 void* stream);
int gptst_fusion_gate_fwd(const float* F, const float* src, int lda, int base, const float* Ws, const float* bs, const float* Wh,
                          const float* bh, const float* Wo, const float* bo, const float* Wt, const float* bt, float* out, float* z,
                          int rows, int C, void* stream);
int gptst_fusion_gate_bwd(const float* dOut, const float* F, const float* z, const float* src, int lda, int base, const float* Wo,
                          const float* Wt, const float* bt, float* dpre, float* dxd, float* Hm, float* xt, int rows, int C, void* stream);
int gptst_rowouter_ws_floats(int J, int C);
int gptst_rowouter_nparts(int rows);
int gptst_rowouter_part(const float* a, int lda, const float* mask, float fill, const float* X, float* part, int want_asum, int rows,
                        int J, int C, void* stream);
int gptst_rowouter(const float* a, int lda, const float* mask, float fill, const float* X, float* out, int olayout, float* csum,
                   float* asum, float* ws, int rows, int J, int C, void* stream);

int gptst_timefeat_fwd(const float* wd, const float* bd, const float* ww, const float* bw, const float* w1, const float* b1,
                       const float* w2, const float* b2, const float* w3, const float* b3, const float* tidx, float* out, int rows,
                       int K, int E, void* stream);
int gptst_timefeat_bwd(const float* wd, const float* bd, const float* ww, const float* bw, const float* w1, const float* b1,
                       const float* w2, const float* b2, const float* w3, const float* b3, float* gwd, float* gbd, float* gww,
                       float* gbw, float* gw1, float* gb1, float* gw2, float* gb2, float* gw3, float* gb3, const float* tidx,
                       const float* dout, int rows, int K, int E, void* stream);

int gptst_tail_parts(int rows);
int gptst_tail_mae(const float* dec, const float* W, const float* b, const float* src, int lda, const float* mask, float sigma, float mu,
                   float thresh, float* out, float* d_dec, float* part, float* sws, int premul, int rows, int J, int C, void* stream);
int gptst_tail_kl(const float* h2, const float* W3, const float* prob, const float* c, float w, float* d_h2, float* part, float* sws,
                  int premul, int rows, int N, int HS, int C, void* stream);
int gptst_stats_fold(const float* sws, int rows, float* stats, void* stream);

int gptst_timefeat_jobs(int njobs, int bwd, const void* const* params, const void* const* grads, const float* tidx,
                        const void* const* io, const int* rows, const int* K, const int* E, void* stream);

int gptst_step_begin(float* z0, long n0, float* z1, long n1, const float* src, float* tidx, int BT, int N, int lda, int base,
                     float* noise, long n_noise, const int* rng, void* stream);

int gptst_mae_fwd(const float* out, const float* src, int lda, const float* mask, float sigma, float mu, float thresh, int rows,
                  int J, float* stats, void* stream);
int gptst_mae_bwd(const float* out, const float* src, int lda, const float* mask, float sigma, float mu, float thresh, int rows,
                  int J, const float* stats, int normalize, float* dOut, void* stream);
int gptst_kl(const float* prob, const float* c, int rows, int N, int HS, float w, float* dlogit, float* stats, void* stream);
int gptst_clip_adam_ws_floats(void);
int gptst_clip_adam(float* p, const float* g, float* m, float* v, long nA, long nB, const float* hyper, float* stats, float* ws,
                    float* stats_out, const float* sws, int sws_rows, void* stream);

int gptst_layer_bytes(int kind, int B, int T, int N, int C, int d, int Hm, int ds, int HS, int HT, int base, long* saved_bytes,
                      long* scratch_bytes);
int gptst_hypertem_layer_fwd(const float* x, const float* node_emb, const float* time_eb, const float* adj, const float* wpool,
                             const float* bpool, float* out, void* saved, long saved_bytes, int B, int T, int N, int C, int d, int Hm,
                             void* stream);
int gptst_hypertem_layer_bwd(const float* dout, const float* x, const float* out, const float* node_emb, const float* time_eb,
                             const float* adj, const float* wpool, const float* bpool, const void* saved, long saved_bytes, float* dx,
                             float* d_node_emb, float* d_time_eb, float* d_adj, float* d_wpool, float* d_bpool, void* scratch,
                             long scratch_bytes, int B, int T, int N, int C, int d, int Hm, void* stream);
int gptst_cap_layer_fwd(const float* x, const float* node_emb_spg, const float* time_eb_spg, const float* teb, const float* ln_p_w,
                        const float* ln_p_b, const float* adj, const float* t_adj, const float* wspa, const float* bspa,
                        const float* mask_template, float* out, float* c_out, float* dyn_out, void* saved, long saved_bytes, int B, int T,
                        int N, int C, int d, int ds, int HS, int HT, int R, void* stream);
int gptst_cap_layer_bwd(const float* dout, const float* x, const float* out, const float* c, const float* dyn, const float* node_emb_spg,
                        const float* time_eb_spg, const float* teb, const float* ln_p_w, const float* ln_p_b, const float* adj,
                        const float* t_adj, const float* wspa, const float* bspa, const float* mask_template, const void* saved,
                        long saved_bytes, float* dx, float* d_node_emb_spg, float* d_time_eb_spg, float* d_teb, float* d_ln_p_w,
                        float* d_ln_p_b, float* d_adj, float* d_t_adj, float* d_wspa, float* d_bspa, void* scratch, long scratch_bytes, int B,
                        int T, int N, int C, int d, int ds, int HS, int HT, void* stream);
int gptst_mlprl_layer_fwd(const float* a, int lda, const float* time_eb, const float* node_emb, const float* ln1_w, const float* ln1_b,
                          const float* wpool_spa, const float* bpool_spa, const float* wpool_tem, const float* bpool_tem, const float* ln3_w,
                          const float* ln3_b, float* logits, void* saved, long saved_bytes, int B, int T, int N, int C, int d, int base,
                          int HS, void* stream);
int gptst_mlprl_layer_bwd(const float* dlogits, const float* a, int lda, const float* time_eb, const float* node_emb, const float* ln1_w,
                          const float* wpool_spa, const float* bpool_spa, const float* wpool_tem, const float* bpool_tem, const float* ln3_w,
                          const void* saved, long saved_bytes, float* d_time_eb, float* d_node_emb, float* d_ln1_w, float* d_ln1_b,
                          float* d_wpool_spa, float* d_bpool_spa, float* d_wpool_tem, float* d_bpool_tem, float* d_ln3_w, float* d_ln3_b,
                          void* scratch, long scratch_bytes, int B, int T, int N, int C, int d, int base, int HS, void* stream);

int gptst_comm_available(void);
int gptst_comm_unique_id(void* out128);
int gptst_comm_init(int rank, int world, const void* unique_id, void** comm_out);
int gptst_allreduce_f32(void* comm, float* buf, long n, void* stream);
int gptst_allgather_i32(void* comm, const int* send, int* recv, long n, void* stream);
int gptst_comm_count(void* comm, int* out);
int gptst_comm_destroy(void* comm);

#if defined(__GNUC__)
#pragma GCC visibility pop
#endif
#ifdef __cplusplus
}
#endif
#endif
```

Baseline: 925.3 steps/s.

## Fuse last decoder hypertem forward, output head, loss and backward into one turn kernel

Adds a 'turn' kernel that runs the decoder's final hypertemporal forward, the output projection, the masked L1 loss gradient, the head weight-gradient partials, the dPre computation and the hypertem backward stage on a single tile kept resident in LDS. Extra workgroups spin on a per-batch counter and compute the weight gradient once the producing tiles publish. The goal is to remove several kernel launches and the global round trips of R, dec, pred and dPre between forward, loss and backward. It also disables Python GC during graph capture. The costs are a much larger LDS footprint per workgroup, spin-wait handoffs between workgroups, and a path that is only taken in non-deterministic fused mode.

```diff
diff --git a/gpt-st_amd/csrc/hypertem.hip b/gpt-st_amd/csrc/hypertem.hip
--- a/gpt-st_amd/csrc/hypertem.hip
+++ b/gpt-st_amd/csrc/hypertem.hip
@@ -156,8 +156,10 @@
                                                    const float* __restrict__ X, const float* __restrict__ G,
                                                    const float* __restrict__ Wbt, float* __restrict__ dX,
                                                    float* __restrict__ dbias, float* __restrict__ dG, int N, int B, int dbg, int b, int tile,
-                                                   float* __restrict__ smem, float4 (&dp)[HT_T]) {
+                                                   float* __restrict__ smem, float4 (&dp)[HT_T], unsigned sbin0 = 0u, unsigned sbin1 = 0u) {
     constexpr int C = 64, P = C + 4, GP = 145, NT = 16;
+    constexpr bool SLAB = PAIR == 3;
+    static_assert(!SLAB || (PREMUL && !HASY), "the turn's backward is a premultiplying dPre stage");
     float* Ds = smem;
     float* Gs = Ds + HT_T * NT * P;
     const int n0 = tile * NT;
@@ -176,19 +178,22 @@
     const float* __restrict__ Sg = HASY ? Y : X;
     float4 yv[HT_T];
     float gv[9];
-    unsigned sb0 = 0u, sb1 = 0u;
-#pragma unroll
-    for (int t = 0; t < 4; ++t) { if (PAIR != 2) dp[t] = ld4(dOut + rowoff + (size_t)t * N * C); if (HASY || PREMUL) yv[t] = ld4(Sg + rowoff + (size_t)t * N * C); }
-#pragma unroll
-    for (int k = 0; k < 9; ++k) gv[k] = G[min(n0 * 144 + tid + k * 256, N * 144 - 1)];
+    unsigned sb0 = sbin0, sb1 = sbin1;
+#pragma unroll
+    for (int t = 0; t < 4; ++t) { if (PAIR < 2) dp[t] = ld4(dOut + rowoff + (size_t)t * N * C); if ((HASY || PREMUL) && !SLAB) yv[t] = ld4(Sg + rowoff + (size_t)t * N * C); }
+    if (!SLAB) {
+#pragma unroll
+        for (int k = 0; k < 9; ++k) gv[k] = G[min(n0 * 144 + tid + k * 256, N * 144 - 1)];
+    }
     HT_LOAD_WT(wave);
 #pragma unroll
-    for (int t = 4; t < HT_T; ++t) { if (PAIR != 2) dp[t] = ld4(dOut + rowoff + (size_t)t * N * C); if (HASY || PREMUL) yv[t] = ld4(Sg + rowoff + (size_t)t * N * C); }
+    for (int t = 4; t < HT_T; ++t) { if (PAIR < 2) dp[t] = ld4(dOut + rowoff + (size_t)t * N * C); if ((HASY || PREMUL) && !SLAB) yv[t] = ld4(Sg + rowoff + (size_t)t * N * C); }
     SB();
 #pragma unroll
     for (int grp = 0; grp < HT_T / 4; ++grp) {
 #pragma unroll
         for (int tt = 0; tt < 4; ++tt) {
+            if (SLAB) break;
             const int t = 4 * grp + tt;
             float4 v = dp[t];
             if (HASY) v = make_float4(dp[t].x * lrelu_grad_from_out(yv[t].x), dp[t].y * lrelu_grad_from_out(yv[t].y),
@@ -201,16 +206,16 @@
             dp[t] = v;
             st4(Ds + (t * NT + nl) * P + 4 * c4, v);
         }
-        if (grp == 0) {
+        if (grp == 0 && !SLAB) {
 #pragma unroll
             for (int k = 0; k < 9; ++k) {
                 const int i = tid + k * 256;
                 Gs[(i / 144) * GP + i % 144] = (n0 + i / 144 < N) ? gv[k] : 0.f;
             }
         }
-        __syncthreads();
+        if (!SLAB || grp == 0) __syncthreads();
         SB();
-        if (PAIR != 0 && grp == 0) GPTST_STAMP(PAIR == 2 ? 6 : 1);
+        if (PAIR != 0 && grp == 0) GPTST_STAMP(PAIR >= 2 ? 6 : 1);
         const int t = 4 * grp + wave;
         if (HT_DBG(dbg) & 32) continue;
         const size_t g = (size_t)b * HT_T + t;
@@ -247,7 +252,7 @@
             st4(dt + j * P + it * 16 + kk * 4, make_float4(acc[it][0], acc[it][1], acc[it][2], acc[it][3]));
     }
     __syncthreads();
-    if (PAIR != 0) GPTST_STAMP(PAIR == 2 ? 7 : 2);
+    if (PAIR != 0) GPTST_STAMP(PAIR >= 2 ? 7 : 2);
     float4 xg[NT / 4][C / 16];
 #pragma unroll
     for (int i = 0; i < NT / 4; ++i) {
@@ -281,7 +286,7 @@
         }
     }
     SB();
-    if (PAIR != 0) GPTST_STAMP(PAIR == 2 ? 8 : 3);
+    if (PAIR != 0) GPTST_STAMP(PAIR >= 2 ? 8 : 3);
 #pragma unroll
     for (int i = 0; i < NT / 4; ++i) {
         const int nn = wave + 4 * i, n = n0 + nn;
@@ -302,7 +307,7 @@
             if (t < HT_T && u < HT_T && !(HT_DBG(dbg) & 2)) dG[((size_t)b * N + n) * 144 + t * HT_T + u] = acc[r];
         }
     }
-    if (PAIR != 0) GPTST_STAMP(PAIR == 2 ? 9 : 4);
+    if (PAIR != 0) GPTST_STAMP(PAIR >= 2 ? 9 : 4);
 }
 
 template <bool HASY, bool PREMUL>
@@ -829,3 +834,300 @@
     GPTST_CHECK_LAUNCH();
     return GPTST_OK;
 }
+
+struct HtTurnArgs {
+    const float* X; const float* G; const float* Wbt; const float* bbt;
+    const float* Wo; const float* bo; const float* src; const float* mask;
+    float* R; float* pred; float* dPre; float* dX; float* dG; float* dWb; float* part; float* sws; unsigned* cnt;
+    int lda, J; float sigma, mu, thresh;
+};
+constexpr int HT_TURN_LDS_FLOATS = HT_T * 16 * 68 + 16 * 145 + 4 * 16 * 17 + 8 + TL_MAXJ * 64;
+static_assert(HT_TURN_LDS_FLOATS >= WGRAD64_SMEM_FLOATS && HT_TURN_LDS_FLOATS * 4 * HT_OCC <= 160 * 1024, "both roles in one allocation, HT_OCC workgroups per CU");
+static_assert(TL_MAXJ * 64 + TL_MAXJ <= 4 * 16 * 17, "the fold row reuses the waves' at tiles");
+
+template <int U>
+__global__ __launch_bounds__(256, HT_OCC) void hypertem_turn_kernel(HtTurnArgs a, int N, int B, int nH, RowMap rm, int rows_per_split) {
+    constexpr int C = 64, P = C + 4, GP = 145, NT = 16;
+    extern __shared__ __attribute__((aligned(16))) float smem[];
+    const int ntiles = (N + 15) / 16;
+    if ((int)blockIdx.x >= nH) {
+        const int w = blockIdx.x - nH;
+        const int g = w % rm.G, sp = w / rm.G;
+        unsigned* s_ok = reinterpret_cast<unsigned*>(smem);
+        if (threadIdx.x == 0) *s_ok = gptst_wait_ge(a.cnt + g / HT_T, (unsigned)ntiles, &g_handoff_lost_hypertem) ? 1u : 0u;
+        __syncthreads();
+        const bool ok = *s_ok != 0u;
+        __syncthreads();
+        wgrad64_body<PRO_NONE, U, true, true>(a.R, a.dPre, nullptr, a.dWb, rm, rows_per_split, 64 * 64 + 64, 2, g, sp, smem);
+        if (!ok) a.dWb[((size_t)sp * rm.G + g) * (size_t)(64 * 64 + 64) + threadIdx.x] = __int_as_float(0x7fc00000);
+        return;
+    }
+    int b, tile;
+    if (!ht_work_at(blockIdx.x, ntiles, B, b, tile)) return;
+    float* Xs = smem;
+    float* Gs = Xs + HT_T * NT * P;
+    float (*at)[16][17] = reinterpret_cast<float (*)[16][17]>(Gs + NT * GP);
+    float* fold = Gs + NT * GP;
+    float (*reds)[4] = reinterpret_cast<float (*)[4]>(Gs + NT * GP + 4 * 16 * 17);
+    float* Ws = Gs + NT * GP + 4 * 16 * 17 + 8;
+    const int n0 = tile * NT;
+    const int tid = threadIdx.x, lane = tid & 63, wave = tid >> 6;
+    const int j = lane & 15, kk = lane >> 4;
+    const int J = a.J;
+    unsigned sb0 = 0u, sb1 = 0u;
+    {
+        const int nl = tid >> 4, c4 = tid & 15;
+        const int n = min(n0 + nl, N - 1);
+        float4 v[HT_T];
+        float gv[9];
+#pragma unroll
+        for (int t = 0; t < HT_T; ++t) v[t] = ld4(a.X + (((size_t)b * HT_T + t) * N + n) * C + 4 * c4);
+#pragma unroll
+        for (int k = 0; k < 9; ++k) gv[k] = a.G[min(n0 * 144 + tid + k * 256, N * 144 - 1)];
+        const float4 wv = ld4(a.Wo + 4 * min(tid, J * (C / 4) - 1));
+#pragma unroll
+        for (int t = 0; t < HT_T; ++t) {
+            const unsigned m4 = (v[t].x > 0.f ? 1u : 0u) | (v[t].y > 0.f ? 2u : 0u) | (v[t].z > 0.f ? 4u : 0u) | (v[t].w > 0.f ? 8u : 0u);
+            if (t < 8) sb0 |= m4 << (4 * t); else sb1 |= m4 << (4 * (t - 8));
+            st4(Xs + (t * NT + nl) * P + 4 * c4, n0 + nl < N ? v[t] : f4zero());
+        }
+#pragma unroll
+        for (int k = 0; k < 9; ++k) {
+            const int i = tid + k * 256;
+            Gs[(i / 144) * GP + i % 144] = (n0 + i / 144 < N) ? gv[k] : 0.f;
+        }
+        if (tid < J * (C / 4)) st4(Ws + 4 * tid, wv);
+    }
+    asm volatile("" : "+v"(sb0), "+v"(sb1));
+    __syncthreads();
+    SB();
+    float4 bv[C / 16][4];
+    float4 b4;
+#define HTT_LOAD_W(tt) do {                                                                                        \
+        const float* W_ = a.Wbt + ((size_t)b * HT_T + (tt)) * C * C;                                               \
+        _Pragma("unroll") for (int q = 0; q < C / 16; ++q)                                                         \
+            _Pragma("unroll") for (int e = 0; e < 4; ++e) bv[q][e] = ld4(W_ + (size_t)(16 * q + 4 * kk + e) * C + 4 * j); \
+        b4 = ld4(a.bbt + ((size_t)b * HT_T + (tt)) * C + 4 * j);                                                   \
+    } while (0)
+    float4 a4a[C / 16], a4b[C / 16], a4c[C / 16];
+#pragma unroll
+    for (int q = 0; q < C / 16; ++q) { a4a[q] = f4zero(); a4b[q] = f4zero(); a4c[q] = f4zero(); }
+    {
+        const float* gr = Gs + j * GP + wave * HT_T;
+        const float* xr = Xs + j * P + 4 * kk;
+#pragma unroll
+        for (int u = 0; u < HT_T; ++u) {
+            float4 x[C / 16];
+#pragma unroll
+            for (int q = 0; q < C / 16; ++q) x[q] = ld4(xr + u * NT * P + 16 * q);
+            const float g0 = gr[u], g1 = gr[4 * HT_T + u], g2 = gr[8 * HT_T + u];
+#pragma unroll
+            for (int q = 0; q < C / 16; ++q) {
+                a4a[q] = f4fma(g0, x[q], a4a[q]);
+                a4b[q] = f4fma(g1, x[q], a4b[q]);
+                a4c[q] = f4fma(g2, x[q], a4c[q]);
+            }
+            if (u % 3 == 2) SB();
+        }
+    }
+    HTT_LOAD_W(wave);
+    __syncthreads();
+    SB();
+    const __amdgpu_buffer_rsrc_t rsR = __builtin_amdgcn_make_buffer_rsrc(a.R + (size_t)b * HT_T * N * C, 0, HT_T * N * C * 4, 0x00020000);
+    const __amdgpu_buffer_rsrc_t rsD = __builtin_amdgcn_make_buffer_rsrc(a.dPre + (size_t)b * HT_T * N * C, 0, HT_T * N * C * 4, 0x00020000);
+    const int nks = (J + 3) / 4;
+    f32x4 gw[4];
+#pragma unroll
+    for (int ct = 0; ct < 4; ++ct) gw[ct] = (f32x4){0.f, 0.f, 0.f, 0.f};
+    float gb = 0.f, s0 = 0.f, s1 = 0.f;
+#pragma nounroll
+    for (int ti = 0; ti < 3; ++ti) {
+        const int t = wave + 4 * ti;
+        const size_t g = (size_t)b * HT_T + t;
+        float o0[4], o1[4];
+        const float bj = (a.bo != nullptr && j < J) ? a.bo[j] : 0.f;
+#pragma unroll
+        for (int r = 0; r < 4; ++r) {
+            const size_t i = g * N + min(n0 + 4 * kk + r, N - 1);
+            const int jc = min(j, J - 1);
+            o0[r] = a.mask[i * J + jc]; o1[r] = a.src[i * a.lda + jc];
+        }
+        float4 m4[C / 16];
+#pragma unroll
+        for (int q = 0; q < C / 16; ++q) { m4[q] = a4a[q]; a4a[q] = a4b[q]; a4b[q] = a4c[q]; }
+        f32x4 acc[C / 16];
+#pragma unroll
+        for (int ct = 0; ct < C / 16; ++ct) acc[ct] = (f32x4){0.f, 0.f, 0.f, 0.f};
+#pragma unroll
+        for (int q = 0; q < C / 16; ++q) {
+            const float av[4] = {m4[q].x, m4[q].y, m4[q].z, m4[q].w};
+#pragma unroll
+            for (int e = 0; e < 4; ++e) {
+                acc[0] = __builtin_amdgcn_mfma_f32_16x16x4f32(av[e], bv[q][e].x, acc[0], 0, 0, 0);
+                acc[1] = __builtin_amdgcn_mfma_f32_16x16x4f32(av[e], bv[q][e].y, acc[1], 0, 0, 0);
+                acc[2] = __builtin_amdgcn_mfma_f32_16x16x4f32(av[e], bv[q][e].z, acc[2], 0, 0, 0);
+                acc[3] = __builtin_amdgcn_mfma_f32_16x16x4f32(av[e], bv[q][e].w, acc[3], 0, 0, 0);
+            }
+        }
+        SB();
+        const float4 bias = b4;
+        if (ti < 2) HTT_LOAD_W(t + 4);
+        SB();
+        if (n0 + j < N) {
+#pragma unroll
+            for (int q = 0; q < C / 16; ++q) st4_sc1(rsR, (int)(((size_t)t * N + n0 + j) * C + 16 * q + 4 * kk) * 4, m4[q]);
+        }
+        float4 y[4];
+#pragma unroll
+        for (int r = 0; r < 4; ++r) {
+            const int nl = kk * 4 + r;
+            float* xs = Xs + (t * NT + nl) * P + 4 * j;
+            float4 v = f4add(f4add(make_float4(acc[0][r], acc[1][r], acc[2][r], acc[3][r]), bias), ld4(xs));
+            v.x = lrelu(v.x); v.y = lrelu(v.y); v.z = lrelu(v.z); v.w = lrelu(v.w);
+            if (n0 + nl >= N) v = f4zero();
+            y[r] = v;
+            st4(xs, v);
+        }
+        SB();
+        float4 xa[C / 16], bz[C / 16], bd[4];
+#pragma unroll
+        for (int q = 0; q < C / 16; ++q) xa[q] = ld4(Xs + (t * NT + j) * P + 16 * q + 4 * kk);
+#pragma unroll
+        for (int q = 0; q < C / 16; ++q) bz[q] = j < J ? ld4(Ws + j * C + 16 * q + 4 * kk) : f4zero();
+        f32x4 acc0 = {0.f, 0.f, 0.f, 0.f}, acc1 = {0.f, 0.f, 0.f, 0.f};
+#pragma unroll
+        for (int q = 0; q < C / 16; ++q) {
+            acc0 = __builtin_amdgcn_mfma_f32_16x16x4f32(xa[q].x, bz[q].x, acc0, 0, 0, 0);
+            acc1 = __builtin_amdgcn_mfma_f32_16x16x4f32(xa[q].y, bz[q].y, acc1, 0, 0, 0);
+            acc0 = __builtin_amdgcn_mfma_f32_16x16x4f32(xa[q].z, bz[q].z, acc0, 0, 0, 0);
+            acc1 = __builtin_amdgcn_mfma_f32_16x16x4f32(xa[q].w, bz[q].w, acc1, 0, 0, 0);
+        }
+        float av[4];
+#pragma unroll
+        for (int r = 0; r < 4; ++r) {
+            const int n = n0 + 4 * kk + r;
+            av[r] = 0.f;
+            if (n < N && j < J) {
+                const float o = acc0[r] + acc1[r] + bj;
+                const size_t e = (g * N + n) * J + j;
+                const float M = 1.f - o0[r];
+                const float p = (o * a.sigma + a.mu) * M;
+                const float yl = (o1[r] * a.sigma + a.mu) * M;
+                if (yl > a.thresh) {
+                    const float d = p - yl;
+                    s0 += fabsf(d); s1 += 1.f;
+                    av[r] = (d > 0.f ? 1.f : (d < 0.f ? -1.f : 0.f)) * M * a.sigma;
+                }
+                a.pred[e] = o;
+            }
+        }
+#pragma unroll
+        for (int r = 0; r < 4; ++r) {
+            gb += av[r];
+            gw[0] = __builtin_amdgcn_mfma_f32_16x16x4f32(av[r], y[r].x, gw[0], 0, 0, 0);
+            gw[1] = __builtin_amdgcn_mfma_f32_16x16x4f32(av[r], y[r].y, gw[1], 0, 0, 0);
+            gw[2] = __builtin_amdgcn_mfma_f32_16x16x4f32(av[r], y[r].z, gw[2], 0, 0, 0);
+            gw[3] = __builtin_amdgcn_mfma_f32_16x16x4f32(av[r], y[r].w, gw[3], 0, 0, 0);
+        }
+#pragma unroll
+        for (int r = 0; r < 4; ++r) at[wave][4 * kk + r][j] = av[r];
+#pragma unroll
+        for (int q = 0; q < 4; ++q) bd[q] = (4 * q + kk < J) ? ld4(Ws + (4 * q + kk) * C + 4 * j) : f4zero();
+        f32x4 dx[4];
+#pragma unroll
+        for (int ct = 0; ct < 4; ++ct) dx[ct] = (f32x4){0.f, 0.f, 0.f, 0.f};
+#pragma unroll
+        for (int s = 0; s < 4; ++s) {
+            if (s < nks) {
+                const float as = at[wave][j][4 * s + kk];
+                dx[0] = __builtin_amdgcn_mfma_f32_16x16x4f32(as, bd[s].x, dx[0], 0, 0, 0);
+                dx[1] = __builtin_amdgcn_mfma_f32_16x16x4f32(as, bd[s].y, dx[1], 0, 0, 0);
+                dx[2] = __builtin_amdgcn_mfma_f32_16x16x4f32(as, bd[s].z, dx[2], 0, 0, 0);
+                dx[3] = __builtin_amdgcn_mfma_f32_16x16x4f32(as, bd[s].w, dx[3], 0, 0, 0);
+            }
+        }
+#pragma unroll
+        for (int r = 0; r < 4; ++r) {
+            const int nl = kk * 4 + r;
+            float4 v = make_float4(dx[0][r], dx[1][r], dx[2][r], dx[3][r]);
+            v.x *= lrelu_grad_from_out(y[r].x); v.y *= lrelu_grad_from_out(y[r].y);
+            v.z *= lrelu_grad_from_out(y[r].z); v.w *= lrelu_grad_from_out(y[r].w);
+            st4(Xs + (t * NT + nl) * P + 4 * j, v);
+            if (n0 + nl < N) st4_sc1(rsD, (int)(((size_t)t * N + n0 + nl) * C + 4 * j) * 4, v);
+        }
+        SB();
+    }
+#undef HTT_LOAD_W
+    gb += __shfl_xor(gb, 16, 64); gb += __shfl_xor(gb, 32, 64);
+    s0 = group_sum<64>(s0); s1 = group_sum<64>(s1);
+    if (lane == 0) { reds[0][wave] = s0; reds[1][wave] = s1; }
+    __syncthreads();
+#pragma unroll 1
+    for (int w = 0; w < 4; ++w) {
+        if (wave == w) {
+#pragma unroll
+            for (int r = 0; r < 4; ++r) {
+                const int cls = 4 * kk + r;
+                if (cls < J) {
+                    float* f = fold + cls * C + 4 * j;
+                    float4 v = make_float4(gw[0][r], gw[1][r], gw[2][r], gw[3][r]);
+                    if (w != 0) v = f4add(ld4(f), v);
+                    st4(f, v);
+                }
+            }
+            if (kk == 0 && j < J) fold[J * C + j] = w != 0 ? fold[J * C + j] + gb : gb;
+        }
+        __syncthreads();
+    }
+    {
+        float* mine = a.part + ((size_t)b * ntiles + tile) * (J * C + J);
+        for (int o = tid; o < J * C + J; o += 256) mine[o] = fold[o];
+        if (tid == 0) {
+            float* w = a.sws + 4 * ((size_t)b * ntiles + tile);
+            w[0] = (reds[0][0] + reds[0][1]) + (reds[0][2] + reds[0][3]);
+            w[1] = (reds[1][0] + reds[1][1]) + (reds[1][2] + reds[1][3]);
+        }
+    }
+    asm volatile("s_waitcnt vmcnt(0)" ::: "memory");
+    __syncthreads();
+    if (tid == 0) { gptst_publish_fence(); __hip_atomic_fetch_add(a.cnt + b, 1u, __ATOMIC_RELAXED, __HIP_MEMORY_SCOPE_AGENT); }
+    float4 dp[HT_T];
+    {
+        const int nl = tid >> 4, c4 = tid & 15;
+#pragma unroll
+        for (int t = 0; t < HT_T; ++t) dp[t] = ld4(Xs + (t * NT + nl) * P + 4 * c4);
+    }
+    hypertem_bwd_stage<false, true, 3>(nullptr, nullptr, a.X, a.G, a.Wbt, a.dX, nullptr, a.dG, N, B, 0, b, tile, smem, dp, sb0, sb1);
+}
+
+extern "C" int gptst_hypertem_turn_parts(int B, int N) { return B * ((N + 15) / 16); }
+
+extern "C" int gptst_hypertem_turn(const float* X, const float* G, const float* Wbt, const float* bbt, const float* Wo, const float* bo,
+                                   const float* src, int lda, const float* mask, float sigma, float mu, float thresh, float* R, float* pred,
+                                   float* dPre, float* dX, float* dG, float* dWb, float* part, float* sws, void* cnt, int B, int T, int N, int C,
+                                   int J, void* stream) {
+    if (!X || !G || !Wbt || !bbt || !Wo || !src || !mask || !R || !pred || !dPre || !dX || !dG || !dWb || !part || !sws || !cnt || B <= 0 || N <= 0 ||
+        J <= 0 || lda < J)
+        return GPTST_EARG;
+    if (C != 64 || T != HT_T || J > TL_MAXJ || (size_t)B * T * N * C * 4 >= ((size_t)1 << 31)) return GPTST_ESHAPE;
+    const size_t smem = HT_TURN_LDS_FLOATS * sizeof(float);
+    const RowMap rm = make_rowmap(0, B * T, N);
+    const int ns = gptst_wgrad_nsplit(0, B * T, N, 64);
+    int rps = (rm.M + ns - 1) / ns;
+    rps = (rps + 1) & ~1;
+    if ((rm.M + rps - 1) / rps != ns) return GPTST_ESHAPE;
+    const int rows = rps < rm.M ? rps : rm.M, steps = ((rows + 3) / 4 + 3) / 4;
+    const bool u6 = (steps + 5) / 6 * 6 <= (steps + 3) / 4 * 4;
+    const int nH = 8 * ((B + 7) / 8) * ((N + 15) / 16), nW = rm.G * ns;
+    static int done = 0;
+    if (!done) {
+        hipFuncSetAttribute((const void*)hypertem_turn_kernel<4>, hipFuncAttributeMaxDynamicSharedMemorySize, (int)smem);
+        hipFuncSetAttribute((const void*)hypertem_turn_kernel<6>, hipFuncAttributeMaxDynamicSharedMemorySize, (int)smem);
+        done = 1;
+    }
+    const HtTurnArgs a{X, G, Wbt, bbt, Wo, bo, src, mask, R, pred, dPre, dX, dG, dWb, part, sws, (unsigned*)cnt, lda, J, sigma, mu, thresh};
+    if (u6) hipLaunchKernelGGL((hypertem_turn_kernel<6>), dim3(nH + nW), dim3(256), smem, (hipStream_t)stream, a, N, B, nH, rm, rps);
+    else hipLaunchKernelGGL((hypertem_turn_kernel<4>), dim3(nH + nW), dim3(256), smem, (hipStream_t)stream, a, N, B, nH, rm, rps);
+    GPTST_CHECK_LAUNCH();
+    return GPTST_OK;
+}
diff --git a/gpt-st_amd/csrc/wgrad64.h b/gpt-st_amd/csrc/wgrad64.h
--- a/gpt-st_amd/csrc/wgrad64.h
+++ b/gpt-st_amd/csrc/wgrad64.h
@@ -20,7 +20,7 @@
 
 #define WGRAD64_SMEM_FLOATS (4 * 64 * 64 + 4 * 64)
 
-template <int PRO, int U, bool ACQ = false>
+template <int PRO, int U, bool ACQ = false, bool ACQA = false>
 __device__ __forceinline__ void wgrad64_body(const float* __restrict__ A, const float* __restrict__ D, const float* __restrict__ D2,
                                              float* __restrict__ dW, RowMap rm, int rows_per_split, int ostride, int csa, int g, int sp,
                                              float* __restrict__ smem) {
@@ -40,13 +40,14 @@
         for (int cb = 0; cb < 4; ++cb) acc[ca][cb] = (f32x4){0.f, 0.f, 0.f, 0.f};
     float4 sa = f4zero();
     const __amdgpu_buffer_rsrc_t rsD = __builtin_amdgcn_make_buffer_rsrc(const_cast<float*>(D), 0, ACQ ? (int)((size_t)rm.G * rm.M * C * 4) : 0, 0x00020000);
+    const __amdgpu_buffer_rsrc_t rsA = __builtin_amdgcn_make_buffer_rsrc(const_cast<float*>(A), 0, ACQA ? (int)((size_t)rm.G * rm.M * C * 4) : 0, 0x00020000);
     for (int m0 = mbeg; m0 < mend; m0 += 4 * U) {
         float4 a[U], d[U], y[U];
 #pragma unroll
         for (int u = 0; u < U; ++u) {
             const int m = min(m0 + 4 * u + kk, mend - 1);
             const size_t off = ((size_t)g * rm.rs_g + (size_t)m * rm.rs_m) * C + 4 * j;
-            a[u] = ld4(A + off); d[u] = ACQ ? ld4_sc1(rsD, (int)(off * 4)) : ld4(D + off);
+            a[u] = ACQA ? ld4_sc1(rsA, (int)(off * 4)) : ld4(A + off); d[u] = ACQ ? ld4_sc1(rsD, (int)(off * 4)) : ld4(D + off);
             if (PRO == PRO_DPRE) y[u] = ld4(D2 + off);
         }
         SB();
diff --git a/gpt-st_amd/engine.py b/gpt-st_amd/engine.py
--- a/gpt-st_amd/engine.py
+++ b/gpt-st_amd/engine.py
@@ -244,6 +244,7 @@
 CARRY_RED = os.environ.get("GPTST_CARRY_RED", "1") == "1"
 CARRY_MB = float(os.environ.get("GPTST_CARRY_MB", "25"))
 CARRY_KL = os.environ.get("GPTST_CARRY_KL", "1") == "1"
+TURN = os.environ.get("GPTST_TURN", "0") == "1"
 PAIR_UNDER_DP = os.environ.get("GPTST_PAIR_UNDER_DP", "1") == "1"
 PAIR_BWD = os.environ.get("GPTST_PAIR_BWD", "1") == "1"
 
@@ -287,6 +288,35 @@
 
     def __init__(self, saved, dd, dG, dWb):
         self.saved, self.dd, self.dG, self.dWb = saved, dd, dG, dWb
+
+
+class PendingTurn:
+
+    def __init__(self, x, G, Wbt, bbt):
+        self.x, self.G, self.Wbt, self.bbt = x, G, Wbt, bbt
+        self.loss = None
+
+    @property
+    def device(self):
+        return self.x.device
+
+
+def turn_ok(p, dims, base, HS):
+    B, T, N, C = dims
+    return (TURN and pair_bwd_on() and CTX.NODE_REDUCE is None and chain_ok(dims) and chain_fwd_ok(dims) and _ht_fused_bwd(dims)
+            and fused_tails_ok(p, C, base, HS) and _ht_pair_shape_ok(dims) and B * T * N * C * 4 < 2 ** 31)
+
+
+def ht_turn(p, g, pt, dG, dims, red):
+    B, T, N, C = dims
+    source, mask, base, sigma, mu, thresh, sws = pt.loss
+    wo = "decoder.dim_flow_out."
+    r = ops.hypertem_turn(pt.x.view(B, T, N, C), pt.G, pt.Wbt, pt.bbt, p[wo + "weight"], p[wo + "bias"], source, base + 2, mask, sigma, mu, thresh,
+                          sws, _zeros(pt.x, B), dG=dG)
+    assert r is not None, "turn_ok() admitted a shape the launch refuses"
+    red.jobs.bwd_pool(_ones(pt.x.device, r.part.shape[0]), r.part, _wb_view(g[wo + "weight"], g[wo + "bias"]))
+    red.keep.append(r)
+    return r.dX.view(-1, C), _wb_parts(r.dWb, C, r.ns), HtSaved(pt.x, r.R.view(-1, C), None, pt.G, pt.Wbt)
 
 
 def ht_pair_bwd(saved1, saved0, dout, dG1, dG0, dims, dWb1=None):
@@ -542,7 +572,7 @@
     return GenAll(sthcn, gd, jobs if defer else None)
 
 
-def sthcn_fwd(p, pfx, tidx, x, dims, num_route, gen=None, head=None, next_gen=None, kl=None):
+def sthcn_fwd(p, pfx, tidx, x, dims, num_route, gen=None, head=None, next_gen=None, kl=None, defer_h4=False):
     if gen is None:
         gen = gen_all(p, tidx, dims, which=(pfx,), guide=False).sthcn[pfx]
     ht = gen.ht
@@ -562,6 +592,8 @@
     if pairs and next_gen is not None:
         (h4, h1n), xn = ht_chain_fwd(x, [ht(3), next_gen.ht(0)], dims, kl)
         x, nhead = h4.out, (xn, h1n)
+    elif defer_h4:
+        x, h4 = PendingTurn(x, *ht(3)), None
     else:
         x, h4 = hypertem_core_fwd(x, *ht(3), dims)
     return x, c1, SthcnSaved(h1, h2, h3, h4, sc1, sc2, gen.emb, gen, gen.slot), nhead
@@ -616,6 +648,10 @@
         red.keep.append(up)
         if after_pending is not None:
             after_pending()
+    elif isinstance(dout, PendingTurn):
+        assert chain and sv.h4 is None
+        dd, hp4, h4 = ht_turn(p, g, dout, dG_all[3], dims, red)
+        sv = sv._replace(h4=h4)
     else:
         dd, hp4 = hypertem_core_bwd(sv.h4, dout, dG_all[3], dims, chain, True)
     queue_ht(hts[3], hp4)
@@ -870,8 +906,9 @@
 
 
 def autoencoder_fwd(p, source, mask, dims, base, num_route, scaler_zeros, gen=None, tidx=None, lowrank_in=False, kl=None, head=True,
-                    decoder=True, join=True):
-    B, T, N, C = dims
+                    decoder=True, join=True, turn=False):
+    B, T, N, C = dims
+    assert not (turn and head), "the turn launch goes through dim_flow_out itself"
     if tidx is None:
         tidx = source[:, :, 0, base:base + 2].contiguous()
     gen_e, gen_d = (gen.sthcn[ENC], gen.sthcn[DEC] if decoder else None) if gen is not None else (None, None)
@@ -888,7 +925,7 @@
     emb, c1, sv_e, dec_h1 = sthcn_fwd(p, ENC, tidx, x0, dims, num_route, gen=gen_e, head=first, next_gen=gen_d if join else None, kl=kl)
     if not decoder:
         return Forward(emb, c1, None, None, sv_e, None)
-    dec, _, sv_d, _ = sthcn_fwd(p, DEC, tidx, emb, dims, num_route, gen=gen_d, head=dec_h1, kl=kl)
+    dec, _, sv_d, _ = sthcn_fwd(p, DEC, tidx, emb, dims, num_route, gen=gen_d, head=dec_h1, kl=kl, defer_h4=turn)
     out = ops.rowdot(dec, p["decoder.dim_flow_out.weight"], p["decoder.dim_flow_out.bias"]) if head else None
     return Forward(emb, c1, dec, out, sv_e, sv_d)
 
@@ -916,7 +953,12 @@
     if sws is not None:
         chain = chain_ok(dims)
         done = kl.out if kl is not None else KlOut()
-        _, dd = loss_tail(p, g, fw.dec, source, mask, base, sigma, mu, thresh, sws, red, chain=chain)
+        if isinstance(fw.dec, PendingTurn):
+            assert chain
+            dd = fw.dec
+            dd.loss = (source, mask, base, sigma, mu, thresh, sws)
+        else:
+            _, dd = loss_tail(p, g, fw.dec, source, mask, base, sigma, mu, thresh, sws, red, chain=chain)
         model_bwd(p, g, source, mask, tidx, fw.sv_e, fw.sv_d, fw.dec, None, None, dims, base, scaler_zeros, red, dd=dd, chain=chain)
         if with_kl:
             dh2 = kl_head(p, g, sv_g, prob, fw.c1, N, 0.1, sws, red, chain=chain, carried=done.head)
diff --git a/gpt-st_amd/ops.py b/gpt-st_amd/ops.py
--- a/gpt-st_amd/ops.py
+++ b/gpt-st_amd/ops.py
@@ -415,6 +415,48 @@
             raise
         return None
     return dXmid, dX0, dWb1, dWb0, ns
+
+
+def hypertem_turn_parts(B, N):
+    return _C.lib().value("gptst_hypertem_turn_parts", B, N)
+
+
+class Turn(NamedTuple):
+    R: Any
+    pred: Any
+    dPre: Any
+    dX: Any
+    dG: Any
+    dWb: Any
+    ns: int
+    part: Any
+
+
+def hypertem_turn(X, G, Wbt, bbt, Wo, bo, src, lda, mask, sigma, mu, thresh, sws, cnt, dG=None):
+    _chk(X, G, Wbt, bbt, Wo, bo, src, mask, sws, cnt, dG)
+    B, T, N, C = X.shape
+    J = Wo.shape[0]
+    if C != 64 or T != 12 or J > TAIL_MAXJ:
+        return None
+    f = dict(device=X.device, dtype=torch.float32)
+    nparts = hypertem_turn_parts(B, N)
+    assert sws.shape[0] >= nparts and cnt.numel() >= B
+    R, dPre, dX = torch.empty_like(X), torch.empty_like(X), torch.empty_like(X)
+    pred = torch.empty(B * T * N, J, **f)
+    if dG is None:
+        dG = torch.empty(B, N, T, T, **f)
+    ns = wgrad_nsplit(MODE_TIME, B * T, N, C)
+    dWb = torch.empty(ns * B * T, C * C + C, **f)
+    part = torch.empty(nparts, J * C + J, **f)
+    try:
+        _call("gptst_hypertem_turn", _p(X), _p(G), _p(Wbt), _p(bbt), _p(Wo), _p(bo), _p(src), lda, _p(mask), float(sigma), float(mu), float(thresh),
+              _p(R), _p(pred), _p(dPre), _p(dX), _p(dG), _p(dWb), _p(part), _p(sws), _p(cnt), B, T, N, C, J,
+              nbytes=_nb(X, X, R, R, dPre, dPre, dX, Wbt, Wbt, dWb))
+    except _C.GptstError as e:
+        if e.code != _C.ESHAPE:
+            raise
+        return None
+    return Turn(R, pred, dPre, dX, dG, dWb, ns, part)
 
 
 def tmix_bwd(dR, X, G, dOut, Y, dG=None):
diff --git a/gpt-st_amd/step.py b/gpt-st_amd/step.py
--- a/gpt-st_amd/step.py
+++ b/gpt-st_amd/step.py
@@ -1,4 +1,5 @@
 import contextlib
+import gc
 import math
 import os
 import random
@@ -165,7 +166,8 @@
             sws = self._tail_sws()
             kl = engine.KlCarry(p, sv_g, prob, src, dims, 0.1, sws)
         fw = engine.autoencoder_fwd(p, src, mask, dims, base, mdl.num_route, mdl.scaler_zeros, gen=gen, tidx=tidx,
-                                    lowrank_in=fused and engine.chain_ok(dims), kl=kl, head=not fused, join=self.join_enc_dec)
+                                    lowrank_in=fused and engine.chain_ok(dims), kl=kl, head=not fused, join=self.join_enc_dec,
+                                    turn=fused and not self.deterministic and engine.turn_ok(p, dims, base, self.HS))
         if fused and sws is None:
             sws = self._tail_sws()
         engine.step_bwd(p, g, src, mask, tidx, fw, prob, sv_g, dims, base, mdl.scaler_zeros, red, (self.std, self.mean, a.mape_thresh),
@@ -214,7 +216,7 @@
             self._optim()
 
     def _tail_sws(self):
-        return self.arena.zeros(ops.tail_parts(self.B * self.T * self.N), 4)
+        return self.arena.zeros(max(ops.tail_parts(self.B * self.T * self.N), ops.hypertem_turn_parts(self.B, self.N)), 4)
 
     def _carry_kl(self, sv_g):
         return (self.fused_tails and self.dp is None and not self.global_count_scale and not self.deterministic and not self.safe_mode
@@ -364,13 +366,24 @@
             torch.cuda.synchronize()
             return self._capture_impl(key)
 
+    @staticmethod
+    @contextlib.contextmanager
+    def _no_gc():
+        was = gc.isenabled()
+        gc.disable()
+        try:
+            yield
+        finally:
+            if was:
+                gc.enable()
+
     def _capture_impl(self, key):
         phase, inject, forced = key
         self.inject_noise, self.force_mask = inject, forced
         keep = (self.model.flat.clone(), self.m.clone(), self.v.clone())
         engine.warm_up(lambda: self._body(phase))
         try:
-            with self._launch_mode():
+            with self._launch_mode(), self._no_gc():
                 g1 = torch.cuda.CUDAGraph()
                 if self._needs_exchange(phase) and not self._dp_in_graph():
                     with torch.cuda.graph(g1, capture_error_mode="thread_local"):
@@ -493,7 +506,7 @@
             torch.cuda.synchronize()
             raise RuntimeError("a group of %d steps would need ~%.0f GB of activations (device: %.0f GB)" % (K, per_step * K / 2**30, total / 2**30))
         try:
-            with self._launch_mode():
+            with self._launch_mode(), self._no_gc():
                 g = torch.cuda.CUDAGraph()
                 with torch.cuda.graph(g, capture_error_mode="thread_local"):
                     for j in range(K):
diff --git a/include/gptst_hip.h b/include/gptst_hip.h
--- a/include/gptst_hip.h
+++ b/include/gptst_hip.h
@@ -9,7 +9,7 @@
 #pragma GCC visibility push(default)
 #endif
 
-#define GPTST_ABI_VERSION 16
+#define GPTST_ABI_VERSION 17
 int gptst_abi_version(void);
 int gptst_set_deterministic(int on);
 int gptst_handoff_timeouts(int* out);
@@ -95,6 +95,11 @@
 int gptst_hypertem_bwd_pair(const float* dOut1, const float* X1, const float* G1, const float* Wbt1, const float* R1, const float* X0,
                             const float* G0, const float* Wbt0, const float* R0, float* dXmid, float* dX0, float* dG1, float* dG0,
                             float* dWb1, float* dWb0, void* cnt, int B, int T, int N, int C, void* stream);
+int gptst_hypertem_turn(const float* X, const float* G, const float* Wbt, const float* bbt, const float* Wo, const float* bo,
+                        const float* src, int lda, const float* mask, float sigma, float mu, float thresh, float* R, float* pred,
+                        float* dPre, float* dX, float* dG, float* dWb, float* part, float* sws, void* cnt, int B, int T, int N, int C,
+                        int J, void* stream);
+int gptst_hypertem_turn_parts(int B, int N);
 
 int gptst_cap_route_fwd(const float* X, const float* Wp, const float* bp, const float* dadj, float* c_out, float* s_out, int BT, int N,
                         int C, int HS, int R, void* stream);
```

Result: no change. 925.5 steps/s (median of 2 runs) (+0.0%).
